# xiezhy6/PASTA-GAN-plusplus

Hardware: AMD Instinct MI355X
Metric: 512-res try-on images/sec (SynthesisNetwork fwd) (higher is better)
Workload: dtype f32

## Files before the change

include/pasta_gan_ops.h:

```cpp
#ifndef PASTA_GAN_OPS_H
#define PASTA_GAN_OPS_H

#include <stdint.h>

#ifdef __cplusplus
extern "C" {
#endif

#define PG_ABI_VERSION 20

enum pg_dtype { PG_F32 = 0, PG_F16 = 1, PG_BF16 = 2, PG_F64 = 3 };

enum pg_error {
    PG_OK = 0,
    PG_ERR_INVALID_ARG = -1,
    PG_ERR_UNSUPPORTED = -2,
    PG_ERR_TOO_LARGE = -3
};

enum pg_act {
    PG_ACT_LINEAR = 1, PG_ACT_RELU = 2, PG_ACT_LRELU = 3, PG_ACT_TANH = 4, PG_ACT_SIGMOID = 5,
    PG_ACT_ELU = 6, PG_ACT_SELU = 7, PG_ACT_SOFTPLUS = 8, PG_ACT_SWISH = 9
};

int pg_bias_act(const void* x, const void* b, const void* xref, const void* yref, const void* dy, void* y,
                int dtype, int64_t sizeX, int sizeB, int64_t stepB,
                int grad, int act, float alpha, float gain, float clamp, void* stream);
int pg_bias_act_abi_version(void);

int64_t pg_bias_act_grad_bias_workspace(int dtype, int64_t sizeX, int sizeB, int64_t stepB);
int pg_bias_act_grad_bias(const void* dy, const void* yref, void* dx, void* db, void* workspace, int64_t workspace_bytes,
                          int dtype, int64_t sizeX, int sizeB, int64_t stepB,
                          int act, float alpha, float gain, float clamp, void* stream);

int pg_upfirdn2d(const void* x, const float* f, void* y, int dtype,
                 int N, int C, int inH, int inW, const int64_t xstride[4],
                 int fh, int fw, const int64_t fstride[2],
                 int outH, int outW, const int64_t ystride[4],
                 int upx, int upy, int downx, int downy, int padx0, int pady0,
                 int flip, float gain, void* stream);
int pg_upfirdn2d_with_odd_samples(const void* x, const float* f, void* y, float* y_odd, int dtype,
                                  int N, int C, int inH, int inW, const int64_t xstride[4],
                                  int fh, int fw, const int64_t fstride[2],
                                  int outH, int outW, const int64_t ystride[4],
                                  int padx0, int pady0, int flip, float gain, void* stream);
typedef struct pg_fir_epilogue {
    const float* noise;
    int64_t      noise_batch_stride;
    float        noise_gain;
    const float* bias;
    int          act;
    float        alpha;
    float        act_gain;
    float        clamp;
} pg_fir_epilogue;
int pg_upfirdn2d_bias_act(const void* x, const float* f, void* y, int dtype,
                          int N, int C, int inH, int inW, const int64_t xstride[4],
                          int fh, int fw, const int64_t fstride[2],
                          int outH, int outW, const int64_t ystride[4],
                          int upx, int upy, int downx, int downy, int padx0, int pady0,
                          int flip, float gain, const pg_fir_epilogue* epilogue, void* stream);
int pg_upfirdn2d_abi_version(void);

int64_t pg_conv2d_packed_size(int Cout, int Cin, int KH, int KW);
int pg_conv2d_pack_weight(const float* w, float* packed, int Cout, int Cin, int KH, int KW,
                          float scale, int flip_hw, int transpose_oi, void* stream);

typedef struct pg_conv2d_fusion {
    const float* in_scale;
    const float* in_bias;
    int          in_act;
    float        in_alpha;
    float        in_gain;
    float        in_clamp;
    const float* out_scale;
    const float* noise;
    int64_t      noise_batch_stride;
    float        noise_gain;
    const float* bias;
    int          act;
    float        alpha;
    float        gain;
    float        clamp;
    const float* residual;
    const float* spade_x;
    const float* spade_mean;
    const float* spade_rstd;
    const float* x2;
    int          cin_split;
    float*       stats_partial;
} pg_conv2d_fusion;

int pg_conv2d_forward(const float* x, const float* packed_w, float* y,
                      int N, int Cin, int H, int W, int Cout, int KH, int KW,
                      int stride, int pad_y, int pad_x, int OH, int OW,
                      const int64_t ystride[4], int out_step_y, int out_step_x, int out_off_y, int out_off_x,
                      const pg_conv2d_fusion* fusion, void* stream);

int pg_conv2d_splitk_plan(int N, int Cin, int OH, int OW, int Cout, int KH, int KW, int stride);
int pg_conv2d_forward_splitk(const float* x, const float* packed_w, float* y,
                             int N, int Cin, int H, int W, int Cout, int KH, int KW,
                             int stride, int pad_y, int pad_x, int OH, int OW,
                             const int64_t ystride[4], int out_step_y, int out_step_x, int out_off_y, int out_off_x,
                             const pg_conv2d_fusion* fusion, float* workspace, int ksplit, void* stream);

enum { PG_WINO_F2 = 1, PG_WINO_F4 = 2, PG_WINO_F4B = 3, PG_WINO_F4X3 = 4 };
int64_t pg_conv2d_winograd_packed_size(int form, int Cout, int Cin);
int pg_conv2d_winograd_pack_weight(int form, const float* w, float* packed, int Cout, int Cin,
                                   float scale, int flip_hw, int transpose_oi, void* stream);
int pg_conv2d_winograd_forward(int form, const float* x, const float* packed_u, float* y,
                               int N, int Cin, int H, int W, int Cout, int pad_y, int pad_x, int OH, int OW,
                               const int64_t ystride[4], const pg_conv2d_fusion* fusion, void* stream);

int pg_conv2d_winograd4_stats_tiles(int OH, int OW);
int pg_instance_norm_finish(const float* stats_partial, float* mean, float* rstd, int NC, int T, int OH, int OW, float eps, void* stream);

int pg_modconv_dcoefs(const float* w, const float* styles, float* dcoefs,
                      int N, int Cout, int Cin, int KHW, float scale, void* stream);

int pg_modconv_w2(const float* w, float* w2, int Cout, int Cin, int KHW, float scale, void* stream);
int pg_modconv_prep(const float* w2, const float* styles, float* out, float* s_norm, void* s16, int half_dtype,
                    int N, int Cout, int Cin, int normalize, int demodulate, void* stream);

#define PG_MODCONV_PREP_MAX_JOBS 32
typedef struct {
    const float* w2[PG_MODCONV_PREP_MAX_JOBS];
    const float* styles[PG_MODCONV_PREP_MAX_JOBS];
    float*       out[PG_MODCONV_PREP_MAX_JOBS];
    float*       s_norm[PG_MODCONV_PREP_MAX_JOBS];
    void*        s16[PG_MODCONV_PREP_MAX_JOBS];
    int          cout[PG_MODCONV_PREP_MAX_JOBS];
    int          cin[PG_MODCONV_PREP_MAX_JOBS];
    int          flags[PG_MODCONV_PREP_MAX_JOBS];
    int          njobs;
    int          half_dtype;
} pg_modconv_prep_jobs;
int pg_modconv_prep_batched(const pg_modconv_prep_jobs* jobs, int N, void* stream);

int pg_conv2d_up2_forward(const float* x, const float* packed, float* y, int N, int Cin, int H, int W, int Cout,
                          const int64_t ystride[4], const float* in_scale, const float* out_scale, void* stream);
int pg_conv2d_up2_splitk_plan(int N, int Cin, int H, int W, int Cout);
int pg_conv2d_up2_forward_splitk(const float* x, const float* packed, float* y, int N, int Cin, int H, int W, int Cout,
                                 const int64_t ystride[4], const float* in_scale, const float* out_scale, float* workspace, int ksplit, void* stream);

int64_t pg_conv2d_up2x3_packed_size(int Cout, int Cin);
int pg_conv2d_up2x3_pack_weight(const float* packed, void* packed_x3, int Cout, int Cin, void* stream);
int pg_conv2d_up2x3_forward(const float* x, const float* packed, const void* packed_x3, float* y, int N, int Cin, int H, int W, int Cout,
                            const int64_t ystride[4], const float* in_scale, const float* out_scale, float* edge_column, void* stream);

int64_t pg_conv2d_stem7x3_packed_size(int Cout);
int pg_conv2d_stem7x3_pack_weight(const float* w, void* packed, int Cout, float scale, int flip_hw, void* stream);
int pg_conv2d_stem7x3_forward(const float* x, const void* packed, float* y, int N, int H, int W, int Cout, const int64_t ystride[4],
                              const pg_conv2d_fusion* fusion, void* stream);

int64_t pg_conv2d_s2x3_packed_size(int Cout, int Cin);
int pg_conv2d_s2x3_pack_weight(const float* packed, void* packed_x3, int Cout, int Cin, void* stream);
int pg_conv2d_s2x3_forward(const float* x, const void* packed_x3, float* y, int N, int Cin, int H, int W, int Cout, const int64_t ystride[4],
                           const pg_conv2d_fusion* fusion, void* stream);

int pg_conv1x1_small(const float* x, const float* w, const float* styles, const float* bias, const float* skip, float* y,
                     int N, int Cin, int64_t HW, int Cout, float scale, float clamp, void* stream);

int pg_conv1x1_fold_prep(const float* wm, const float* bm, const float* wh, const float* bh, const float* styles, float* w_out, float* b_out,
                         int N, int Cm, int C, int Cout, void* stream);
int pg_conv1x1_fold_heads(const float* x, const float* x2, const float* w, const float* bias, const float* skip, float* y_a, float* y_b,
                          int N, int C1, int C2, int64_t HW, int Cout, int c_a, int n_skip, float clamp, void* stream);

int pg_conv3x3_fold_head(const float* xa, const float* xb, const float* w, const float* bias, const float* skip, float* y,
                         int N, int C, int H, int W, int Cout, float clamp, void* stream);

int pg_conv3x3_cin1(const float* x, const float* w, float* y, int N, int H, int W, int Cout, float scale, int act, void* stream);

int pg_instance_norm_stats(const float* x, float* mean, float* rstd, int NC, int64_t HW, float eps, void* stream);
int pg_spade_norm(const float* x, const float* mean, const float* rstd, const float* gamma, const float* beta,
                  float* y, int NC, int64_t HW, void* stream);

#define PG_STATS16_MAX_CHUNKS 256
int pg_instance_norm_stats_cl16(const void* x, float* mean, float* rstd, float* workspace, int dtype, int N, int64_t HW, int C, float eps, void* stream);
int pg_spade_combine_cl16(const void* x, const float* mean, const float* rstd, const void* gamma_beta, void* y, int dtype, int N, int64_t HW, int C,
                          int act, float alpha, float gain, float clamp, void* stream);

int pg_spade_train_forward(const float* x, const float* mean, const float* rstd, const float* gamma, const float* beta, float* y,
                           int N, int C, int64_t HW, int64_t gamma_sample_stride, int64_t beta_sample_stride, void* stream);
int pg_spade_train_backward(const float* dy, const float* x, const float* mean, const float* rstd, const float* gamma, float* sums,
                            float* dx, float* dgamma, float* dbeta, int N, int C, int64_t HW,
                            int64_t gamma_sample_stride, int64_t dgamma_sample_stride, int64_t dbeta_sample_stride, void* stream);

int pg_spade_masked_sums(const float* feat, const float* mask, const float* denorm_mask, float* sums, float* counts,
                         int N, int C, int H, int W, void* stream);
int pg_spade_feat_assemble(const float* feat_upper, const float* feat_lower, const float* mask_upper, const float* mask_lower,
                           const float* denorm_mask_upper, const float* denorm_mask_lower,
                           const float* sums_upper, const float* sums_lower, const float* counts_upper, const float* counts_lower,
                           float* out, int N, int C, int H, int W, void* stream);
int pg_conv2d_abi_version(void);
int pg_conv2d_reserve_cus(int n);

int pg_conv2d_wgrad_plan(int N, int Cin, int OH, int OW, int Cout, int KH, int KW, int stride);
int pg_conv2d_wgrad(const float* x, const float* dy, float* dw, float* workspace,
                    int N, int Cin, int H, int W, int Cout, int KH, int KW, int stride, int pad_y, int pad_x, int OH, int OW,
                    int splits, void* stream);

int pg_conv2d16_wgrad_plan(int N, int Cin, int OH, int OW, int Cout, int KH, int KW, int stride);
int pg_conv2d16_wgrad(const void* x, const void* dy, float* dw, float* workspace, int dtype,
                      int N, int Cin, int H, int W, int Cout, int KH, int KW, int stride, int pad_y, int pad_x, int OH, int OW,
                      int splits, void* stream);

int pg_split3_bf16_cl(const float* x, void* out, int N, int C, int64_t HW, void* stream);
int pg_conv2d16_wgrad_x3(const void* x3, const void* dy3, float* dw, float* workspace,
                         int N, int Cin, int H, int W, int Cout, int KH, int KW, int stride, int pad_y, int pad_x, int OH, int OW,
                         int splits, void* stream);

int64_t pg_conv2d16_packed_size(int Cout, int Cin, int KH, int KW);
int pg_conv2d16_pack_weight(const float* w, void* packed, int dtype, int Cout, int Cin, int KH, int KW,
                            const int* taps_y, int ntaps_y, const int* taps_x, int ntaps_x,
                            float scale, int flip_hw, int transpose_oi,
                            const float* styles, const float* dcoefs, int nsamples, void* stream);
int pg_conv2d16_pack_weight_grouped(const float* w, void* packed, int dtype, int ngroups, int64_t w_group_stride,
                                    int Cout, int Cin, int KH, int KW, float scale, int flip_hw, int transpose_oi,
                                    const float* styles, const float* dcoefs, int nsamples, void* stream);

#define PG_CONV2D16_PACK_MAX_JOBS 16
typedef struct {
    const float* w[PG_CONV2D16_PACK_MAX_JOBS];
    void*        packed[PG_CONV2D16_PACK_MAX_JOBS];
    const float* styles[PG_CONV2D16_PACK_MAX_JOBS];
    const float* dcoefs[PG_CONV2D16_PACK_MAX_JOBS];
    int          cout[PG_CONV2D16_PACK_MAX_JOBS];
    int          cin[PG_CONV2D16_PACK_MAX_JOBS];
    int          flags[PG_CONV2D16_PACK_MAX_JOBS];
    int          dcoefs_mod[PG_CONV2D16_PACK_MAX_JOBS];
    float        scale[PG_CONV2D16_PACK_MAX_JOBS];
    int          njobs;
    int          nsamples;
    int          dtype;
} pg_conv2d16_pack_jobs;
int pg_conv2d16_pack_weight_batched(const pg_conv2d16_pack_jobs* jobs, void* stream);

typedef struct pg_conv2d16_fusion {
    const float* out_scale;
    const float* noise;
    int64_t      noise_batch_stride;
    float        noise_gain;
    const float* bias;
    int          act;
    float        alpha;
    float        gain;
    float        clamp;
    const void*  residual;
    int          phase_cout;
    int64_t      noise_phase_stride;
} pg_conv2d16_fusion;

int pg_conv2d16_forward(const void* x, const void* packed, void* y, int dtype, int out_dtype,
                        int N, int Cin, int H, int W, int Cout, int KH, int KW,
                        int stride, int pad_y, int pad_x, int OH, int OW, int64_t w_sample_stride,
                        const int64_t ystride[4], int out_step_y, int out_step_x, int out_off_y, int out_off_x,
                        const pg_conv2d16_fusion* fusion, void* stream);

int pg_conv2d16_up2_fused(const void* x, const void* packed, void* y, int dtype, int N, int Cin, int H, int W, int Cout,
                          int64_t w_sample_stride, const int64_t ystride[4], const float fir_x[4],
                          const pg_conv2d16_fusion* fusion, void* stream);

int pg_adam_flat_chunk(void);
int pg_adam_flat_step(float* p, float* g, float* m, float* v, const int* chunks, int nchunks, const float* alive, const float* steps_in, float* steps_out,
                      float lr, float beta1, float beta2, float eps, float nan_value, float posinf_value, float neginf_value, void* stream);

int pg_conv2d16_splitk_plan(int N, int Cin, int OH, int OW, int Cout, int KH, int KW, int stride);
int pg_conv2d16_forward_splitk(const void* x, const void* packed, void* y, int dtype, int out_dtype,
                               int N, int Cin, int H, int W, int Cout, int KH, int KW,
                               int stride, int pad_y, int pad_x, int OH, int OW, int64_t w_sample_stride,
                               const int64_t ystride[4], int out_step_y, int out_step_x, int out_off_y, int out_off_x,
                               const pg_conv2d16_fusion* fusion, float* workspace, int ksplit, void* stream);

int pg_conv1x1_small16(const void* x, const float* w, const float* styles, const float* bias, const float* skip, float* y,
                       int dtype, int N, int Cin, int64_t HW, int Cout, float clamp, int skip_up2_width, void* stream);

// ... 166 lines not shown
```

pasta-gan-plusplus_amd/csrc/conv1x1_fold.hip:

```cpp
#include "pg_common.h"

#ifndef PG_FOLD_MIN_WAVES
#define PG_FOLD_MIN_WAVES 1
#endif
#ifndef PG_FOLD_UNROLL
#define PG_FOLD_UNROLL 8
#endif

namespace {
typedef float f32x4s __attribute__((ext_vector_type(4)));

__global__ __launch_bounds__(256) void conv1x1_fold_prep_kernel(const float* __restrict__ wm, const float* __restrict__ bm, const float* __restrict__ wh,
                                                                const float* __restrict__ bh, const float* __restrict__ styles, float* __restrict__ w_out,
                                                                float* __restrict__ b_out, int Cm, int C, int Cout) {
    const int o = blockIdx.x, n = blockIdx.y;
    const float* who = wh + (int64_t)o * Cm;
    const float* sn = styles ? styles + (int64_t)n * Cm : nullptr;
    for (int c = threadIdx.x; c <= C; c += 256) {
        double acc = 0.0;
        if (c < C) {
            for (int k = 0; k < Cm; k++) acc += (double)who[k] * (double)(sn ? sn[k] : 1.f) * (double)wm[(int64_t)k * C + c];
            w_out[((int64_t)n * Cout + o) * C + c] = (float)acc;
        } else {
            if (bm)
                for (int k = 0; k < Cm; k++) acc += (double)who[k] * (double)(sn ? sn[k] : 1.f) * (double)bm[k];
            b_out[(int64_t)n * Cout + o] = (float)(acc + (double)(bh ? bh[o] : 0.f));
        }
    }
}

template <int CP>
__global__ __launch_bounds__(256, PG_FOLD_MIN_WAVES) void conv1x1_fold_heads_kernel(const float* __restrict__ x, const float* __restrict__ x2, const float* __restrict__ w,
                                                                 const float* __restrict__ bias, const float* __restrict__ skip, float* __restrict__ ya,
                                                                 float* __restrict__ yb, int C1, int C2, int64_t HW4, int Cout, int c_a, int n_skip, float clamp) {
    extern __shared__ __attribute__((aligned(16))) float wl[];
    const int n = blockIdx.y, C = C1 + C2;
    const float* wn = w + (int64_t)n * Cout * C;
    for (int e = threadIdx.x; e < CP * C; e += 256) {
        const int c = e / CP, o = e % CP;
        wl[e] = o < Cout ? wn[o * C + c] : 0.f;
    }
    __syncthreads();
    const float cl = clamp >= 0.f ? clamp : __builtin_inff();
    const f32x4s* xa = (const f32x4s*)x + (int64_t)n * C1 * HW4;
    const f32x4s* xb = (const f32x4s*)x2 + (int64_t)n * C2 * HW4;
    for (int64_t p = (int64_t)blockIdx.x * 256 + threadIdx.x; p < HW4; p += (int64_t)gridDim.x * 256) {
        f32x4s acc[CP];
#pragma unroll
        for (int o = 0; o < CP; o++) acc[o] = (f32x4s){0.f, 0.f, 0.f, 0.f};
        auto mac = [&](const f32x4s& xv, const float* wc) __attribute__((always_inline)) {
#pragma unroll
            for (int q = 0; q < CP / 4; q++) {
                const f32x4s wq = *(const f32x4s*)(wc + 4 * q);
#pragma unroll
                for (int j = 0; j < 4; j++) acc[4 * q + j] += xv * wq[j];
            }
        };
        auto walk = [&](const f32x4s* xs, int Cs, const float* ws) __attribute__((always_inline)) {
            int c0 = 0;
            for (; c0 + PG_FOLD_UNROLL <= Cs; c0 += PG_FOLD_UNROLL) {
                f32x4s v[PG_FOLD_UNROLL];
#pragma unroll
                for (int u = 0; u < PG_FOLD_UNROLL; u++) v[u] = xs[(int64_t)(c0 + u) * HW4 + p];
                __builtin_amdgcn_sched_barrier(0);
#pragma unroll
                for (int u = 0; u < PG_FOLD_UNROLL; u++) mac(v[u], ws + (c0 + u) * CP);
            }
            for (; c0 < Cs; c0++) mac(xs[(int64_t)c0 * HW4 + p], ws + c0 * CP);
        };
        walk(xa, C1, wl);
        walk(xb, C2, wl + C1 * CP);
#pragma unroll
        for (int o = 0; o < CP; o++) {
            if (o < Cout) {
                f32x4s r = acc[o] + bias[(int64_t)n * Cout + o];
#pragma unroll
                for (int e = 0; e < 4; e++) r[e] = fminf(fmaxf(r[e], -cl), cl);
                if (o < n_skip) r += ((const f32x4s*)skip)[((int64_t)n * n_skip + o) * HW4 + p];
                if (o < c_a) ((f32x4s*)ya)[((int64_t)n * c_a + o) * HW4 + p] = r;
                else ((f32x4s*)yb)[((int64_t)n * (Cout - c_a) + (o - c_a)) * HW4 + p] = r;
            }
        }
    }
}
}

PG_EXPORT int pg_conv1x1_fold_prep(const float* wm, const float* bm, const float* wh, const float* bh, const float* styles, float* w_out, float* b_out,
                                   int N, int Cm, int C, int Cout, void* stream) {
    if (!wm || !wh || !w_out || !b_out || N <= 0 || Cm <= 0 || C <= 0 || Cout <= 0) return PG_ERR_INVALID_ARG;
    if (N > 65535) return PG_ERR_TOO_LARGE;
    hipLaunchKernelGGL(conv1x1_fold_prep_kernel, dim3((unsigned)Cout, (unsigned)N), dim3(256), 0, (hipStream_t)stream, wm, bm, wh, bh, styles, w_out, b_out, Cm, C, Cout);
    return pg::launch_status();
}

PG_EXPORT int pg_conv1x1_fold_heads(const float* x, const float* x2, const float* w, const float* bias, const float* skip, float* y_a, float* y_b,
                                    int N, int C1, int C2, int64_t HW, int Cout, int c_a, int n_skip, float clamp, void* stream) {
    if (!x || !w || !bias || !y_a || N <= 0 || C1 <= 0 || C2 < 0 || HW <= 0 || Cout <= 0 || c_a <= 0 || c_a > Cout || n_skip < 0 || n_skip > Cout) return PG_ERR_INVALID_ARG;
    if ((C2 > 0 && !x2) || (c_a < Cout && !y_b) || (n_skip > 0 && !skip)) return PG_ERR_INVALID_ARG;
    const int CP = (Cout + 3) / 4 * 4;
    const size_t lds = (size_t)(C1 + C2) * CP * sizeof(float);
    if (Cout > 16 || HW % 4 != 0 || !pg::aligned16(x) || (C2 > 0 && !pg::aligned16(x2)) || !pg::aligned16(y_a) || (c_a < Cout && !pg::aligned16(y_b)) ||
        (n_skip > 0 && !pg::aligned16(skip)) || lds > 64 * 1024)
        return PG_ERR_UNSUPPORTED;
    if (N > 65535) return PG_ERR_TOO_LARGE;
    const int64_t HW4 = HW / 4;
    int64_t bx = (HW4 + 255) / 256;
    const int64_t cap = (int64_t)pg::num_cu() * 8 / N + 1;
    if (bx > cap) bx = cap;
    const dim3 grid((unsigned)bx, (unsigned)N);
    hipStream_t s = (hipStream_t)stream;
#define PG_FOLD(P) case P: hipLaunchKernelGGL((conv1x1_fold_heads_kernel<P>), grid, dim3(256), lds, s, x, x2, w, bias, skip, y_a, y_b, C1, C2, HW4, Cout, c_a, n_skip, clamp); break;
    switch (CP) { PG_FOLD(4) PG_FOLD(8) PG_FOLD(12) PG_FOLD(16) }
#undef PG_FOLD
    return pg::launch_status();
}
```

pasta-gan-plusplus_amd/csrc/conv2d.hip:

```cpp
#include "conv2d_kernel.h"
#include "bf16x3.h"

namespace {

using namespace pg;
using pgconv::ConvParams;
typedef float f32x4 __attribute__((ext_vector_type(4)));

__global__ __launch_bounds__(256) void pack_weight_kernel(const float* __restrict__ w, float* __restrict__ wp, int Cout, int Cin, int KH, int KW,
                                                          int CinP, int CoutP, float scale, int flip, int transpose_oi) {
    const int T = KH * KW;
    const int64_t total = (int64_t)CinP * T * CoutP;
    for (int64_t i = (int64_t)blockIdx.x * 256 + threadIdx.x; i < total; i += (int64_t)gridDim.x * 256) {
        const int co = (int)(i % CoutP);
        const int tap = (int)((i / CoutP) % T);
        const int ci = (int)(i / ((int64_t)CoutP * T));
        float v = 0.f;
        int ky = tap / KW, kx = tap % KW;
        int cs = ci;
        if (Cin == 3 && KH == 7 && KW == 7 && ci == 3 && (ky & 1) == 0 && ky + 1 < KH) { cs = 2; ky += 1; }
        if (co < Cout && cs < Cin) {
            const int ci = cs;
            if (flip) { ky = KH - 1 - ky; kx = KW - 1 - kx; }
            const int64_t src = transpose_oi ? (((int64_t)ci * Cout + co) * KH + ky) * KW + kx
                                             : (((int64_t)co * Cin + ci) * KH + ky) * KW + kx;
            v = w[src] * scale;
        }
        wp[i] = v;
    }
}

__device__ __forceinline__ float wino_gather(const float* __restrict__ w, int co, int ci, int ky, int kx, int Cout, int Cin, float scale, int flip, int transpose_oi) {
    if (co >= Cout || ci >= Cin) return 0.f;
    const int sy = flip ? 2 - ky : ky, sx = flip ? 2 - kx : kx;
    const int64_t src = transpose_oi ? (((int64_t)ci * Cout + co) * 3 + sy) * 3 + sx
                                     : (((int64_t)co * Cin + ci) * 3 + sy) * 3 + sx;
    return w[src] * scale;
}

__global__ __launch_bounds__(256) void wino_pack_kernel(const float* __restrict__ w, float* __restrict__ up, int Cout, int Cin,
                                                        int CinP, int CoutP, float scale, int flip, int transpose_oi) {
    const int64_t total = (int64_t)CinP * CoutP;
    for (int64_t i = (int64_t)blockIdx.x * 256 + threadIdx.x; i < total; i += (int64_t)gridDim.x * 256) {
        const int co = (int)(i % CoutP), ci = (int)(i / CoutP);
        float g[3][3];
#pragma unroll
        for (int ky = 0; ky < 3; ky++)
#pragma unroll
            for (int kx = 0; kx < 3; kx++) g[ky][kx] = wino_gather(w, co, ci, ky, kx, Cout, Cin, scale, flip, transpose_oi);
        float t[4][3];
#pragma unroll
        for (int kx = 0; kx < 3; kx++) {
            t[0][kx] = g[0][kx];
            t[1][kx] = 0.5f * (g[0][kx] + g[1][kx] + g[2][kx]);
            t[2][kx] = 0.5f * (g[0][kx] - g[1][kx] + g[2][kx]);
            t[3][kx] = g[2][kx];
        }
#pragma unroll
        for (int a = 0; a < 4; a++) {
            const float u[4] = {t[a][0], 0.5f * (t[a][0] + t[a][1] + t[a][2]), 0.5f * (t[a][0] - t[a][1] + t[a][2]), t[a][2]};
#pragma unroll
            for (int b = 0; b < 4; b++) {
                const int64_t dst = ((((int64_t)a * (CoutP / 32) + (co >> 5)) * (CinP / 2) + (ci >> 1)) * 2 + (ci & 1)) * 128 + (co & 31) * 4 + b;
                up[dst] = u[b];
            }
        }
    }
}

struct Wino4PackF4 {
    typedef float word;
    static __device__ __forceinline__ void store(float* __restrict__ up, int co, int ci, int a, int b, int nchunks, double u) {
        const int mb = co >> 6, mt = (co >> 5) & 1, m = co & 31;
        const int k = ci >> 4, cc = ci & 15, pair = cc >> 1, h = cc & 1, quad = pair >> 2, sp = pair & 3;
        const int jg = b / 3, jj = b % 3;
        const int64_t unit = ((int64_t)(mb * 2 + mt) * 6 + a) * nchunks + k;
        up[((((unit * 2 + jg) * 2 + quad) * 3 + jj) * 64 + (h * 32 + m)) * 4 + sp] = (float)u;
    }
};
struct Wino4PackF4B {
    typedef float word;
    static __device__ __forceinline__ void store(float* __restrict__ up, int co, int ci, int a, int b, int nchunks, double u) {
        const int mb = co >> 6, cbk = (co >> 4) & 3, m = co & 15;
        const int k = ci >> 4, cc = ci & 15, j = cc >> 2, kq = cc & 3;
// ... 312 lines not shown
            for (int u = 0; u < 2; u++)
                if (ok[u]) {
#pragma unroll
                    for (int k = 0; k < 4; k++) {
                        const float v = m[u][k] * d[u][k];
#pragma unroll
                        for (int g = 0; g < G; g++) s[g] += f[u][g][k] * v;
                        cnt += v;
                    }
                }
        }
    } else {
        for (int i = threadIdx.x; i < H * W; i += IN_THREADS) {
            const int y = i / W, x = i - y * W;
            const int64_t mi = (int64_t)(2 * y) * (2 * W) + 2 * x;
            const float v = (mp[mi] > 0.9f && dp[mi] > 0.9f) ? 1.f : 0.f;
#pragma unroll
            for (int g = 0; g < G; g++) s[g] += fp[g * HWl + i] * v;
            cnt += v;
        }
    }
    const float Cn = block_sum_1024(cnt, red);
#pragma unroll
    for (int g = 0; g < G; g++) {
        const float S = block_sum_1024(s[g], red);
        if (threadIdx.x == 0) sums[plane0 + g] = S;
    }
    if (threadIdx.x == 0 && plane0 % C == 0) counts[n] = Cn;
}

__global__ __launch_bounds__(256) void spade_feat_assemble_kernel(const float* __restrict__ fu, const float* __restrict__ fl,
                                                                  const float* __restrict__ mu, const float* __restrict__ ml,
                                                                  const float* __restrict__ du, const float* __restrict__ dl,
                                                                  const float* __restrict__ su, const float* __restrict__ sl,
                                                                  const float* __restrict__ cu, const float* __restrict__ cl,
                                                                  float* __restrict__ out, int C, int H, int W, int vec) {
    if (vec) {
        const int n = blockIdx.x;
        const float nu = cu[n] > 10.f ? cu[n] : 65536.f, nl = cl[n] > 10.f ? cl[n] : 65536.f;
        const int64_t mb = (int64_t)n * 4 * H * W, HWl = (int64_t)H * W;
        const int W4 = W / 4, n4 = H * W4;
        for (int i = blockIdx.y * 256 + threadIdx.x; i < n4; i += gridDim.y * 256) {
            const int y = i / W4, x4 = i - y * W4;
            const int64_t mi = mb + (int64_t)(2 * y) * (2 * W) + 8 * x4;
            const f32x4 m_u = even_mask4(mu + mi), m_l = even_mask4(ml + mi), d_u = even_mask4(du + mi), d_l = even_mask4(dl + mi);
            f32x4 r_u, r_l;
#pragma unroll
            for (int k = 0; k < 4; k++) { r_u[k] = m_u[k] - m_u[k] * d_u[k]; r_l[k] = m_l[k] - m_l[k] * d_l[k]; }
            const int cz = (C + gridDim.z - 1) / gridDim.z, c_lo = blockIdx.z * cz, c_hi = c_lo + cz < C ? c_lo + cz : C;
#pragma unroll 4
            for (int c = c_lo; c < c_hi; c++) {
                const int plane = n * C + c;
                const float au = su[plane] / nu, al = sl[plane] / nl;
                const int64_t pb = (int64_t)plane * HWl;
                const f32x4 a = ((const f32x4*)(fu + pb))[i], b = ((const f32x4*)(fl + pb))[i];
                f32x4 o;
#pragma unroll
                for (int k = 0; k < 4; k++) {
                    const float b_u = a[k] * (1.f - r_u[k]) + au * r_u[k];
                    const float b_l = b[k] * (1.f - r_l[k]) + al * r_l[k];
                    o[k] = b_u * m_u[k] + b_l * m_l[k];
                }
                ((f32x4*)(out + pb))[i] = o;
            }
        }
        return;
    }
    const int plane = blockIdx.x, n = plane / C;
    const float nu = cu[n] > 10.f ? cu[n] : 65536.f, nl = cl[n] > 10.f ? cl[n] : 65536.f;
    const float au = su[plane] / nu, al = sl[plane] / nl;
    const int64_t pb = (int64_t)plane * H * W, mb = (int64_t)n * 4 * H * W;
    for (int i = blockIdx.y * 256 + threadIdx.x; i < H * W; i += gridDim.y * 256) {
        const int y = i / W, x = i - y * W;
        const int64_t mi = mb + (int64_t)(2 * y) * (2 * W) + 2 * x;
        const float m_u = mu[mi] > 0.9f ? 1.f : 0.f, m_l = ml[mi] > 0.9f ? 1.f : 0.f;
        const float v_u = (m_u != 0.f && du[mi] > 0.9f) ? 1.f : 0.f, v_l = (m_l != 0.f && dl[mi] > 0.9f) ? 1.f : 0.f;
        const float r_u = m_u - v_u, r_l = m_l - v_l;
        const float b_u = fu[pb + i] * (1.f - r_u) + au * r_u;
        const float b_l = fl[pb + i] * (1.f - r_l) + al * r_l;
        out[pb + i] = b_u * m_u + b_l * m_l;
    }
}

__global__ __launch_bounds__(256) void splitk_finish_kernel(const float* __restrict__ ws, float* __restrict__ y, int ksplit, int64_t slice,
                                                            int N, int Cout, int OH, int OW, int64_t ys0, int64_t ys1, int64_t ys2, int64_t ys3,
                                                            int osy, int osx, int ooy, int oox, pg_conv2d_fusion f) {
    const int64_t total = (int64_t)N * Cout * OH * OW;
    const float slope = f.act == PG_ACT_LINEAR ? 1.f : (f.act == PG_ACT_RELU ? 0.f : f.alpha);
    const float cl = f.clamp >= 0.f ? f.clamp : __builtin_inff();
    for (int64_t i = (int64_t)blockIdx.x * 256 + threadIdx.x; i < total; i += (int64_t)gridDim.x * 256) {
        const int ox = (int)(i % OW), oy = (int)((i / OW) % OH), co = (int)((i / ((int64_t)OW * OH)) % Cout), n = (int)(i / ((int64_t)OW * OH * Cout));
        float v = 0.f;
        for (int z = 0; z < ksplit; z++) v += ws[(int64_t)z * slice + i];
        if (f.out_scale) v *= f.out_scale[(int64_t)n * Cout + co];
        if (f.noise) v += f.noise[n * f.noise_batch_stride + (int64_t)oy * OW + ox] * f.noise_gain;
        if (f.bias) v += f.bias[co];
        v = v > 0.f ? v : v * slope;
        v = fminf(fmaxf(v * f.gain, -cl), cl);
        const int64_t off = n * ys0 + co * ys1 + (int64_t)(oy * osy + ooy) * ys2 + (int64_t)(ox * osx + oox) * ys3;
        if (f.residual) v += f.residual[off];
        y[off] = v;
    }
}

inline int round_up(int v, int m) { return (v + m - 1) / m * m; }

}

PG_EXPORT int pg_conv2d_abi_version(void) { return PG_ABI_VERSION; }

PG_EXPORT int pg_conv2d_reserve_cus(int n) {
    pg::reserved_cus().store(n > 0 ? n : 0, std::memory_order_relaxed);
    return pg::num_cu();
}

PG_EXPORT int64_t pg_conv2d_packed_size(int Cout, int Cin, int KH, int KW) {
    if (Cout <= 0 || Cin <= 0 || KH <= 0 || KW <= 0) return 0;
    return (int64_t)round_up(Cin, 16) * KH * KW * round_up(Cout, 32);
}

PG_EXPORT int pg_conv2d_pack_weight(const float* w, float* packed, int Cout, int Cin, int KH, int KW,
                                    float scale, int flip_hw, int transpose_oi, void* stream) {
    if (!w || !packed || Cout <= 0 || Cin <= 0 || KH <= 0 || KW <= 0) return PG_ERR_INVALID_ARG;
    const int CinP = round_up(Cin, 16), CoutP = round_up(Cout, 32);
    const int64_t total = (int64_t)CinP * KH * KW * CoutP;
    int64_t blocks = (total + 255) / 256;
    if (blocks > pg::max_stream_blocks()) blocks = pg::max_stream_blocks();
    hipLaunchKernelGGL(pack_weight_kernel, dim3((unsigned)blocks), dim3(256), 0, (hipStream_t)stream, w, packed, Cout, Cin, KH, KW, CinP, CoutP, scale, flip_hw, transpose_oi);
    return pg::launch_status();
}

static int conv_forward(int form, const float* x, const float* packed_w, float* y,
                        int N, int Cin, int H, int W, int Cout, int KH, int KW,
                        int stride, int pad_y, int pad_x, int OH, int OW,
                        const int64_t ystride[4], int out_step_y, int out_step_x, int out_off_y, int out_off_x,
                        const pg_conv2d_fusion* fusion, void* stream, float* workspace = nullptr, int ksplit = 1) {
    if (!x || !packed_w || !y || !ystride) return PG_ERR_INVALID_ARG;
    if (N <= 0 || Cin <= 0 || H <= 0 || W <= 0 || Cout <= 0 || OH <= 0 || OW <= 0) return PG_ERR_INVALID_ARG;
    if (out_step_y < 1 || out_step_x < 1) return PG_ERR_INVALID_ARG;
    if ((int64_t)Cin * H * W * 4 > 0x7fffffffLL || (int64_t)16 * H * W * 4 > 0x7fffffffLL) return PG_ERR_TOO_LARGE;
    {
        int64_t ext = 1 + (int64_t)(N - 1) * ystride[0] + (int64_t)(Cout - 1) * ystride[1] +
                      ((int64_t)(OH - 1) * out_step_y + out_off_y) * ystride[2] + ((int64_t)(OW - 1) * out_step_x + out_off_x) * ystride[3];
        if (ext > 0x7fffffffLL || (int64_t)N * OH * OW > 0x7fffffffLL) return PG_ERR_TOO_LARGE;
    }
    ConvParams p;
    p.ksplit = 1; p.kpart = 0; p.ws_slice = 0; p.wino_gmap = 0; p.rowpair = 0;
    p.rowpair_pack = 1;
    p.x = x; p.wp = packed_w; p.y = y;
    p.N = N; p.Cin = Cin; p.H = H; p.W = W; p.Cout = Cout; p.CoutP = round_up(Cout, 32); p.OH = OH; p.OW = OW;
    p.pad_y = pad_y; p.pad_x = pad_x;
    for (int i = 0; i < 4; i++) p.ys[i] = ystride[i];
    p.osy = out_step_y; p.osx = out_step_x; p.ooy = out_off_y; p.oox = out_off_x;
    if (fusion) {
        p.f = *fusion;
    } else {
        pg_conv2d_fusion z = {};
        z.in_clamp = -1.f; z.clamp = -1.f;
        p.f = z;
    }
    if (p.f.in_gain == 0.f) p.f.in_gain = 1.f;
    if (p.f.gain == 0.f) p.f.gain = 1.f;
    if (p.f.in_act == 0) p.f.in_act = PG_ACT_LINEAR;
    if (p.f.act == 0) p.f.act = PG_ACT_LINEAR;
    if (p.f.in_act < PG_ACT_LINEAR || p.f.in_act > PG_ACT_SWISH || p.f.act < PG_ACT_LINEAR || p.f.act > PG_ACT_SWISH) return PG_ERR_INVALID_ARG;
    if (p.f.in_act > PG_ACT_LRELU || p.f.act > PG_ACT_LRELU) return PG_ERR_UNSUPPORTED;
// ... 43 lines not shown
        else if (KH == 1 && KW == 2) st = pgconv::launch_k1x2(p, s);
        else if (KH == 7 && KW == 7) st = pgconv::launch_k7s1(p, s);
    } else if (stride == 2) {
        if (KH == 3 && KW == 3) st = pgconv::launch_k3s2(p, s);
        else if (KH == 1 && KW == 1) st = pgconv::launch_k1s2(p, s);
    }
    if (st != PG_OK || ksplit <= 1) return st;
    int64_t blocks = (slice + 255) / 256;
    if (blocks > pg::max_stream_blocks()) blocks = pg::max_stream_blocks();
    hipLaunchKernelGGL(splitk_finish_kernel, dim3((unsigned)blocks), dim3(256), 0, s, workspace, y, ksplit, slice, N, Cout, OH, OW,
                       ystride[0], ystride[1], ystride[2], ystride[3], out_step_y, out_step_x, out_off_y, out_off_x, tail);
    return pg::launch_status();
}

PG_EXPORT int pg_conv2d_forward(const float* x, const float* packed_w, float* y,
                                int N, int Cin, int H, int W, int Cout, int KH, int KW,
                                int stride, int pad_y, int pad_x, int OH, int OW,
                                const int64_t ystride[4], int out_step_y, int out_step_x, int out_off_y, int out_off_x,
                                const pg_conv2d_fusion* fusion, void* stream) {
    return conv_forward(0, x, packed_w, y, N, Cin, H, W, Cout, KH, KW, stride, pad_y, pad_x, OH, OW,
                        ystride, out_step_y, out_step_x, out_off_y, out_off_x, fusion, stream);
}

PG_EXPORT int pg_conv2d_splitk_plan(int N, int Cin, int OH, int OW, int Cout, int KH, int KW, int stride) {
    if (N <= 0 || Cin <= 0 || OH <= 0 || OW <= 0 || Cout <= 0) return 1;
    if (!((stride == 1 && ((KH == 3 && KW == 3) || (KH == 1 && KW == 1) || (KH == 2 && KW == 2) || (KH == 2 && KW == 1) || (KH == 1 && KW == 2) || (KH == 7 && KW == 7))) ||
          (stride == 2 && ((KH == 3 && KW == 3) || (KH == 1 && KW == 1))))) return 1;
    const int kc = pgconv::kc_for(KH, KW, stride);
    const int nchunks = round_up(Cin, kc) / kc;
    const int64_t tiles64 = (int64_t)N * ((OW + pgconv::TW - 1) / pgconv::TW) * ((OH + pgconv::TH - 1) / pgconv::TH) * ((round_up(Cout, 32) + 63) / 64);
    if (tiles64 >= pg::num_cu() || nchunks < 8) return 1;
    int best = 1;
    for (int k = 2; k <= 16; k++)
        if (nchunks % k == 0 && nchunks / k >= 4 && tiles64 * k <= 4 * pg::num_cu()) best = k;
    return best;
}

PG_EXPORT int pg_conv2d_forward_splitk(const float* x, const float* packed_w, float* y,
                                       int N, int Cin, int H, int W, int Cout, int KH, int KW,
                                       int stride, int pad_y, int pad_x, int OH, int OW,
                                       const int64_t ystride[4], int out_step_y, int out_step_x, int out_off_y, int out_off_x,
                                       const pg_conv2d_fusion* fusion, float* workspace, int ksplit, void* stream) {
    if (ksplit < 1 || (ksplit > 1 && !workspace)) return PG_ERR_INVALID_ARG;
    return conv_forward(0, x, packed_w, y, N, Cin, H, W, Cout, KH, KW, stride, pad_y, pad_x, OH, OW,
                        ystride, out_step_y, out_step_x, out_off_y, out_off_x, fusion, stream, workspace, ksplit);
}

PG_EXPORT int64_t pg_conv2d_winograd_packed_size(int form, int Cout, int Cin) {
    static const int per_weight[] = {0, 16, 36, 36, 54};
    if (form < PG_WINO_F2 || form > PG_WINO_F4X3 || Cout <= 0 || Cin <= 0) return 0;
    return (int64_t)per_weight[form] * round_up(Cin, 16) * round_up(Cout, 64);
}

PG_EXPORT int pg_conv2d_winograd_pack_weight(int form, const float* w, float* packed, int Cout, int Cin,
                                             float scale, int flip_hw, int transpose_oi, void* stream) {
    if (form < PG_WINO_F2 || form > PG_WINO_F4X3 || !w || !packed || Cout <= 0 || Cin <= 0) return PG_ERR_INVALID_ARG;
    const int CinP = round_up(Cin, 16), CoutP = round_up(Cout, 64);
    const int64_t total = (int64_t)CinP * CoutP;
    int64_t blocks = (total + 255) / 256;
    if (blocks > pg::max_stream_blocks()) blocks = pg::max_stream_blocks();
    const dim3 grid((unsigned)blocks), block(256);
    hipStream_t s = (hipStream_t)stream;
    switch (form) {
    case PG_WINO_F2:   hipLaunchKernelGGL(wino_pack_kernel, grid, block, 0, s, w, packed, Cout, Cin, CinP, CoutP, scale, flip_hw, transpose_oi); break;
    case PG_WINO_F4:   hipLaunchKernelGGL(wino4_pack_kernel<Wino4PackF4>, grid, block, 0, s, w, packed, Cout, Cin, CinP, CoutP, scale, flip_hw, transpose_oi); break;
    case PG_WINO_F4B:  hipLaunchKernelGGL(wino4_pack_kernel<Wino4PackF4B>, grid, block, 0, s, w, packed, Cout, Cin, CinP, CoutP, scale, flip_hw, transpose_oi); break;
    case PG_WINO_F4X3: hipLaunchKernelGGL(wino4_pack_kernel<Wino4PackF4X3>, grid, block, 0, s, w, (unsigned short*)packed, Cout, Cin, CinP, CoutP, scale, flip_hw, transpose_oi); break;
    }
    return pg::launch_status();
}

PG_EXPORT int pg_conv2d_winograd_forward(int form, const float* x, const float* packed_u, float* y,
                                         int N, int Cin, int H, int W, int Cout, int pad_y, int pad_x, int OH, int OW,
                                         const int64_t ystride[4], const pg_conv2d_fusion* fusion, void* stream) {
    if (form < PG_WINO_F2 || form > PG_WINO_F4X3) return PG_ERR_INVALID_ARG;
    return conv_forward(form, x, packed_u, y, N, Cin, H, W, Cout, 3, 3, 1, pad_y, pad_x, OH, OW, ystride, 1, 1, 0, 0, fusion, stream);
}

namespace {
typedef float f32x4s __attribute__((ext_vector_type(4)));
template <int COUT>
__global__ __launch_bounds__(256) void conv1x1_small_f32_kernel(const float* __restrict__ x, const float* __restrict__ w, const float* __restrict__ styles,
                                                                const float* __restrict__ bias, const float* __restrict__ skip, float* __restrict__ y,
                                                                int Cin, int64_t HW4, float scale, float clamp) {
    extern __shared__ __attribute__((aligned(16))) float wl[];
    const int n = blockIdx.y;
    for (int e = threadIdx.x; e < 8 * Cin; e += 256) {
        const int c = e >> 3, o = e & 7;
        wl[e] = o < COUT ? w[o * Cin + c] * scale * (styles ? styles[(int64_t)n * Cin + c] : 1.f) : 0.f;
    }
    __syncthreads();
    const float cl = clamp >= 0.f ? clamp : __builtin_inff();
    const f32x4s* xn = (const f32x4s*)x + (int64_t)n * Cin * HW4;
    for (int64_t p = (int64_t)blockIdx.x * 256 + threadIdx.x; p < HW4; p += (int64_t)gridDim.x * 256) {
        f32x4s acc[COUT];
#pragma unroll
        for (int o = 0; o < COUT; o++) acc[o] = (f32x4s){0.f, 0.f, 0.f, 0.f};
        auto mac = [&](const f32x4s& xv, int c) __attribute__((always_inline)) {
            const f32x4s w0 = *(const f32x4s*)(wl + c * 8), w1 = *(const f32x4s*)(wl + c * 8 + 4);
#pragma unroll
            for (int o = 0; o < COUT; o++) acc[o] += xv * (o < 4 ? w0[o & 3] : w1[o & 3]);
        };
        int c0 = 0;
        for (; c0 + 8 <= Cin; c0 += 8) {
            f32x4s v[8];
#pragma unroll
            for (int u = 0; u < 8; u++) v[u] = xn[(int64_t)(c0 + u) * HW4 + p];
            __builtin_amdgcn_sched_barrier(0);
#pragma unroll
            for (int u = 0; u < 8; u++) mac(v[u], c0 + u);
        }
        for (; c0 < Cin; c0++) mac(xn[(int64_t)c0 * HW4 + p], c0);
#pragma unroll
        for (int o = 0; o < COUT; o++) {
            f32x4s r = acc[o] + (bias ? bias[o] : 0.f);
#pragma unroll
            for (int e = 0; e < 4; e++) r[e] = fminf(fmaxf(r[e], -cl), cl);
            const int64_t off = ((int64_t)n * COUT + o) * HW4 + p;
            if (skip) r += ((const f32x4s*)skip)[off];
            ((f32x4s*)y)[off] = r;
        }
    }
}


template <int COUT, int QB>
__global__ __launch_bounds__(256) void conv1x1_small_f32_split_kernel(const float* __restrict__ x, const float* __restrict__ w, const float* __restrict__ styles,
                                                                      const float* __restrict__ bias, const float* __restrict__ skip, float* __restrict__ y,
                                                                      int Cin, int64_t HW4, float scale, float clamp) {
    constexpr int CS = 256 / QB;
    static_assert(QB * COUT <= 256, "one output thread per (quad, channel)");
    __shared__ f32x4s part[CS][COUT][QB];
    const int n = blockIdx.y;
    const int q = threadIdx.x % QB, cs = threadIdx.x / QB;
    const int64_t p = (int64_t)blockIdx.x * QB + q;
    const bool live = p < HW4;
    const f32x4s* xn = (const f32x4s*)x + (int64_t)n * Cin * HW4 + (live ? p : 0);
    const float* sn = styles ? styles + (int64_t)n * Cin : nullptr;
    f32x4s acc[COUT];
#pragma unroll
    for (int o = 0; o < COUT; o++) acc[o] = (f32x4s){0.f, 0.f, 0.f, 0.f};
    for (int c0 = cs; c0 < Cin; c0 += 8 * CS) {
        f32x4s v[8];
        float wv[8][COUT];
#pragma unroll
        for (int u = 0; u < 8; u++) {
            const int c = c0 + u * CS;
            const bool ok = c < Cin;
            v[u] = ok ? xn[(int64_t)c * HW4] : (f32x4s){0.f, 0.f, 0.f, 0.f};
            const float sc = ok ? scale * (sn ? sn[c] : 1.f) : 0.f;
#pragma unroll
            for (int o = 0; o < COUT; o++) wv[u][o] = ok ? w[o * Cin + c] * sc : 0.f;
        }
#pragma unroll
        for (int u = 0; u < 8; u++)
#pragma unroll
            for (int o = 0; o < COUT; o++) acc[o] += v[u] * wv[u][o];
    }
#pragma unroll
    for (int o = 0; o < COUT; o++) part[cs][o][q] = acc[o];
    __syncthreads();
    if (threadIdx.x < QB * COUT) {
        const int oq = threadIdx.x % QB, o = threadIdx.x / QB;
        const int64_t po = (int64_t)blockIdx.x * QB + oq;
        f32x4s r = part[0][o][oq];
#pragma unroll 8
        for (int z = 1; z < CS; z++) r += part[z][o][oq];
        r += bias ? bias[o] : 0.f;
        const float cl = clamp >= 0.f ? clamp : __builtin_inff();
#pragma unroll
        for (int e = 0; e < 4; e++) r[e] = fminf(fmaxf(r[e], -cl), cl);
        if (po < HW4) {
            const int64_t off = ((int64_t)n * COUT + o) * HW4 + po;
            if (skip) r += ((const f32x4s*)skip)[off];
            ((f32x4s*)y)[off] = r;
        }
    }
}


template <bool RELU>
__global__ __launch_bounds__(256) void conv3x3_cin1_kernel(const float* __restrict__ x, const float* __restrict__ w, float* __restrict__ y,
                                                           int H, int W, int Cout, float scale) {
    const int n = blockIdx.y;
    const int W4 = W >> 2;
    const int64_t HW = (int64_t)H * W;
    const float* xn = x + (int64_t)n * HW;
    for (int64_t q = (int64_t)blockIdx.x * 256 + threadIdx.x; q < (int64_t)H * W4; q += (int64_t)gridDim.x * 256) {
        const int oy = (int)(q / W4), ox = 4 * (int)(q % W4);
        float v[3][6];
#pragma unroll
        for (int r = 0; r < 3; r++) {
            const int gy = oy + r - 1;
            const bool row_ok = gy >= 0 && gy < H;
            const float* row = xn + (int64_t)(row_ok ? gy : 0) * W;
            const f32x4s m = *(const f32x4s*)(row + ox);
            const float l = row[ox > 0 ? ox - 1 : 0], rr = row[ox + 4 < W ? ox + 4 : W - 1];
            v[r][0] = (row_ok && ox > 0) ? l : 0.f;
            v[r][5] = (row_ok && ox + 4 < W) ? rr : 0.f;
#pragma unroll
            for (int e = 0; e < 4; e++) v[r][1 + e] = row_ok ? m[e] : 0.f;
        }
        f32x4s* yo = (f32x4s*)(y + (int64_t)n * Cout * HW + (int64_t)oy * W + ox);
        for (int co = 0; co < Cout; co++) {
            const float* wc = w + co * 9;
            f32x4s acc = {0.f, 0.f, 0.f, 0.f};
#pragma unroll
            for (int r = 0; r < 3; r++)
#pragma unroll
                for (int k = 0; k < 3; k++) {
                    const float wk = wc[r * 3 + k] * scale;
#pragma unroll
                    for (int e = 0; e < 4; e++) acc[e] = fmaf(v[r][e + k], wk, acc[e]);
                }
            if (RELU) {
#pragma unroll
                for (int e = 0; e < 4; e++) acc[e] = fmaxf(acc[e], 0.f);
            }
            yo[(int64_t)co * (HW >> 2)] = acc;
        }
    }
}
}

PG_EXPORT int pg_conv1x1_small(const float* x, const float* w, const float* styles, const float* bias, const float* skip, float* y,
                               int N, int Cin, int64_t HW, int Cout, float scale, float clamp, void* stream) {
    if (!x || !w || !y || N <= 0 || Cin <= 0 || HW <= 0 || Cout <= 0) return PG_ERR_INVALID_ARG;
    if (Cout > 8 || HW % 4 != 0 || !pg::aligned16(x) || !pg::aligned16(y) || (skip && !pg::aligned16(skip)) || (size_t)Cin * 32 > 64 * 1024) return PG_ERR_UNSUPPORTED;
    if (N > 65535) return PG_ERR_TOO_LARGE;
    const int64_t HW4 = HW / 4;
    hipStream_t s = (hipStream_t)stream;
    static const bool split_on = [] { const char* e = getenv("PG_HEAD32_SPLIT"); return !e || atoi(e) != 0; }();
    if (split_on && (int64_t)N * ((HW4 + 255) / 256) < (int64_t)pg::num_cu() / 2 && Cin >= 64) {
        int qb = 4;
        if ((int64_t)N * ((HW4 + 15) / 16) >= 2 * (int64_t)pg::num_cu()) qb = 16;
        const dim3 g2((unsigned)((HW4 + qb - 1) / qb), (unsigned)N);
#define PG_SPLIT(C) case C: \
        if (qb == 16) hipLaunchKernelGGL((conv1x1_small_f32_split_kernel<C, 16>), g2, dim3(256), 0, s, x, w, styles, bias, skip, y, Cin, HW4, scale, clamp); \
        else hipLaunchKernelGGL((conv1x1_small_f32_split_kernel<C, 4>), g2, dim3(256), 0, s, x, w, styles, bias, skip, y, Cin, HW4, scale, clamp); \
        break;
        switch (Cout) { PG_SPLIT(1) PG_SPLIT(2) PG_SPLIT(3) PG_SPLIT(4) PG_SPLIT(5) PG_SPLIT(6) PG_SPLIT(7) PG_SPLIT(8) }
#undef PG_SPLIT
        return pg::launch_status();
    }
    int64_t bx = (HW4 + 255) / 256;
    const int64_t cap = (int64_t)pg::num_cu() * 8 / N + 1;
    if (bx > cap) bx = cap;
    const dim3 grid((unsigned)bx, (unsigned)N);
    const size_t lds = (size_t)Cin * 32;
#define PG_SMALL(C) case C: hipLaunchKernelGGL((conv1x1_small_f32_kernel<C>), grid, dim3(256), lds, s, x, w, styles, bias, skip, y, Cin, HW4, scale, clamp); break;
    switch (Cout) { PG_SMALL(1) PG_SMALL(2) PG_SMALL(3) PG_SMALL(4) PG_SMALL(5) PG_SMALL(6) PG_SMALL(7) PG_SMALL(8) }
#undef PG_SMALL
    return pg::launch_status();
}

PG_EXPORT int pg_conv3x3_cin1(const float* x, const float* w, float* y, int N, int H, int W, int Cout, float scale, int act, void* stream) {
    if (!x || !w || !y || N <= 0 || H <= 0 || W <= 0 || Cout <= 0) return PG_ERR_INVALID_ARG;
    if (act != PG_ACT_LINEAR && act != PG_ACT_RELU) return PG_ERR_UNSUPPORTED;
    if (W % 4 != 0 || !pg::aligned16(x) || !pg::aligned16(y)) return PG_ERR_UNSUPPORTED;
    if (N > 65535 || (int64_t)Cout * H * W > 0x7fffffffLL * 4) return PG_ERR_TOO_LARGE;
    int64_t bx = ((int64_t)H * (W / 4) + 255) / 256;
    const int64_t cap = (int64_t)pg::num_cu() * 8 / N + 1;
    if (bx > cap) bx = cap;
    const dim3 grid((unsigned)bx, (unsigned)N);
    if (act == PG_ACT_RELU) hipLaunchKernelGGL(conv3x3_cin1_kernel<true>, grid, dim3(256), 0, (hipStream_t)stream, x, w, y, H, W, Cout, scale);
    else hipLaunchKernelGGL(conv3x3_cin1_kernel<false>, grid, dim3(256), 0, (hipStream_t)stream, x, w, y, H, W, Cout, scale);
    return pg::launch_status();
}

PG_EXPORT int pg_modconv_dcoefs(const float* w, const float* styles, float* dcoefs,
                                int N, int Cout, int Cin, int KHW, float scale, void* stream) {
    if (!w || !styles || !dcoefs || N <= 0 || Cout <= 0 || Cin <= 0 || KHW <= 0) return PG_ERR_INVALID_ARG;
    hipLaunchKernelGGL(dcoefs_kernel, dim3((unsigned)(N * Cout)), dim3(256), 0, (hipStream_t)stream, w, styles, dcoefs, Cout, Cin, KHW, scale);
    return pg::launch_status();
}

PG_EXPORT int pg_modconv_w2(const float* w, float* w2, int Cout, int Cin, int KHW, float scale, void* stream) {
    if (!w || !w2 || Cout <= 0 || Cin <= 0 || KHW <= 0) return PG_ERR_INVALID_ARG;
    const int64_t total = (int64_t)Cout * Cin;
    hipLaunchKernelGGL(modconv_w2_kernel, dim3((unsigned)((total + 255) / 256)), dim3(256), 0, (hipStream_t)stream, w, w2, total, KHW, scale * scale);
    return pg::launch_status();
}

PG_EXPORT int pg_modconv_prep(const float* w2, const float* styles, float* out, float* s_norm, void* s16, int half_dtype,
                              int N, int Cout, int Cin, int normalize, int demodulate, void* stream) {
    if (!styles || !out || N <= 0 || Cout <= 0 || Cin <= 0 || (demodulate && !w2)) return PG_ERR_INVALID_ARG;
    if (s16 && half_dtype != PG_BF16 && half_dtype != PG_F16) return PG_ERR_INVALID_ARG;
    if (N > 65535 || (size_t)Cin * 4 > 64 * 1024) return PG_ERR_TOO_LARGE;
    hipLaunchKernelGGL(modconv_prep_kernel, dim3((unsigned)((Cout + 15) / 16), (unsigned)N), dim3(256), (size_t)Cin * 4, (hipStream_t)stream,
                       w2, styles, out, s_norm, (unsigned short*)s16, half_dtype, Cout, Cin, normalize, demodulate);
    return pg::launch_status();
}

PG_EXPORT int pg_modconv_prep_batched(const pg_modconv_prep_jobs* jobs, int N, void* stream) {
    if (!jobs || N <= 0 || N > 65535 || jobs->njobs <= 0 || jobs->njobs > PG_MODCONV_PREP_MAX_JOBS) return PG_ERR_INVALID_ARG;
    if (jobs->half_dtype != 0 && jobs->half_dtype != PG_BF16 && jobs->half_dtype != PG_F16) return PG_ERR_INVALID_ARG;
    int max_cout = 0, max_cin = 0;
    for (int j = 0; j < jobs->njobs; j++) {
        const int dem = (jobs->flags[j] >> 1) & 1;
        if (!jobs->styles[j] || !jobs->out[j] || jobs->cout[j] <= 0 || jobs->cin[j] <= 0 || (dem && !jobs->w2[j])) return PG_ERR_INVALID_ARG;
        if (jobs->s16[j] && !jobs->half_dtype) return PG_ERR_INVALID_ARG;
        if (jobs->cout[j] > max_cout) max_cout = jobs->cout[j];
        if (jobs->cin[j] > max_cin) max_cin = jobs->cin[j];
    }
    if ((size_t)max_cin * 4 > 64 * 1024) return PG_ERR_TOO_LARGE;
    hipLaunchKernelGGL(modconv_prep_batched_kernel, dim3((unsigned)((max_cout + 15) / 16), (unsigned)N, (unsigned)jobs->njobs), dim3(256), (size_t)max_cin * 4,
                       (hipStream_t)stream, *jobs);
    return pg::launch_status();
}

PG_EXPORT int pg_instance_norm_stats(const float* x, float* mean, float* rstd, int NC, int64_t HW, float eps, void* stream) {
    if (!x || !mean || !rstd || NC <= 0 || HW <= 0) return PG_ERR_INVALID_ARG;
    hipLaunchKernelGGL(instance_norm_stats_kernel, dim3((unsigned)NC), dim3(IN_THREADS), 0, (hipStream_t)stream, x, mean, rstd, HW, eps);
    return pg::launch_status();
}

__global__ __launch_bounds__(64) void instance_norm_finish_kernel(const float* __restrict__ part, float* __restrict__ mean, float* __restrict__ rstd, int T, int OH, int OW, float eps) {
    const float* pp = part + (int64_t)blockIdx.x * T * 2;
    const int tiles_x = (OW + 63) / 64;
    double n = 0.0, s = 0.0, q = 0.0;
    auto merge = [](double& na, double& sa, double& qa, double nb, double sb, double qb) {
        if (nb <= 0.0) return;
        if (na <= 0.0) { na = nb; sa = sb; qa = qb; return; }
        const double d = sb / nb - sa / na;
        qa += qb + d * d * na * nb / (na + nb);
        sa += sb; na += nb;
    };
    for (int t = threadIdx.x; t < T; t += 64) {
        const int ty = t / tiles_x, tx = t - ty * tiles_x;
        const int rows = OH - ty * 8 < 8 ? OH - ty * 8 : 8, cols = OW - tx * 64 < 64 ? OW - tx * 64 : 64;
        merge(n, s, q, (double)rows * cols, (double)pp[2 * t], (double)pp[2 * t + 1]);
    }
#pragma unroll
// ... 29 lines not shown
    if (blocks > pg::max_stream_blocks()) blocks = pg::max_stream_blocks();
    if (vec)
        hipLaunchKernelGGL(spade_norm_kernel, dim3((unsigned)blocks), dim3(256), 0, (hipStream_t)stream, x, mean, rstd, gamma, beta, y, HW / 4, total / 4);
    else
        hipLaunchKernelGGL(spade_norm_scalar_kernel, dim3((unsigned)blocks), dim3(256), 0, (hipStream_t)stream, x, mean, rstd, gamma, beta, y, HW, total);
    return pg::launch_status();
}

PG_EXPORT int pg_spade_train_forward(const float* x, const float* mean, const float* rstd, const float* gamma, const float* beta, float* y,
                                     int N, int C, int64_t HW, int64_t gamma_sample_stride, int64_t beta_sample_stride, void* stream) {
    if (!x || !mean || !rstd || !gamma || !beta || !y || N <= 0 || C <= 0 || HW <= 0) return PG_ERR_INVALID_ARG;
    const int64_t total = (int64_t)N * C * HW;
    const bool vec = HW % 4 == 0 && gamma_sample_stride % 4 == 0 && beta_sample_stride % 4 == 0 && pg::aligned16(x) && pg::aligned16(gamma) && pg::aligned16(beta) && pg::aligned16(y);
    int64_t blocks = ((vec ? total / 4 : total) + 255) / 256;
    if (blocks > pg::max_stream_blocks()) blocks = pg::max_stream_blocks();
    if (vec)
        hipLaunchKernelGGL(spade_train_forward_kernel<4>, dim3((unsigned)blocks), dim3(256), 0, (hipStream_t)stream, x, mean, rstd, gamma, beta, y, C, HW / 4, total / 4,
                           gamma_sample_stride, beta_sample_stride);
    else
        hipLaunchKernelGGL(spade_train_forward_kernel<1>, dim3((unsigned)blocks), dim3(256), 0, (hipStream_t)stream, x, mean, rstd, gamma, beta, y, C, HW, total,
                           gamma_sample_stride, beta_sample_stride);
    return pg::launch_status();
}

PG_EXPORT int pg_spade_train_backward(const float* dy, const float* x, const float* mean, const float* rstd, const float* gamma, float* sums,
                                      float* dx, float* dgamma, float* dbeta, int N, int C, int64_t HW,
                                      int64_t gamma_sample_stride, int64_t dgamma_sample_stride, int64_t dbeta_sample_stride, void* stream) {
    if (!dy || !x || !mean || !rstd || !gamma || !sums || N <= 0 || C <= 0 || HW <= 0 || (!dgamma != !dbeta) || (!dx && !dgamma)) return PG_ERR_INVALID_ARG;
    const int64_t total = (int64_t)N * C * HW;
    const bool vec = HW % 4 == 0 && gamma_sample_stride % 4 == 0 && dgamma_sample_stride % 4 == 0 && dbeta_sample_stride % 4 == 0 && pg::aligned16(dy) && pg::aligned16(x) &&
                     pg::aligned16(gamma) && (!dx || pg::aligned16(dx)) && (!dgamma || (pg::aligned16(dgamma) && pg::aligned16(dbeta)));
    if (dx)
        hipLaunchKernelGGL(spade_train_sums_kernel, dim3((unsigned)(N * C)), dim3(IN_THREADS), 0, (hipStream_t)stream, dy, x, mean, rstd, gamma, sums, C, HW,
                           gamma_sample_stride, (int)vec);
    int64_t blocks = ((vec ? total / 4 : total) + 255) / 256;
    if (blocks > pg::max_stream_blocks()) blocks = pg::max_stream_blocks();
    if (vec)
        hipLaunchKernelGGL(spade_train_backward_kernel<4>, dim3((unsigned)blocks), dim3(256), 0, (hipStream_t)stream, dy, x, mean, rstd, gamma, (const float*)sums, dx, dgamma, dbeta,
                           C, HW / 4, total / 4, gamma_sample_stride, dgamma_sample_stride, dbeta_sample_stride);
    else
        hipLaunchKernelGGL(spade_train_backward_kernel<1>, dim3((unsigned)blocks), dim3(256), 0, (hipStream_t)stream, dy, x, mean, rstd, gamma, (const float*)sums, dx, dgamma, dbeta,
                           C, HW, total, gamma_sample_stride, dgamma_sample_stride, dbeta_sample_stride);
    return pg::launch_status();
}

PG_EXPORT int pg_spade_masked_sums(const float* feat, const float* mask, const float* denorm_mask, float* sums, float* counts,
                                   int N, int C, int H, int W, void* stream) {
    if (!feat || !mask || !denorm_mask || !sums || !counts || N <= 0 || C <= 0 || H <= 0 || W <= 0) return PG_ERR_INVALID_ARG;
    if ((int64_t)H * W > 0x3fffffffLL) return PG_ERR_TOO_LARGE;
    const int vec = (W % 4 == 0 && pg::aligned16(feat) && pg::aligned16(mask) && pg::aligned16(denorm_mask)) ? 1 : 0;
    static const int grp = [] { const char* e = getenv("PG_SPADE_SUMS_G"); return e ? atoi(e) : 0; }();
    const int g = grp ? grp : ((int64_t)N * C / 4 >= pg::num_cu() ? 4 : 2);
    if (g == 4 && C % 4 == 0) hipLaunchKernelGGL(spade_masked_sums_kernel<4>, dim3((unsigned)(N * C / 4)), dim3(IN_THREADS), 0, (hipStream_t)stream, feat, mask, denorm_mask, sums, counts, C, H, W, vec);
    else if (g >= 2 && C % 2 == 0) hipLaunchKernelGGL(spade_masked_sums_kernel<2>, dim3((unsigned)(N * C / 2)), dim3(IN_THREADS), 0, (hipStream_t)stream, feat, mask, denorm_mask, sums, counts, C, H, W, vec);
    else hipLaunchKernelGGL(spade_masked_sums_kernel<1>, dim3((unsigned)(N * C)), dim3(IN_THREADS), 0, (hipStream_t)stream, feat, mask, denorm_mask, sums, counts, C, H, W, vec);
    return pg::launch_status();
}

PG_EXPORT int pg_spade_feat_assemble(const float* feat_upper, const float* feat_lower, const float* mask_upper, const float* mask_lower,
                                     const float* denorm_mask_upper, const float* denorm_mask_lower,
                                     const float* sums_upper, const float* sums_lower, const float* counts_upper, const float* counts_lower,
                                     float* out, int N, int C, int H, int W, void* stream) {
    if (!feat_upper || !feat_lower || !mask_upper || !mask_lower || !denorm_mask_upper || !denorm_mask_lower || !sums_upper || !sums_lower ||
        !counts_upper || !counts_lower || !out || N <= 0 || C <= 0 || H <= 0 || W <= 0) return PG_ERR_INVALID_ARG;
    if ((int64_t)H * W > 0x3fffffffLL) return PG_ERR_TOO_LARGE;
    const int vec = (W % 4 == 0 && pg::aligned16(feat_upper) && pg::aligned16(feat_lower) && pg::aligned16(out) && pg::aligned16(mask_upper) && pg::aligned16(mask_lower) &&
                     pg::aligned16(denorm_mask_upper) && pg::aligned16(denorm_mask_lower)) ? 1 : 0;
    int chunks = (int)(((int64_t)H * W + 256 * 16 - 1) / (256 * 16));
    if (chunks < 1) chunks = 1;
    if (chunks > 64) chunks = 64;
    if (vec) {
        chunks = (int)(((int64_t)H * (W / 4) + 255) / 256);
        const int want = (8 * pg::num_cu() + N - 1) / N;
        if (chunks > want) chunks = want;
        if (chunks < 1) chunks = 1;
    }
    static const int zsplit = [] { const char* e = getenv("PG_SPADE_ASM_Z"); return e && atoi(e) > 0 ? atoi(e) : 2; }();
    const int gz = vec ? (C >= 4 * zsplit ? zsplit : 1) : 1;
    hipLaunchKernelGGL(spade_feat_assemble_kernel, dim3((unsigned)(vec ? N : N * C), (unsigned)chunks, (unsigned)gz), dim3(256), 0, (hipStream_t)stream,
                       feat_upper, feat_lower, mask_upper, mask_lower, denorm_mask_upper, denorm_mask_lower,
                       sums_upper, sums_lower, counts_upper, counts_lower, out, C, H, W, vec);
    return pg::launch_status();
}
```

pasta-gan-plusplus_amd/csrc/conv3x3_fold.hip:

```cpp
#include "pg_common.h"

namespace {
typedef float f32x4s __attribute__((ext_vector_type(4)));
typedef unsigned u32x4s __attribute__((ext_vector_type(4)));

constexpr int F3_ROWS = 4;
constexpr int F3_WAVES = 4;
constexpr int F3_COLS = 256;
constexpr int F3_OOB = 0x40000000;
constexpr int DPP_WAVE_SHL1 = 0x130, DPP_WAVE_SHR1 = 0x138;

template <int CTRL> __device__ __forceinline__ float dpp_or(float old, float v) {
    return __builtin_bit_cast(float, __builtin_amdgcn_update_dpp(__builtin_bit_cast(int, old), __builtin_bit_cast(int, v), CTRL, 0xf, 0xf, false));
}

struct F3Planes {
    f32x4s a[F3_ROWS + 2];
    float e[F3_ROWS + 2];
    f32x4s b[F3_ROWS];
};

template <int CO>
__global__ __launch_bounds__(256, 2) void conv3x3_fold_head_kernel(const float* __restrict__ xa, const float* __restrict__ xb, const float* __restrict__ w,
                                                                   const float* __restrict__ bias, const float* __restrict__ skip, float* __restrict__ y,
                                                                   int C, int H, int W, float clamp) {
    const int n = blockIdx.z;
    const int wave = __builtin_amdgcn_readfirstlane((int)threadIdx.x >> 6), lane = (int)threadIdx.x & 63;
    const int r0 = ((int)blockIdx.y * F3_WAVES + wave) * F3_ROWS;
    if (r0 >= H) return;
    const int col = (int)blockIdx.x * F3_COLS + lane * 4;
    const bool colok = col < W;
    const int plane_bytes = H * W * 4;
    const int off_col = colok ? col * 4 : F3_OOB;
    const int off_edge = lane == 0 ? (col > 0 && colok ? (col - 1) * 4 : F3_OOB) : (lane == 63 && col + 4 < W ? (col + 4) * 4 : F3_OOB);
    int off_a[F3_ROWS + 2], off_e[F3_ROWS + 2];
#pragma unroll
    for (int j = 0; j < F3_ROWS + 2; j++) {
        const int r = r0 - 1 + j;
        const int ro = r >= 0 && r < H ? r * W * 4 : F3_OOB;
        off_a[j] = ro + off_col;
        off_e[j] = ro + off_edge;
    }
    const float* pa = xa + (int64_t)n * C * H * W;
    const float* pb = xb + (int64_t)n * C * H * W;
    const float* wn = w + (int64_t)n * CO * 10 * C;
    const int64_t HW = (int64_t)H * W;

    auto load = [&](int c, F3Planes& p) __attribute__((always_inline)) {
        const __amdgpu_buffer_rsrc_t ra = __builtin_amdgcn_make_buffer_rsrc(const_cast<float*>(pa + c * HW), 0, plane_bytes, 0x00020000);
        const __amdgpu_buffer_rsrc_t rb = __builtin_amdgcn_make_buffer_rsrc(const_cast<float*>(pb + c * HW), 0, plane_bytes, 0x00020000);
#pragma unroll
        for (int j = 0; j < F3_ROWS + 2; j++) p.a[j] = __builtin_bit_cast(f32x4s, __builtin_amdgcn_raw_buffer_load_b128(ra, off_a[j], 0, 0));
#pragma unroll
        for (int j = 0; j < F3_ROWS; j++) p.b[j] = __builtin_bit_cast(f32x4s, __builtin_amdgcn_raw_buffer_load_b128(rb, off_a[j + 1], 0, 0));
#pragma unroll
        for (int j = 0; j < F3_ROWS + 2; j++) p.e[j] = __builtin_bit_cast(float, __builtin_amdgcn_raw_buffer_load_b32(ra, off_e[j], 0, 0));
    };

    float acc[CO][F3_ROWS][4];
#pragma unroll
    for (int o = 0; o < CO; o++)
#pragma unroll
        for (int t = 0; t < F3_ROWS; t++)
#pragma unroll
            for (int q = 0; q < 4; q++) acc[o][t][q] = 0.f;

    auto mac = [&](int c, const F3Planes& p) __attribute__((always_inline)) {
        float w3[CO][9], w1[CO];
#pragma unroll
        for (int o = 0; o < CO; o++) {
#pragma unroll
            for (int k = 0; k < 9; k++) w3[o][k] = wn[o * 10 * C + c * 9 + k];
            w1[o] = wn[o * 10 * C + 9 * C + c];
        }
        float v[F3_ROWS + 2][6];
#pragma unroll
        for (int j = 0; j < F3_ROWS + 2; j++) {
            v[j][0] = dpp_or<DPP_WAVE_SHR1>(p.e[j], p.a[j][3]);
            v[j][1] = p.a[j][0]; v[j][2] = p.a[j][1]; v[j][3] = p.a[j][2]; v[j][4] = p.a[j][3];
            v[j][5] = dpp_or<DPP_WAVE_SHL1>(p.e[j], p.a[j][0]);
        }
#pragma unroll
        for (int t = 0; t < F3_ROWS; t++) {
            float part[CO][4];
#pragma unroll
            for (int o = 0; o < CO; o++)
#pragma unroll
                for (int q = 0; q < 4; q++) part[o][q] = p.b[t][q] * w1[o];
#pragma unroll
            for (int ky = 0; ky < 3; ky++)
#pragma unroll
                for (int kx = 0; kx < 3; kx++)
#pragma unroll
                    for (int o = 0; o < CO; o++)
#pragma unroll
                        for (int q = 0; q < 4; q++) part[o][q] = __builtin_fmaf(v[t + ky][q + kx], w3[o][3 * ky + kx], part[o][q]);
#pragma unroll
            for (int o = 0; o < CO; o++)
#pragma unroll
                for (int q = 0; q < 4; q++) acc[o][t][q] += part[o][q];
        }
    };

    F3Planes pA, pB;
    load(0, pA);
    int c = 0;
    for (; c + 1 < C; c += 2) {
        load(c + 1, pB);
        __builtin_amdgcn_sched_barrier(0);
        mac(c, pA);
        if (c + 2 < C) load(c + 2, pA);
        __builtin_amdgcn_sched_barrier(0);
        mac(c + 1, pB);
    }
    if (c < C) mac(c, pA);

    if (!colok) return;
    const float cl = clamp >= 0.f ? clamp : __builtin_inff();
#pragma unroll
    for (int o = 0; o < CO; o++) {
        const float bo = bias[n * CO + o];
#pragma unroll
        for (int t = 0; t < F3_ROWS; t++) {
            if (r0 + t < H) {
                const int64_t at = (((int64_t)n * CO + o) * H + (r0 + t)) * W + col;
                f32x4s r;
#pragma unroll
                for (int q = 0; q < 4; q++) r[q] = fminf(fmaxf(acc[o][t][q] + bo, -cl), cl);
                if (skip) r += *(const f32x4s*)(skip + at);
                *(f32x4s*)(y + at) = r;
            }
        }
    }
}
}

PG_EXPORT int pg_conv3x3_fold_head(const float* xa, const float* xb, const float* w, const float* bias, const float* skip, float* y,
                                   int N, int C, int H, int W, int Cout, float clamp, void* stream) {
    if (!xa || !xb || !w || !bias || !y || N <= 0 || C <= 0 || H <= 0 || W <= 0 || Cout <= 0) return PG_ERR_INVALID_ARG;
    if (Cout > 4 || W % 4 != 0 || !pg::aligned16(xa) || !pg::aligned16(xb) || !pg::aligned16(y) || (skip && !pg::aligned16(skip))) return PG_ERR_UNSUPPORTED;
    if ((int64_t)H * W * 4 > (int64_t)1 << 29 || (int64_t)C * 10 * Cout > (int64_t)1 << 24) return PG_ERR_UNSUPPORTED;
    const int64_t by = ((int64_t)H + F3_WAVES * F3_ROWS - 1) / (F3_WAVES * F3_ROWS);
    if (N > 65535 || by > 65535) return PG_ERR_TOO_LARGE;
    const dim3 grid((unsigned)((W + F3_COLS - 1) / F3_COLS), (unsigned)by, (unsigned)N);
    hipStream_t s = (hipStream_t)stream;
#define PG_FOLD3(P) case P: hipLaunchKernelGGL((conv3x3_fold_head_kernel<P>), grid, dim3(64 * F3_WAVES), 0, s, xa, xb, w, bias, skip, y, C, H, W, clamp); break;
    switch (Cout) { PG_FOLD3(1) PG_FOLD3(2) PG_FOLD3(3) PG_FOLD3(4) }
#undef PG_FOLD3
    return pg::launch_status();
}
```

pasta-gan-plusplus_amd/torch_utils/custom_ops.py:

```python

import concurrent.futures
import ctypes
import fcntl
import glob
import hashlib
import os
import re
import shutil
import subprocess
import sys

verbosity = 'brief'

CSRC_DIR = os.path.normpath(os.path.join(os.path.dirname(os.path.abspath(__file__)), '..', 'csrc'))
INCLUDE_DIR = os.path.normpath(os.path.join(CSRC_DIR, '..', '..', 'include'))
DEV_DIR = os.path.join(CSRC_DIR, 'dev')
OFFLOAD_ARCH = 'gfx950'
HIPCC_FLAGS = ['-O3', '-std=c++17', '-fPIC', '-fvisibility=hidden', f'--offload-arch={OFFLOAD_ARCH}']

PLUGIN_SOURCES = {
    'bias_act_plugin': ['bias_act.hip'],
    'upfirdn2d_plugin': ['upfirdn2d.hip'],
    'patch_routing_plugin': ['patch_routing.hip'],
    'augment_plugin': ['augment.hip'],
    'tryon_plugin': ['tryon.hip'],
    'tryon_front_plugin': ['tryon_front.hip'],
    'train_fetch_plugin': ['train_fetch.hip'],
    'snapshot_grid_plugin': ['snapshot_grid.hip'],
    'vgg_loss_plugin': ['vgg_loss.hip'],
    'image_metrics_plugin': ['image_metrics.hip'],
    'conv2d_plugin': ['conv2d.hip', 'conv2d_inst_k3s1.hip', 'conv2d_inst_k1s1.hip', 'conv2d_inst_k2x2.hip', 'conv2d_inst_k2x1.hip',
                      'conv2d_inst_k1x2.hip', 'conv2d_inst_k7s1.hip', 'conv2d_inst_k3s2.hip', 'conv2d_inst_k1s2.hip', 'conv2d_inst_wino.hip', 'conv2d_inst_wino4.hip', 'conv2d_inst_wino4s.hip', 'conv2d_inst_wino4t.hip', 'conv2d_inst_wino4x.hip', 'conv2d_inst_wino4xs.hip', 'conv2d_inst_wino4xt.hip', 'conv2d_inst_wino4b.hip', 'conv2d_inst_wino4bs.hip', 'conv2d_inst_up2.hip', 'conv2d_inst_stem7.hip', 'conv2d_inst_s2x3.hip', 'conv2d_inst_s1x1.hip',
                      'conv2d_wgrad.hip', 'conv2d16.hip', 'conv2d16_inst_k3s1.hip', 'conv2d16_inst_k3s1b.hip', 'conv2d16_inst_k1s1.hip', 'conv2d16_inst_k2x2.hip', 'conv2d16_inst_k2x1.hip',
                      'conv2d16_inst_k1x2.hip', 'conv2d16_inst_k3s2.hip', 'conv2d16_inst_up2f.hip', 'conv1x1_head16.hip', 'spade16.hip', 'conv1x1_fold.hip', 'conv3x3_fold.hip', 'optim.hip'],
}

ABI_VERSION = 20

_cached_plugins = dict()


class NativePlugin:

    def __init__(self, name, path, abi_name=None):
        self.name = name
        self.path = path
        self.lib = ctypes.CDLL(path)
        probe = getattr(self.lib, 'pg_' + (abi_name or name).replace('_plugin', '') + '_abi_version', None)
        if probe is None:
            raise RuntimeError(f'{path} does not export its ABI version; rebuild it from csrc/')
        probe.restype = ctypes.c_int
        if probe() != ABI_VERSION:
            raise RuntimeError(f'{path} implements ABI version {probe()}, the bindings expect {ABI_VERSION}; rebuild it from csrc/')

    def __repr__(self):
        return f'<NativePlugin {self.name} at {self.path}>'


def _find_hipcc():
    for cand in (os.environ.get('HIPCC'), shutil.which('hipcc'), '/opt/rocm/bin/hipcc'):
        if cand and os.path.isfile(cand):
            return cand
    return None


def _digest(sources, extra_flags):
    h = hashlib.md5()
    deps = sorted(set(list(sources) + glob.glob(os.path.join(CSRC_DIR, '*.h')) + glob.glob(os.path.join(INCLUDE_DIR, '*.h'))))
    for path in deps:
        h.update(os.path.basename(path).encode())
        with open(path, 'rb') as f:
            h.update(f.read())
    h.update(' '.join(HIPCC_FLAGS + list(extra_flags)).encode())
    return h.hexdigest()


def _log(msg, end='\n'):
    if verbosity != 'none':
        print(msg, end=end, flush=True)


def source_flags(src):
    flags = []
    with open(src) as f:
        for _ in range(8):
            m = re.match(r'\s*//\s*hipcc-flags:\s*(.*)', f.readline())
            if m:
                flags += m.group(1).split()
    return flags


def _compile_one(hipcc, src, obj, extra_flags):
    cmd = [hipcc] + HIPCC_FLAGS + list(extra_flags) + source_flags(src) + ['-I', INCLUDE_DIR, '-I', CSRC_DIR, '-c', src, '-o', obj]
    if verbosity == 'full':
        print(' '.join(cmd), flush=True)
    proc = subprocess.run(cmd, stdout=subprocess.PIPE, stderr=subprocess.STDOUT, text=True)
    if proc.returncode != 0:
        raise RuntimeError(f'hipcc failed on {src}:\n{proc.stdout}')
    return obj


def _build(module_name, sources, so_path, digest, extra_flags):
    hipcc = _find_hipcc()
    if hipcc is None:
        raise RuntimeError(f'cannot build "{module_name}": hipcc not found and no up-to-date {so_path}')
    obj_dir = os.path.join(CSRC_DIR, 'build', module_name)
    os.makedirs(obj_dir, exist_ok=True)
    jobs = max(1, min(len(sources), int(os.environ.get('PG_BUILD_JOBS', os.cpu_count() or 1))))
    objs = [os.path.join(obj_dir, os.path.splitext(os.path.basename(s))[0] + '.o') for s in sources]
    with concurrent.futures.ThreadPoolExecutor(max_workers=jobs) as pool:
        list(pool.map(lambda so: _compile_one(hipcc, so[0], so[1], extra_flags), zip(sources, objs)))
    tmp = so_path + f'.tmp{os.getpid()}'
    cmd = [hipcc, '-shared', '-fPIC', f'--offload-arch={OFFLOAD_ARCH}', '-o', tmp] + objs
    try:
        proc = subprocess.run(cmd, stdout=subprocess.PIPE, stderr=subprocess.STDOUT, text=True)
        if proc.returncode != 0:
            raise RuntimeError(f'link of {module_name} failed:\n{proc.stdout}')
        os.replace(tmp, so_path)
    finally:
        clean(only=module_name)
# ... 130 lines not shown
```

pasta-gan-plusplus_amd/torch_utils/ops/conv2d_mfma.py:

```python

import contextlib
import ctypes
import os
import weakref

import torch

from .. import custom_ops
from . import _native as nat

ACT_INDEX = {'linear': 1, 'relu': 2, 'lrelu': 3, 'tanh': 4, 'sigmoid': 5, 'elu': 6, 'selu': 7, 'softplus': 8, 'swish': 9}

FUSED_ACTS = ('linear', 'relu', 'lrelu')

SUPPORTED = {(3, 3, 1), (1, 1, 1), (2, 2, 1), (2, 1, 1), (1, 2, 1), (7, 7, 1), (3, 3, 2), (1, 1, 2)}


class Fusion(ctypes.Structure):
    _fields_ = [
        ('in_scale', ctypes.c_void_p), ('in_bias', ctypes.c_void_p), ('in_act', ctypes.c_int), ('in_alpha', ctypes.c_float),
        ('in_gain', ctypes.c_float), ('in_clamp', ctypes.c_float),
        ('out_scale', ctypes.c_void_p), ('noise', ctypes.c_void_p), ('noise_batch_stride', ctypes.c_int64), ('noise_gain', ctypes.c_float),
        ('bias', ctypes.c_void_p), ('act', ctypes.c_int), ('alpha', ctypes.c_float), ('gain', ctypes.c_float), ('clamp', ctypes.c_float),
        ('residual', ctypes.c_void_p),
# ... 2 lines not shown
        ('stats_partial', ctypes.c_void_p),
    ]


_plugin = None

_timeline = None
_wgrad_timeline = None


def reserve_cus(n):
    lib = _init().lib
    lib.pg_conv2d_reserve_cus.restype = ctypes.c_int
    lib.pg_conv2d_reserve_cus.argtypes = [ctypes.c_int]
    return int(lib.pg_conv2d_reserve_cus(int(n)))


def start_timeline():
    global _timeline
    _timeline = []
    return _timeline


def start_wgrad_timeline():
    global _wgrad_timeline
    _wgrad_timeline = []
    return _wgrad_timeline


def stop_wgrad_timeline():
    global _wgrad_timeline
    tl, _wgrad_timeline = _wgrad_timeline, None
    return tl


def stop_timeline():
    global _timeline
    tl, _timeline = _timeline, None
    return tl


def timed_launch(tl):
    if tl is None:
        return None
    ev0, ev1 = torch.cuda.Event(enable_timing=True), torch.cuda.Event(enable_timing=True)
    ev0.record()

    def done(key, flops, nbytes):
        ev1.record()
        tl.append((key, flops, ev0, ev1, nbytes))
    return done


def _init(plugin_name='conv2d_plugin'):
    global _plugin
    if _plugin is None:
        plugin = custom_ops.get_plugin(plugin_name)
        lib = plugin.lib
        i, f, vp, i64 = ctypes.c_int, ctypes.c_float, ctypes.c_void_p, ctypes.c_int64
        lib.pg_conv2d_packed_size.restype = i64
        lib.pg_conv2d_packed_size.argtypes = [i, i, i, i]
        lib.pg_conv2d_pack_weight.restype = i
        lib.pg_conv2d_pack_weight.argtypes = [vp, vp, i, i, i, i, f, i, i, vp]
        lib.pg_conv2d_forward.restype = i
        lib.pg_conv2d_forward.argtypes = [vp, vp, vp, i, i, i, i, i, i, i, i, i, i, i, i, ctypes.POINTER(i64), i, i, i, i, ctypes.POINTER(Fusion), vp]
        lib.pg_conv2d_splitk_plan.restype = i
        lib.pg_conv2d_splitk_plan.argtypes = [i] * 8
        lib.pg_conv2d_forward_splitk.restype = i
        lib.pg_conv2d_forward_splitk.argtypes = [vp, vp, vp, i, i, i, i, i, i, i, i, i, i, i, i, ctypes.POINTER(i64), i, i, i, i, ctypes.POINTER(Fusion), vp, i, vp]
        lib.pg_conv2d_winograd_packed_size.restype = i64
        lib.pg_conv2d_winograd_packed_size.argtypes = [i, i, i]
        lib.pg_conv2d_winograd_pack_weight.restype = i
        lib.pg_conv2d_winograd_pack_weight.argtypes = [i, vp, vp, i, i, f, i, i, vp]
        lib.pg_conv2d_winograd_forward.restype = i
        lib.pg_conv2d_winograd_forward.argtypes = [i, vp, vp, vp, i, i, i, i, i, i, i, i, i, ctypes.POINTER(i64), ctypes.POINTER(Fusion), vp]
        lib.pg_conv2d_winograd4_stats_tiles.restype = i
        lib.pg_conv2d_winograd4_stats_tiles.argtypes = [i, i]
        lib.pg_instance_norm_finish.restype = i
        lib.pg_instance_norm_finish.argtypes = [vp, vp, vp, i, i, i, i, f, vp]
        lib.pg_spade_masked_sums.restype = i
        lib.pg_spade_masked_sums.argtypes = [vp, vp, vp, vp, vp, i, i, i, i, vp]
        lib.pg_spade_feat_assemble.restype = i
        lib.pg_spade_feat_assemble.argtypes = [vp] * 11 + [i, i, i, i, vp]
        lib.pg_modconv_dcoefs.restype = i
        lib.pg_modconv_dcoefs.argtypes = [vp, vp, vp, i, i, i, i, f, vp]
        lib.pg_modconv_w2.restype = i
        lib.pg_modconv_w2.argtypes = [vp, vp, i, i, i, f, vp]
        lib.pg_modconv_prep.restype = i
        lib.pg_modconv_prep.argtypes = [vp, vp, vp, vp, vp, i, i, i, i, i, i, vp]
        lib.pg_modconv_prep_batched.restype = i
        lib.pg_modconv_prep_batched.argtypes = [ctypes.POINTER(PrepJobs), i, vp]
        lib.pg_instance_norm_stats.restype = i
        lib.pg_instance_norm_stats.argtypes = [vp, vp, vp, i, i64, f, vp]
        lib.pg_spade_norm.restype = i
        lib.pg_spade_norm.argtypes = [vp, vp, vp, vp, vp, vp, i, i64, vp]
        lib.pg_spade_train_forward.restype = i
        lib.pg_spade_train_forward.argtypes = [vp] * 6 + [i, i, i64, i64, i64, vp]
        lib.pg_spade_train_backward.restype = i
        lib.pg_spade_train_backward.argtypes = [vp] * 9 + [i, i, i64, i64, i64, i64, vp]
        lib.pg_conv2d_wgrad_plan.restype = i
        lib.pg_conv2d_wgrad_plan.argtypes = [i] * 8
        lib.pg_conv2d_wgrad.restype = i
        lib.pg_conv2d_wgrad.argtypes = [vp, vp, vp, vp] + [i] * 13 + [vp]
        lib.pg_conv2d_up2_forward.restype = i
        lib.pg_conv2d_up2_forward.argtypes = [vp, vp, vp, i, i, i, i, i, ctypes.POINTER(ctypes.c_int64), vp, vp, vp]
        lib.pg_split3_bf16_cl.restype = i
        lib.pg_split3_bf16_cl.argtypes = [vp, vp, i, i, i64, vp]
        lib.pg_conv2d16_wgrad_x3.restype = i
        lib.pg_conv2d16_wgrad_x3.argtypes = [vp, vp, vp, vp] + [i] * 13 + [vp]
        lib.pg_conv2d16_wgrad_plan.restype = i
        lib.pg_conv2d16_wgrad_plan.argtypes = [i] * 8
        lib.pg_conv2d_up2_splitk_plan.restype = i
        lib.pg_conv2d_up2_splitk_plan.argtypes = [i, i, i, i, i]
        lib.pg_conv2d_up2x3_packed_size.restype = i64
        lib.pg_conv2d_up2x3_packed_size.argtypes = [i, i]
        lib.pg_conv2d_up2x3_pack_weight.restype = i
        lib.pg_conv2d_up2x3_pack_weight.argtypes = [vp, vp, i, i, vp]
        lib.pg_conv2d_up2x3_forward.restype = i
        lib.pg_conv2d_up2x3_forward.argtypes = [vp, vp, vp, vp, i, i, i, i, i, ctypes.POINTER(ctypes.c_int64), vp, vp, vp, vp]
        lib.pg_conv2d_up2_forward_splitk.restype = i
        lib.pg_conv2d_up2_forward_splitk.argtypes = [vp, vp, vp, i, i, i, i, i, ctypes.POINTER(ctypes.c_int64), vp, vp, vp, i, vp]
        lib.pg_conv2d_stem7x3_packed_size.restype = i64
        lib.pg_conv2d_stem7x3_packed_size.argtypes = [i]
        lib.pg_conv2d_stem7x3_pack_weight.restype = i
        lib.pg_conv2d_stem7x3_pack_weight.argtypes = [vp, vp, i, ctypes.c_float, i, vp]
        lib.pg_conv2d_stem7x3_forward.restype = i
        lib.pg_conv2d_stem7x3_forward.argtypes = [vp, vp, vp, i, i, i, i, ctypes.POINTER(ctypes.c_int64), ctypes.POINTER(Fusion), vp]
        lib.pg_conv2d_s2x3_packed_size.restype = i64
        lib.pg_conv2d_s2x3_packed_size.argtypes = [i, i]
        lib.pg_conv2d_s2x3_pack_weight.restype = i
        lib.pg_conv2d_s2x3_pack_weight.argtypes = [vp, vp, i, i, vp]
        lib.pg_conv2d_s2x3_forward.restype = i
        lib.pg_conv2d_s2x3_forward.argtypes = [vp, vp, vp, i, i, i, i, i, ctypes.POINTER(i64), ctypes.POINTER(Fusion), vp]
        lib.pg_conv3x3_cin1.restype = i
        lib.pg_conv3x3_cin1.argtypes = [vp, vp, vp, i, i, i, i, f, i, vp]
        lib.pg_conv1x1_small.restype = i
        lib.pg_conv1x1_small.argtypes = [vp] * 6 + [i, i, i64, i, f, f, vp]
        lib.pg_conv1x1_fold_prep.restype = i
        lib.pg_conv1x1_fold_prep.argtypes = [vp] * 7 + [i, i, i, i, vp]
        lib.pg_conv1x1_fold_heads.restype = i
        lib.pg_conv1x1_fold_heads.argtypes = [vp] * 7 + [i, i, i, i64, i, i, i, f, vp]
        lib.pg_conv3x3_fold_head.restype = i
        lib.pg_conv3x3_fold_head.argtypes = [vp] * 6 + [i, i, i, i, i, f, vp]
        _plugin = plugin
    return _plugin


WINO_F2, WINO_F4, WINO_F4B, WINO_F4X3 = 1, 2, 3, 4
WINO_FORMS = {0: ('direct', False, False), WINO_F2: ('winograd', False, False), WINO_F4: ('winograd4', True, False),
              WINO_F4B: ('winograd4', False, True), WINO_F4X3: ('winograd4x3', True, False)}


def _wino_form(winograd):
    if int(winograd) not in WINO_FORMS:
        raise nat.NativeOpError(f'conv2d_mfma: winograd={winograd!r} is not one of the forms {sorted(WINO_FORMS)}')
    return (int(winograd), *WINO_FORMS[int(winograd)])


_WINO4B = os.environ.get('PG_WINO4B', '1')
F4_FORM = WINO_F4 if _WINO4B == '0' else WINO_F4B
F4_WIDE = WINO_F4 if os.environ.get('PG_WINO4_X3', '1') == '0' else WINO_F4X3


def f4_form(hw):
    if _WINO4B == '2':
        return WINO_F4B
    return F4_FORM if int(hw[1]) < 64 else F4_WIDE


_algo_override = []


@contextlib.contextmanager
def algo(mode):
    if mode is None:
        yield
        return
    assert mode in ('auto', 'direct', 'winograd', 'winograd2', 'winograd4')
    _algo_override.append(mode)
    try:
        yield
    finally:
        _algo_override.pop()


def use_winograd(kh, kw, stride, cout, cin=None, x2=None, pad=None, hw=None, xf=False, ep=None):
    if (int(kh), int(kw), int(stride)) != (3, 3, 1) or x2 is not None:
        return 0
    if pad is not None and not 0 <= int(pad[1]) <= 4:
        return 0
    mode = _algo_override[-1] if _algo_override else os.environ.get('PG_CONV_ALGO', 'auto')
    if mode == 'direct':
        return 0
    f4_possible = hw is not None and not xf and int(hw[1]) % 4 == 0 and (pad is None or (int(hw[1]) + 2 * int(pad[1]) - 2) % 4 == 0)
    if ep:
        gain = ep.get('gain', 1.0)
        alpha = ep.get('alpha', 0.2)
        if (gain is not None and not float(gain) > 0) or (ep.get('act', 'linear') == 'lrelu' and alpha is not None and not 0 <= float(alpha) <= 1):
            f4_possible = False
    if mode == 'winograd4' and f4_possible:
        return f4_form(hw)
    if mode in ('winograd', 'winograd2', 'winograd4'):
        return WINO_F2
    if not (int(cout) > 32 and (cin is None or int(cin) >= 16)):
        return 0
    if f4_possible and cin is not None and int(cin) >= 64 and int(cin) % 16 == 0 and int(cout) % 64 == 0 and int(hw[0]) >= 32 and int(hw[1]) >= 32:
        return f4_form(hw)
    return WINO_F2


def supported(kh, kw, stride):
    return (int(kh), int(kw), int(stride)) in SUPPORTED


def _f32c(t, name):
    if t is None:
        return None
    if t.dtype != torch.float32 or not t.is_cuda:
        raise nat.NativeOpError(f'conv2d_mfma: {name} must be a float32 GPU tensor')
    return t.contiguous()


def pack_weight(w, scale=1.0, flip=False, transpose_oi=False, winograd=False):
    lib = _init().lib
    w = _f32c(w.detach(), 'weight')
    if transpose_oi:
# ... 345 lines not shown
    with torch.cuda.device(x.device):
        done = timed_launch(_timeline)
        ksplit = lib.pg_conv2d_up2_splitk_plan(n, cin, h, w, cout)
        x3 = packs.get('x3') if (x3 is not False and UP2_X3 and ksplit == 1 and w > 16 and w % 4 == 0 and cin % 16 == 0 and cin >= 32 and x.data_ptr() % 16 == 0) else None
        if x3 is not None:
            xcol = torch.empty([n * cin * h], dtype=torch.float32, device=x.device) if edge_column else None
            st = lib.pg_conv2d_up2x3_forward(nat.ptr(x), nat.ptr(packs['main']), nat.ptr(x3), nat.ptr(y), n, cin, h, w, cout, nat.i64arr(y.stride()), nat.ptr(s_in), nat.ptr(s_out),
                                             nat.ptr(xcol), nat.stream_of(x))
        elif ksplit > 1:
            ws = torch.empty([ksplit * buf.numel()], dtype=torch.float32, device=x.device)
            st = lib.pg_conv2d_up2_forward_splitk(nat.ptr(x), nat.ptr(packs['main']), nat.ptr(y), n, cin, h, w, cout, nat.i64arr(y.stride()), nat.ptr(s_in), nat.ptr(s_out),
                                                  nat.ptr(ws), ksplit, nat.stream_of(x))
        else:
            st = lib.pg_conv2d_up2_forward(nat.ptr(x), nat.ptr(packs['main']), nat.ptr(y), n, cin, h, w, cout, nat.i64arr(y.stride()), nat.ptr(s_in), nat.ptr(s_out),
                                           nat.stream_of(x))
        if done:
            done((3, 3, 2, 'direct', f'N{n} {cin}->{cout} {h}x{w} up2' + (' x3' if x3 is not None else '') + (' mod' if in_scale is not None else '')), 2.0 * n * cout * cin * 9 * h * w,
                 4 * (x.numel() + n * cout * oh * ow))
    nat.check(st, 'pg_conv2d_up2_forward')
    return y


STEM7_X3 = os.environ.get('PG_STEM7_X3', '1') != '0'


def pack_stem7(weight, scale=1.0, flip=False):
    lib = _init().lib
    w = _f32c(weight.detach(), 'weight')
    cout, cin, kh, kw = w.shape
    if (cin, kh, kw) != (3, 7, 7):
        raise nat.NativeOpError('conv2d_mfma.pack_stem7: a [Cout, 3, 7, 7] kernel')
    packed = torch.empty([lib.pg_conv2d_stem7x3_packed_size(cout)], dtype=torch.uint8, device=w.device)
    with torch.cuda.device(w.device):
        nat.check(lib.pg_conv2d_stem7x3_pack_weight(nat.ptr(w), nat.ptr(packed), cout, float(scale), int(bool(flip)), nat.stream_of(w)), 'pg_conv2d_stem7x3_pack_weight')
    return packed


def conv_stem7_forward(x, packed, cout, bias=None, act='linear', alpha=0.0, gain=1.0, clamp=None):
    lib = _init().lib
    x = _f32c(x, 'x')
    n, cin, h, w = x.shape
    if cin != 3 or act not in FUSED_ACTS:
        raise nat.NativeNotCovered('conv2d_mfma.conv_stem7_forward: three input channels, linear / relu / lrelu')
    y = torch.empty([n, cout, h, w], dtype=torch.float32, device=x.device)
    fz = Fusion()
    b = _f32c(bias, 'bias') if bias is not None else None
    fz.bias = b.data_ptr() if b is not None else None
    fz.act, fz.alpha, fz.gain = ACT_INDEX[act], float(alpha), float(gain)
    fz.clamp = -1.0 if clamp is None else float(clamp)
    fz.in_clamp, fz.in_gain = -1.0, 1.0
    with torch.cuda.device(x.device):
        done = timed_launch(_timeline)
        st = lib.pg_conv2d_stem7x3_forward(nat.ptr(x), nat.ptr(packed), nat.ptr(y), n, h, w, cout, nat.i64arr(y.stride()), ctypes.byref(fz), nat.stream_of(x))
        if done:
            done((7, 7, 1, 'direct', f'N{n} 3->{cout} {h}x{w} x3'), 2.0 * n * cout * h * w * 3 * 49, 4 * (x.numel() + y.numel()))
    if st == -2:
        raise nat.NativeNotCovered('pg_conv2d_stem7x3_forward declined the launch')
    nat.check(st, 'pg_conv2d_stem7x3_forward')
    return y


def conv3x3_cin1_ok(x, weight, padding=1):
    return (x.dtype == torch.float32 and x.is_cuda and x.is_contiguous() and int(x.shape[1]) == 1 and tuple(weight.shape[1:]) == (1, 3, 3)
            and int(padding) == 1 and x.shape[3] % 4 == 0)


def conv3x3_cin1(x, weight, scale=1.0, act='linear'):
    lib = _init().lib
    n, _, h, w = x.shape
    cout = int(weight.shape[0])
    wf = _f32c(weight.detach(), 'weight')
    y = torch.empty([n, cout, h, w], dtype=torch.float32, device=x.device)
    with torch.cuda.device(x.device):
        rc = lib.pg_conv3x3_cin1(nat.ptr(x), nat.ptr(wf), nat.ptr(y), n, h, w, cout, float(scale), ACT_INDEX[act], nat.stream_of(x))
    nat.check(rc, 'pg_conv3x3_cin1')
    return y


def conv1x1_small_ok(x, weight, skip=None):
    return (x.dtype == torch.float32 and x.is_cuda and x.is_contiguous() and tuple(weight.shape[2:]) == (1, 1) and int(weight.shape[0]) <= 8
            and (x.shape[2] * x.shape[3]) % 4 == 0 and int(x.shape[1]) <= 2048 and (skip is None or (skip.dtype == torch.float32 and skip.is_contiguous())))


def conv1x1_small(x, weight, styles=None, bias=None, skip=None, scale=1.0, clamp=None):
    lib = _init().lib
    n, cin, h, w = x.shape
    cout = int(weight.shape[0])
    wf = _f32c(weight.detach().reshape(cout, cin), 'weight')
    st = _f32c(styles.detach(), 'styles') if styles is not None else None
    b = _f32c(bias.detach(), 'bias') if bias is not None else None
    y = torch.empty([n, cout, h, w], dtype=torch.float32, device=x.device)
    with torch.cuda.device(x.device):
        rc = lib.pg_conv1x1_small(nat.ptr(x), nat.ptr(wf), nat.ptr(st), nat.ptr(b), nat.ptr(skip), nat.ptr(y), n, cin, h * w, cout,
                                  float(scale), float(clamp) if clamp is not None else -1.0, nat.stream_of(x))
    nat.check(rc, 'pg_conv1x1_small')
    return y


def conv1x1_fold_ok(x, x2, skip=None):
    return (x.dtype == torch.float32 and x.is_cuda and x.is_contiguous() and x2.dtype == torch.float32 and x2.is_cuda and x2.is_contiguous()
            and x.shape[0] == x2.shape[0] and x.shape[2:] == x2.shape[2:] and (x.shape[2] * x.shape[3]) % 4 == 0
            and (skip is None or (skip.dtype == torch.float32 and skip.is_cuda and skip.is_contiguous() and skip.shape[0] == x.shape[0] and skip.shape[2:] == x.shape[2:])))


def conv1x1_fold_prep(wm, bm, wh, bh, styles):
    lib = _init().lib
    wm, bm, wh, bh, styles = _f32c(wm, 'wm'), _f32c(bm, 'bm'), _f32c(wh, 'wh'), _f32c(bh, 'bh'), _f32c(styles, 'styles')
    cm, c = wm.shape
    cout, n = int(wh.shape[0]), int(styles.shape[0])
    if tuple(wh.shape) != (cout, cm) or tuple(styles.shape) != (n, cm) or (bm is not None and bm.numel() != cm) or (bh is not None and bh.numel() != cout):
        raise nat.NativeOpError('conv1x1_fold_prep: wm [Cm, C], bm [Cm], wh [Cout, Cm], bh [Cout], styles [N, Cm]')
    w = torch.empty([n, cout, c], dtype=torch.float32, device=wm.device)
    b = torch.empty([n, cout], dtype=torch.float32, device=wm.device)
    with torch.cuda.device(wm.device):
        rc = lib.pg_conv1x1_fold_prep(nat.ptr(wm), nat.ptr(bm), nat.ptr(wh), nat.ptr(bh), nat.ptr(styles), nat.ptr(w), nat.ptr(b), n, cm, c, cout, nat.stream_of(wm))
    nat.check(rc, 'pg_conv1x1_fold_prep')
    return w, b


def conv1x1_fold_heads(x, x2, w, b, c_a, skip=None, clamp=None):
    lib = _init().lib
    x, x2, w, b, skip = _f32c(x, 'x'), _f32c(x2, 'x2'), _f32c(w, 'w'), _f32c(b, 'b'), _f32c(skip, 'skip')
    n, c1, h, wd = x.shape
    c2, cout, c_a = int(x2.shape[1]), int(w.shape[1]), int(c_a)
    n_skip = int(skip.shape[1]) if skip is not None else 0
    if (tuple(x2.shape) != (n, c2, h, wd) or tuple(w.shape) != (n, cout, c1 + c2) or tuple(b.shape) != (n, cout) or not 0 < c_a <= cout
            or (skip is not None and (tuple(skip.shape) != (n, n_skip, h, wd) or n_skip > cout))):
        raise nat.NativeOpError('conv1x1_fold_heads: x [N, C1, H, W], x2 [N, C2, H, W], w [N, Cout, C1 + C2], b [N, Cout], skip [N, <= Cout, H, W]')
    ya = torch.empty([n, c_a, h, wd], dtype=torch.float32, device=x.device)
    yb = torch.empty([n, cout - c_a, h, wd], dtype=torch.float32, device=x.device) if c_a < cout else None
    with torch.cuda.device(x.device):
        rc = lib.pg_conv1x1_fold_heads(nat.ptr(x), nat.ptr(x2), nat.ptr(w), nat.ptr(b), nat.ptr(skip), nat.ptr(ya), nat.ptr(yb), n, c1, c2, h * wd, cout, c_a,
                                       n_skip, float(clamp) if clamp is not None else -1.0, nat.stream_of(x))
    nat.check(rc, 'pg_conv1x1_fold_heads')
    return ya, yb


def conv3x3_fold_ok(xa, xb, skip=None):
    return (xa.dtype == torch.float32 and xa.is_cuda and xa.is_contiguous() and xb.dtype == torch.float32 and xb.is_cuda and xb.is_contiguous()
            and xa.shape == xb.shape
            and (skip is None or (skip.dtype == torch.float32 and skip.is_cuda and skip.is_contiguous() and skip.shape[0] == xa.shape[0] and skip.shape[2:] == xa.shape[2:])))


def conv3x3_fold_head(xa, xb, w, b, skip=None, clamp=None):
    lib = _init().lib
    xa, xb, w, b, skip = _f32c(xa, 'xa'), _f32c(xb, 'xb'), _f32c(w, 'w'), _f32c(b, 'b'), _f32c(skip, 'skip')
    n, c, h, wd = xa.shape
    cout = int(w.shape[1])
    if (tuple(xb.shape) != (n, c, h, wd) or tuple(w.shape) != (n, cout, 10 * c) or tuple(b.shape) != (n, cout)
            or (skip is not None and tuple(skip.shape) != (n, cout, h, wd))):
        raise nat.NativeOpError('conv3x3_fold_head: xa, xb [N, C, H, W], w [N, Cout, 10 C], b [N, Cout], skip [N, Cout, H, W]')
    y = torch.empty([n, cout, h, wd], dtype=torch.float32, device=xa.device)
    with torch.cuda.device(xa.device):
        rc = lib.pg_conv3x3_fold_head(nat.ptr(xa), nat.ptr(xb), nat.ptr(w), nat.ptr(b), nat.ptr(skip), nat.ptr(y), n, c, h, wd, cout,
                                      float(clamp) if clamp is not None else -1.0, nat.stream_of(xa))
    nat.check(rc, 'pg_conv3x3_fold_head')
    return y


def modconv_dcoefs(weight, styles, scale=1.0):
    lib = _init().lib
    weight, styles = _f32c(weight.detach(), 'weight'), _f32c(styles.detach(), 'styles')
    cout, cin, kh, kw = weight.shape
    n = styles.shape[0]
    assert styles.shape[1] == cin
    d = torch.empty([n, cout], dtype=torch.float32, device=weight.device)
    with torch.cuda.device(weight.device):
        st = lib.pg_modconv_dcoefs(nat.ptr(weight), nat.ptr(styles), nat.ptr(d), n, cout, cin, kh * kw, float(scale), nat.stream_of(weight))
    nat.check(st, 'pg_modconv_dcoefs')
    return d


def modconv_w2(weight, scale=1.0):
    lib = _init().lib
    weight = _f32c(weight.detach(), 'weight')
    cout, cin, kh, kw = weight.shape
    w2 = torch.empty([cout, cin], dtype=torch.float32, device=weight.device)
    with torch.cuda.device(weight.device):
        st = lib.pg_modconv_w2(nat.ptr(weight), nat.ptr(w2), cout, cin, kh * kw, float(scale), nat.stream_of(weight))
    nat.check(st, 'pg_modconv_w2')
    return w2


PREP_MAX_JOBS = 32


class PrepJobs(ctypes.Structure):
    _fields_ = [('w2', ctypes.c_void_p * PREP_MAX_JOBS), ('styles', ctypes.c_void_p * PREP_MAX_JOBS), ('out', ctypes.c_void_p * PREP_MAX_JOBS),
                ('s_norm', ctypes.c_void_p * PREP_MAX_JOBS), ('s16', ctypes.c_void_p * PREP_MAX_JOBS), ('cout', ctypes.c_int * PREP_MAX_JOBS),
                ('cin', ctypes.c_int * PREP_MAX_JOBS), ('flags', ctypes.c_int * PREP_MAX_JOBS), ('njobs', ctypes.c_int), ('half_dtype', ctypes.c_int)]


_prep_registry = {}


def modconv_prep_batched(jobs, half_dtype=None):
    lib = _init().lib
    assert 0 < len(jobs) <= PREP_MAX_JOBS
    table = PrepJobs()
    table.njobs, table.half_dtype = len(jobs), (nat.PG_DTYPE[half_dtype] if half_dtype is not None else 0)
    n = int(jobs[0][1].shape[0])
    keep = []
    for j, (w2, styles, cout, normalize, demodulate) in enumerate(jobs):
        assert styles.dtype == torch.float32 and styles.is_contiguous() and styles.shape[0] == n
        cin = int(styles.shape[1])
        out = torch.empty([n, cout], dtype=torch.float32, device=styles.device)
        s_norm = torch.empty_like(styles) if normalize else None
        s16 = torch.empty([n, cin], dtype=half_dtype, device=styles.device) if (normalize and half_dtype is not None) else None
        if demodulate:
            w2 = _f32c(w2, 'w2')
            assert tuple(w2.shape) == (cout, cin)
        table.w2[j] = w2.data_ptr() if demodulate else None
        table.styles[j], table.out[j] = styles.data_ptr(), out.data_ptr()
        table.s_norm[j] = s_norm.data_ptr() if s_norm is not None else None
        table.s16[j] = s16.data_ptr() if s16 is not None else None
        table.cout[j], table.cin[j], table.flags[j] = int(cout), cin, int(bool(normalize)) | (int(bool(demodulate)) << 1)
        keep.append((styles, w2))
        _prep_registry[styles.data_ptr()] = (bool(normalize), bool(demodulate), half_dtype if normalize else None, (out, s_norm, s16), styles)
    with torch.cuda.device(jobs[0][1].device):
        st = lib.pg_modconv_prep_batched(ctypes.byref(table), n, nat.stream_of(jobs[0][1]))
    nat.check(st, 'pg_modconv_prep_batched')


def modconv_prep_peek(styles):
    hit = _prep_registry.get(styles.data_ptr())
    if hit is None or hit[0] or not hit[1]:
        return None
    return hit[3][0]


def modconv_prep_clear():
    _prep_registry.clear()


def modconv_prep(w2, styles, cout, normalize=False, demodulate=True, half_dtype=None):
    hit = _prep_registry.pop(styles.data_ptr(), None) if _prep_registry else None
    if hit is not None and hit[0] == bool(normalize) and hit[1] == bool(demodulate) and hit[2] == (half_dtype if normalize else None) and hit[3][0].shape[1] == cout:
        return hit[3]
# ... 10 lines not shown
    with torch.cuda.device(styles.device):
        st = lib.pg_modconv_prep(nat.ptr(w2) if demodulate else None, nat.ptr(styles), nat.ptr(out), nat.ptr(s_norm) if s_norm is not None else None,
                                 nat.ptr(s16) if s16 is not None else None, code, n, cout, cin, int(bool(normalize)), int(bool(demodulate)), nat.stream_of(styles))
    nat.check(st, 'pg_modconv_prep')
    return out, s_norm, s16


def instance_norm_stats(x, eps=1e-5):
    lib = _init().lib
    x = _f32c(x, 'x')
    n, c, h, w = x.shape
    mean = torch.empty([n * c], dtype=torch.float32, device=x.device)
    rstd = torch.empty_like(mean)
    with torch.cuda.device(x.device):
        st = lib.pg_instance_norm_stats(nat.ptr(x), nat.ptr(mean), nat.ptr(rstd), n * c, h * w, float(eps), nat.stream_of(x))
    nat.check(st, 'pg_instance_norm_stats')
    return mean, rstd


def spade_norm(x, mean, rstd, gamma, beta):
    lib = _init().lib
    x, gamma, beta = _f32c(x, 'x'), _f32c(gamma, 'gamma'), _f32c(beta, 'beta')
    assert gamma.shape == x.shape and beta.shape == x.shape
    n, c, h, w = x.shape
    y = torch.empty_like(x)
    with torch.cuda.device(x.device):
        st = lib.pg_spade_norm(nat.ptr(x), nat.ptr(mean), nat.ptr(rstd), nat.ptr(gamma), nat.ptr(beta), nat.ptr(y), n * c, h * w, nat.stream_of(x))
    nat.check(st, 'pg_spade_norm')
    return y


def _gamma_beta_planes(gb, c):
    gb = _f32c(gb, 'gamma_beta')
    assert gb.shape[1] == 2 * c
    return gb, int(gb.stride(0)), int(gb.stride(1)) * c


def spade_train_forward(x, mean, rstd, gamma_beta):
    lib = _init().lib
    x = _f32c(x, 'x')
    n, c, h, w = x.shape
    gb, gs, off = _gamma_beta_planes(gamma_beta, c)
    y = torch.empty_like(x)
    with torch.cuda.device(x.device):
        st = lib.pg_spade_train_forward(nat.ptr(x), nat.ptr(mean), nat.ptr(rstd), gb.data_ptr(), gb.data_ptr() + 4 * off, nat.ptr(y), n, c, h * w, gs, gs, nat.stream_of(x))
    nat.check(st, 'pg_spade_train_forward')
    return y


def spade_train_backward(dy, x, mean, rstd, gamma_beta, need_dx=True, need_dgb=True):
    lib = _init().lib
    x, dy = _f32c(x, 'x'), _f32c(dy, 'dy')
    n, c, h, w = x.shape
    gb, gs, off = _gamma_beta_planes(gamma_beta, c)
    sums = torch.empty([2 * n * c], dtype=torch.float32, device=x.device)
    dx = torch.empty_like(x) if need_dx else None
    dgb = torch.empty_like(gb) if need_dgb else None
    with torch.cuda.device(x.device):
        st = lib.pg_spade_train_backward(nat.ptr(dy), nat.ptr(x), nat.ptr(mean), nat.ptr(rstd), gb.data_ptr(), nat.ptr(sums), nat.ptr(dx),
                                         dgb.data_ptr() if need_dgb else None, dgb.data_ptr() + 4 * off if need_dgb else None,
                                         n, c, h * w, gs, gs, gs, nat.stream_of(x))
    nat.check(st, 'pg_spade_train_backward')
    return dx, dgb


def spade_feat_assemble(feat_upper, feat_lower, mask_upper, mask_lower, denorm_mask_upper, denorm_mask_lower):
    lib = _init().lib
    fu, fl = _f32c(feat_upper, 'feat_upper'), _f32c(feat_lower, 'feat_lower')
    masks = [_f32c(m, 'mask') for m in (mask_upper, mask_lower, denorm_mask_upper, denorm_mask_lower)]
    n, c, h, w = fu.shape
    if fl.shape != fu.shape or any(tuple(m.shape) != (n, 1, 2 * h, 2 * w) for m in masks):
        raise nat.NativeOpError('spade_feat_assemble: feat [N,C,H,W] x2 and masks [N,1,2H,2W] x4 expected')
    mu, ml, du, dl = masks
    sums = torch.empty([2, n * c], dtype=torch.float32, device=fu.device)
    counts = torch.empty([2, n], dtype=torch.float32, device=fu.device)
    out = torch.empty_like(fu)
    with torch.cuda.device(fu.device):
        st = nat.stream_of(fu)
        nat.check(lib.pg_spade_masked_sums(nat.ptr(fu), nat.ptr(mu), nat.ptr(du), nat.ptr(sums[0]), nat.ptr(counts[0]), n, c, h, w, st), 'pg_spade_masked_sums')
        nat.check(lib.pg_spade_masked_sums(nat.ptr(fl), nat.ptr(ml), nat.ptr(dl), nat.ptr(sums[1]), nat.ptr(counts[1]), n, c, h, w, st), 'pg_spade_masked_sums')
        nat.check(lib.pg_spade_feat_assemble(nat.ptr(fu), nat.ptr(fl), nat.ptr(mu), nat.ptr(ml), nat.ptr(du), nat.ptr(dl), nat.ptr(sums[0]), nat.ptr(sums[1]),
                                             nat.ptr(counts[0]), nat.ptr(counts[1]), nat.ptr(out), n, c, h, w, st), 'pg_spade_feat_assemble')
    return out
```

pasta-gan-plusplus_amd/training/networks.py:

```python

import os
from typing import NamedTuple, Optional
import numpy as np
import torch
import torch.nn as nn

from torch_utils import misc
from torch_utils.ops import _native as nat
from torch_utils.ops import bias_act
from torch_utils.ops import conv2d_gradfix
from torch_utils.ops import conv2d_mfma
from torch_utils.ops import conv2d_mfma16
from torch_utils.ops import conv2d_resample
from torch_utils.ops import fma
from torch_utils.ops import upfirdn2d

SQRT_HALF = float(np.sqrt(0.5))


def _needs_graph(*tensors):
    return torch.is_grad_enabled() and any(t is not None and t.requires_grad for t in tensors)


def _fast_ok(x, *others):
# ... 878 lines not shown
        self.skip = Spade_Conv2dLayer(in_channels, out_channels, kernel_size=1, **kw)
        self.spade_skip = Spade_Norm_Block(spade_channels, in_channels)
        self.spade0 = Spade_Norm_Block(spade_channels, in_channels)
        self.spade1 = Spade_Norm_Block(spade_channels, out_channels)

    def forward(self, x, denorm_feat, _defer_tail=False):
        if (_fast_ok(x, denorm_feat, self.conv.weight, self.conv0.weight) or _fast16_ok(x, denorm_feat, self.conv.weight, self.conv0.weight)) and all(l.bias is None and l.activation in conv2d_mfma.FUSED_ACTS for l in (self.skip, self.conv0, self.conv1)):
            assert self.spade_skip.param_free_norm.eps == self.spade0.param_free_norm.eps
            x, stats = self.conv(x, no_act=True, stats_eps=self.spade0.param_free_norm.eps)
            s = self.spade_skip(x, denorm_feat, post=self.skip.pre_activation(SQRT_HALF), stats=stats)
            defer = _defer_tail and s.dtype == torch.float32
            y = None if defer else self.skip(s, no_act=True)
            x, stats1 = self.conv0(self.spade0(x, denorm_feat, post=self.conv0.pre_activation(), stats=stats), no_act=True, stats_eps=self.spade1.param_free_norm.eps)
            h = self.spade1(x, denorm_feat, post=self.conv1.pre_activation(SQRT_HALF), stats=stats1)
            return (h, s) if defer else self.conv1(h, no_act=True, residual=y)
        x = self.conv(x, no_act=True)
        y = self.skip(self.spade_skip(x, denorm_feat), gain=SQRT_HALF)
        x = self.conv0(self.spade0(x, denorm_feat))
        return self.conv1(self.spade1(x, denorm_feat), gain=SQRT_HALF, residual=y)

    def tail(self, h, s):
        return self.conv1(h, no_act=True, residual=self.skip(s, no_act=True))


class SynthesisLayer(nn.Module):

    def __init__(self, in_channels, out_channels, w_dim, resolution, kernel_size=3, up=1, use_noise=True, activation='lrelu',
                 resample_filter=[1, 3, 3, 1], conv_clamp=None, channels_last=False):
        super().__init__()
        self.resolution, self.up, self.use_noise, self.activation, self.conv_clamp = resolution, up, use_noise, activation, conv_clamp
        self.register_buffer('resample_filter', upfirdn2d.setup_filter(resample_filter))
        self.padding = kernel_size // 2
        self.act_gain = bias_act.activation_funcs[activation].def_gain
        self.affine = FullyConnectedLayer(w_dim, in_channels, bias_init=1)
        memory_format = torch.channels_last if channels_last else torch.contiguous_format
        self.weight = nn.Parameter(torch.randn([out_channels, in_channels, kernel_size, kernel_size]).to(memory_format=memory_format))
        if use_noise:
            self.register_buffer('noise_const', torch.randn([resolution, resolution]))
            self.noise_strength = nn.Parameter(torch.zeros([]))
        self.bias = nn.Parameter(torch.zeros([out_channels]))
        self._cache = _PackCache()

    def forward(self, x, w, noise_mode='random', fused_modconv=True, gain=1, styles=None):
        assert noise_mode in ['random', 'const', 'none']
        in_res = self.resolution // self.up
        misc.assert_shape(x, [None, self.weight.shape[1], in_res, in_res])
        if styles is None:
            styles = self.affine(w)
        noise = None
        if self.use_noise and noise_mode == 'random':
            noise = torch.randn([x.shape[0], 1, self.resolution, self.resolution], device=x.device) * self.noise_strength
        if self.use_noise and noise_mode == 'const':
            if torch.is_grad_enabled() and self.noise_strength.requires_grad:
                noise = self.noise_const * self.noise_strength
            else:
                noise = self._cache.get(('noise',), [self.noise_const, self.noise_strength], lambda: (self.noise_const * self.noise_strength).detach())
        act_gain = self.act_gain * gain
        act_clamp = self.conv_clamp * gain if self.conv_clamp is not None else None
        fusable = (_fast_ok(x, self.weight, self.bias, styles, noise) or _fast16_ok(x, self.weight, self.bias, styles, noise)
                   or (self.up == 1 and _train_fused_ok(x, self.weight, styles, noise, self.padding))
                   or (self.up == 2 and _train_fused_up2_ok(x, self.weight, styles, noise, self.padding, self.resample_filter)))
        if fusable and self.activation in conv2d_mfma.FUSED_ACTS:
            ep = dict(bias=self.bias, act=self.activation, alpha=bias_act.activation_funcs[self.activation].def_alpha, gain=act_gain, clamp=act_clamp)
            return modulated_conv2d(x=x, weight=self.weight, styles=styles, noise=noise, up=self.up, padding=self.padding,
                                    resample_filter=self.resample_filter, flip_weight=(self.up == 1), fused_modconv=fused_modconv,
                                    _cache=self._cache, _epilogue=ep)
        x = modulated_conv2d(x=x, weight=self.weight, styles=styles, noise=noise, up=self.up, padding=self.padding,
                             resample_filter=self.resample_filter, flip_weight=(self.up == 1), fused_modconv=fused_modconv)
        return bias_act.bias_act(x, self.bias.to(x.dtype), act=self.activation, gain=act_gain, clamp=act_clamp)




def _is_1331(f):
    hit = getattr(f, '_pg_is_1331', None)
    if hit is None or hit[0] != f._version:
        ref = torch.tensor([1.0, 3.0, 3.0, 1.0])
        ref = torch.outer(ref, ref) / 64.0
        hit = (f._version, bool(f.ndim == 2 and tuple(f.shape) == (4, 4) and torch.equal(f.detach().float().cpu(), ref)))
        f._pg_is_1331 = hit
    return hit[1]


class _ToRGBBase(nn.Module):
    PARSING_CHANNELS = 7

    def __init__(self, in_channels, out_channels, w_dim, kernel_size=1, conv_clamp=None, channels_last=False, is_last=False, is_style=False):
        super().__init__()
        self.conv_clamp = conv_clamp
        self.affine = FullyConnectedLayer(w_dim, in_channels, bias_init=1)
        memory_format = torch.channels_last if channels_last else torch.contiguous_format
        self.weight = nn.Parameter(torch.randn([out_channels, in_channels, kernel_size, kernel_size]).to(memory_format=memory_format))
        self.bias = nn.Parameter(torch.zeros([out_channels]))
        self.weight_gain = 1 / np.sqrt(in_channels * (kernel_size ** 2))
        self.is_last, self.is_style = is_last, is_style
        if self.is_last and self.is_style:
            self.m_weight1 = nn.Parameter(torch.randn([self.PARSING_CHANNELS, in_channels, kernel_size, kernel_size]).to(memory_format=memory_format))
            self.m_bias1 = nn.Parameter(torch.zeros([self.PARSING_CHANNELS]))
        self._cache, self._cache_p = _PackCache(), _PackCache()

    def forward(self, x, w, fused_modconv=True, skip_img=None, styles=None, skip_up2_filter=None):
        if styles is None:
            styles = self.affine(w) * self.weight_gain
        if _fast16_ok(x, self.weight, self.bias, styles, skip_img) and self.weight.shape[2:] == (1, 1):
            up2 = False
            if skip_up2_filter is not None and skip_img is not None:
                if _is_1331(skip_up2_filter) and x.shape[2] % 2 == 0 and x.shape[3] % 2 == 0 and skip_img.dtype == torch.float32 and os.environ.get('PG_HEAD16_UP2', '1') != '0':
                    up2 = True
                else:
                    skip_img = upfirdn2d.upsample2d(skip_img, skip_up2_filter)
            pred_parsing = None
            if self.is_last and self.is_style:
                pred_parsing = conv2d_mfma16.conv1x1_small(x, self.m_weight1, styles, self.m_bias1, clamp=self.conv_clamp)
            return conv2d_mfma16.conv1x1_small(x, self.weight, styles, self.bias, skip=skip_img, clamp=self.conv_clamp, skip_up2=up2), pred_parsing
        if skip_up2_filter is not None and skip_img is not None:
            skip_img = upfirdn2d.upsample2d(skip_img, skip_up2_filter)
        fast = _fast_ok(x, self.weight, self.bias, styles, skip_img)
        if fast and conv2d_mfma.conv1x1_small_ok(x, self.weight, skip_img) and os.environ.get('PG_HEAD_STREAM', '1') != '0':
            pred_parsing = None
            if self.is_last and self.is_style:
                pred_parsing = conv2d_mfma.conv1x1_small(x, self.m_weight1, styles, self.m_bias1, clamp=self.conv_clamp)
            return conv2d_mfma.conv1x1_small(x, self.weight, styles, self.bias, skip=skip_img, clamp=self.conv_clamp), pred_parsing
        pred_parsing = None
        if self.is_last and self.is_style:
            if fast:
                pred_parsing = modulated_conv2d(x=x, weight=self.m_weight1, styles=styles, demodulate=False, fused_modconv=fused_modconv,
                                                _cache=self._cache_p, _epilogue=dict(bias=self.m_bias1, clamp=self.conv_clamp))
            elif _train_fused_ok(x, self.m_weight1, styles, None, 0):
                pred_parsing = modulated_conv2d(x=x, weight=self.m_weight1, styles=styles, demodulate=False, fused_modconv=fused_modconv,
                                                _epilogue=dict(bias=self.m_bias1, clamp=self.conv_clamp))
            else:
                pred_parsing = modulated_conv2d(x=x, weight=self.m_weight1, styles=styles, demodulate=False, fused_modconv=fused_modconv)
                pred_parsing = bias_act.bias_act(pred_parsing, self.m_bias1.to(x.dtype), clamp=self.conv_clamp)
        if fast:
            y = modulated_conv2d(x=x, weight=self.weight, styles=styles, demodulate=False, fused_modconv=fused_modconv,
                                 _cache=self._cache, _epilogue=dict(bias=self.bias, clamp=self.conv_clamp, residual=skip_img))
            return y, pred_parsing
        if _train_fused_ok(x, self.weight, styles, None, 0):
            y = modulated_conv2d(x=x, weight=self.weight, styles=styles, demodulate=False, fused_modconv=fused_modconv,
                                 _epilogue=dict(bias=self.bias, clamp=self.conv_clamp))
        else:
            y = modulated_conv2d(x=x, weight=self.weight, styles=styles, demodulate=False, fused_modconv=fused_modconv)
            y = bias_act.bias_act(y, self.bias.to(x.dtype), clamp=self.conv_clamp)
        if skip_img is not None:
            y = skip_img + y
        return y, pred_parsing


class ToRGBLayerFull_v1_v5(_ToRGBBase):
    PARSING_CHANNELS = 7


class ToRGBLayerFull_v1_v4(_ToRGBBase):
    PARSING_CHANNELS = 6


class _SynthesisBlockBase(nn.Module):
    TORGB = ToRGBLayerFull_v1_v5
    TEXTURE = False

    def __init__(self, in_channels, out_channels, w_dim, resolution, img_channels, is_last, is_style=False, architecture='skip',
                 resample_filter=[1, 3, 3, 1], conv_clamp=None, use_fp16=False, fp16_channels_last=False, **layer_kwargs):
        assert architecture in ['orig', 'skip', 'resnet']
        super().__init__()
        self.in_channels, self.w_dim, self.resolution, self.img_channels = in_channels, w_dim, resolution, img_channels
        self.is_last, self.architecture, self.use_fp16 = is_last, architecture, use_fp16
        self.channels_last = (use_fp16 and fp16_channels_last)
        self.half_dtype = None
        self.register_buffer('resample_filter', upfirdn2d.setup_filter(resample_filter))
        first = in_channels == 0
        layer = dict(w_dim=w_dim, resolution=resolution, conv_clamp=conv_clamp, channels_last=self.channels_last, **layer_kwargs)
        if first:
            self.const = nn.Parameter(torch.randn([out_channels, resolution, resolution]))
        else:
            self.conv0 = SynthesisLayer(in_channels, out_channels, up=2, resample_filter=resample_filter, **layer)
        self.conv1 = SynthesisLayer(out_channels, out_channels, **layer)
        self.num_conv = 1 if first else 2
        self.has_torgb = is_last or architecture == 'skip'
        self.num_torgb = int(self.has_torgb)
        if self.has_torgb:
            self.torgb = self.TORGB(out_channels, img_channels, w_dim=w_dim, conv_clamp=conv_clamp, channels_last=self.channels_last,
                                    is_last=is_last, is_style=is_style)
        if not first and architecture == 'resnet':
            self.skip = Conv2dLayer(in_channels, out_channels, kernel_size=1, bias=False, up=2, resample_filter=resample_filter, channels_last=self.channels_last)
        if resolution > 32:
            self.merge_conv = Conv2dLayer(out_channels + 64, out_channels, kernel_size=1, resample_filter=resample_filter, channels_last=self.channels_last)
        if self.TEXTURE:
            self.spade_b512 = Spade_ResBlockV4_512(out_channels, out_channels, spade_channels=1)
        self._fold_cache = _PackCache()

    def affine_layers(self):
        convs = [self.conv1] if self.in_channels == 0 else [self.conv0, self.conv1]
        return [(m, i, 1.0) for i, m in enumerate(convs)] + ([(self.torgb, self.num_conv, self.torgb.weight_gain)] if self.has_torgb else [])

    def _heads_folded(self, x, feat, w, styles, img):
        mc, tr = getattr(self, 'merge_conv', None), getattr(self, 'torgb', None)
        if mc is None or tr is None or self.TEXTURE or self.architecture != 'skip' or os.environ.get('PG_HEAD_FOLD', '1') == '0' or os.environ.get('PG_HEAD_STREAM', '1') == '0':
            return None
        if (mc.conv_clamp is not None or mc.activation != 'linear' or mc.up != 1 or mc.down != 1 or tuple(mc.weight.shape[2:]) != (1, 1)
                or tuple(tr.weight.shape[2:]) != (1, 1) or int(mc.weight.shape[1]) != int(x.shape[1]) + int(feat.shape[1])):
            return None
        parsing = tr.is_last and tr.is_style
        params = [mc.weight, tr.weight, tr.bias] + ([mc.bias] if mc.bias is not None else []) + ([tr.m_weight1, tr.m_bias1] if parsing else [])
        if not (_fast_ok(x, feat, styles, img, tr.affine.weight, tr.affine.bias, *params) and conv2d_mfma.conv1x1_fold_ok(x, feat, img)):
            return None

        def build():
            cm = int(mc.weight.shape[0])
            heads = [(tr.weight, tr.bias)] + ([(tr.m_weight1, tr.m_bias1)] if parsing else [])
            return ((mc.weight.detach().float().reshape(cm, -1) * mc.weight_gain * mc.act_gain).contiguous(),
                    (mc.bias.detach().float() * mc.act_gain).contiguous() if mc.bias is not None else None,
                    torch.cat([hw.detach().float().reshape(hw.shape[0], cm) for hw, _ in heads]).contiguous(),
                    torch.cat([hb.detach().float() for _, hb in heads]).contiguous())
        wm, bm, wh, bh = self._fold_cache.get(('fold',), params, build)
        if styles is None:
            styles = tr.affine(w) * tr.weight_gain
        try:
            wn, bn = conv2d_mfma.conv1x1_fold_prep(wm, bm, wh, bh, styles)
            return conv2d_mfma.conv1x1_fold_heads(x, feat, wn, bn, int(tr.weight.shape[0]), skip=img, clamp=tr.conv_clamp)
        except nat.NativeNotCovered:
            return None

    def _merge_heads(self, x, feat, w, styles, img, fused_modconv, feat_unused=False):
        if feat_unused:
            heads = self._heads_folded(x, feat, w, styles, img)
            if heads is not None:
                return (None,) + tuple(heads)
        x = self.merge_conv(x, x2=feat)
        rgb, pred_parsing = self.torgb(x, w, fused_modconv=fused_modconv, skip_img=img, styles=styles)
        return x, rgb, pred_parsing

    def _tail_fold_ok(self):
        sb, tr = getattr(self, 'spade_b512', None), getattr(self, 'torgb', None)
        if sb is None or tr is None or not self.TEXTURE or torch.is_grad_enabled() or os.environ.get('PG_TEX_FOLD', '1') == '0':
            return False
        c1, sk = sb.conv1, sb.skip
        cm = int(tr.weight.shape[1])
        return (all(l.bias is None and l.up == 1 and l.down == 1 and int(l.weight.shape[0]) == cm for l in (c1, sk))
                and tuple(c1.weight.shape[2:]) == (3, 3) and c1.padding == 1 and tuple(sk.weight.shape[2:]) == (1, 1) and sk.padding == 0
                and c1.weight.shape[1] == sk.weight.shape[1] and tuple(tr.weight.shape[2:]) == (1, 1) and not (tr.is_last and tr.is_style))

    def _tail_folded(self, h, s, w, styles, img):
        sb, tr = self.spade_b512, self.torgb
        c1, sk = sb.conv1, sb.skip
        params = [c1.weight, sk.weight, tr.weight, tr.bias]
        if not (_fast_ok(h, s, styles, img, tr.affine.weight, tr.affine.bias, *params) and conv2d_mfma.conv3x3_fold_ok(h, s, img)):
            return None

        def build():
            cm = int(c1.weight.shape[0])
            return (torch.cat([(c1.weight.detach().float() * c1.weight_gain).reshape(cm, -1), (sk.weight.detach().float() * sk.weight_gain).reshape(cm, -1)], dim=1).contiguous(),
                    tr.weight.detach().float().reshape(tr.weight.shape[0], cm).contiguous(), tr.bias.detach().float().contiguous())
        wm, wh, bh = self._fold_cache.get(('tail',), params, build)
        if styles is None:
            styles = tr.affine(w) * tr.weight_gain
        try:
            wn, bn = conv2d_mfma.conv1x1_fold_prep(wm, None, wh, bh, styles)
            return conv2d_mfma.conv3x3_fold_head(h, s, wn, bn, skip=img, clamp=tr.conv_clamp)
        except nat.NativeNotCovered:
            return None

    def _spade_heads(self, x, parsing, w, styles, img, fused_modconv, feat_unused=False):
        x = self.spade_b512(x, parsing, _defer_tail=feat_unused and self._tail_fold_ok())
        if isinstance(x, tuple):
            rgb = self._tail_folded(*x, w, styles, img)
            if rgb is not None:
                return None, rgb, None
            x = self.spade_b512.tail(*x)
        rgb, pred_parsing = self.torgb(x, w, fused_modconv=fused_modconv, skip_img=img, styles=styles)
        return x, rgb, pred_parsing

    def _forward(self, x, img, ws, pose_feature, cat_feat, parsing, force_fp32, fused_modconv, styles=None, _feat_unused=False, **layer_kwargs):
        misc.assert_shape(ws, [None, self.num_conv + self.num_torgb, self.w_dim])
        half = (self.use_fp16 or self.half_dtype is not None) and not force_fp32
        fmt = dict(dtype=(self.half_dtype or torch.float16) if half else torch.float32,
                   memory_format=torch.channels_last if ((self.channels_last or self.half_dtype is not None) and not force_fp32) else torch.contiguous_format)
        if fused_modconv is None:
            fused_modconv = (not self.training) and (not half or int(ws.shape[0]) == 1)
        style = lambda i: ws[:, i]
        st = styles if styles is not None else [None] * (self.num_conv + self.num_torgb)
        conv = lambda layer, t, i, **kw: layer(t, style(i), fused_modconv=fused_modconv, styles=st[i], **kw, **layer_kwargs)

        if self.in_channels == 0:
            x = conv(self.conv1, pose_feature.to(**fmt), 0)
        else:
            misc.assert_shape(x, [None, self.in_channels, self.resolution // 2, self.resolution // 2])
            x = x.to(**fmt)
            if self.architecture == 'resnet':
                shortcut = self.skip(x, gain=SQRT_HALF)
                x = conv(self.conv1, conv(self.conv0, x, 0), 1, gain=SQRT_HALF)
                x = shortcut.add_(x)
            else:
                x = conv(self.conv1, conv(self.conv0, x, 0), 1)
                if self.resolution > 32:
                    feat = cat_feat[str(self.resolution)].to(**fmt)
                    if _feat_unused and self.has_torgb and not self.TEXTURE and not half:
                        if img is not None:
                            misc.assert_shape(img, [None, self.img_channels, self.resolution // 2, self.resolution // 2])
                            img = upfirdn2d.upsample2d(img, self.resample_filter)
                        x, rgb, pred_parsing = self._merge_heads(x, feat, style(self.num_conv), st[self.num_conv], img, fused_modconv, feat_unused=True)
                        return x, rgb.to(dtype=torch.float32, memory_format=torch.contiguous_format), pred_parsing
                    x = self.merge_conv(x, x2=feat)
                if self.TEXTURE:
                    if _feat_unused and self.has_torgb and not half:
                        if img is not None:
                            misc.assert_shape(img, [None, self.img_channels, self.resolution // 2, self.resolution // 2])
                            img = upfirdn2d.upsample2d(img, self.resample_filter)
                        x, rgb, pred_parsing = self._spade_heads(x, parsing, style(self.num_conv), st[self.num_conv], img, fused_modconv, feat_unused=True)
                        return x, rgb.to(dtype=torch.float32, memory_format=torch.contiguous_format), pred_parsing
                    x = self.spade_b512(x, parsing)

        if img is not None:
            misc.assert_shape(img, [None, self.img_channels, self.resolution // 2, self.resolution // 2])
            img = upfirdn2d.upsample2d(img, self.resample_filter)
        pred_parsing = None
        if self.has_torgb:
            rgb, pred_parsing = self.torgb(x, style(self.num_conv), fused_modconv=fused_modconv, skip_img=img, styles=st[self.num_conv])
            img = rgb.to(dtype=torch.float32, memory_format=torch.contiguous_format)
        return x, img, pred_parsing


class SynthesisBlockFull_v1_v6(_SynthesisBlockBase):
    TORGB = ToRGBLayerFull_v1_v5

    def forward(self, x, img, ws, pose_feature, cat_feat, force_fp32=False, fused_modconv=None, styles=None, _feat_unused=False, **layer_kwargs):
        return self._forward(x, img, ws, pose_feature, cat_feat, None, force_fp32, fused_modconv, styles=styles, _feat_unused=_feat_unused, **layer_kwargs)


class SynthesisBlockFull_v1_v4(_SynthesisBlockBase):
    TORGB = ToRGBLayerFull_v1_v4
    TEXTURE = True

    def forward(self, x, img, ws, pose_feature, cat_feat, parsing, force_fp32=False, fused_modconv=None, styles=None, _feat_unused=False, **layer_kwargs):
        return self._forward(x, img, ws, pose_feature, cat_feat, parsing, force_fp32, fused_modconv, styles=styles, _feat_unused=_feat_unused, **layer_kwargs)


def _half_nearest(t):
    return t[:, :, ::2, ::2]


def _batched_affine(owner, entries, ws, num_ws, w_dim):
    n = ws.shape[0]
    params = [t for _, m, _, _ in entries for t in (m.affine.weight, m.affine.bias)]

    def build():
        wt = torch.cat([m.affine.weight.detach().float() * (m.affine.weight_gain * g) for _, m, _, g in entries]).t().contiguous()
        b = torch.cat([m.affine.bias.detach().float() * (m.affine.bias_gain * g) for _, m, _, g in entries]).contiguous()
        return wt, b
    if not hasattr(owner, '_affine_cache'):
        owner._affine_cache, owner._gather = _PackCache(), {}
    wt, b = owner._affine_cache.get(('all',), params, build)
    total = wt.shape[1]
    key = (n, ws.device)
    if key not in owner._gather:
        idx, col = [], 0
        rows = torch.arange(n, dtype=torch.int64)[:, None] * num_ws
        for _, m, wi, _ in entries:
            c = m.affine.weight.shape[0]
            idx.append(((rows + wi) * total + col + torch.arange(c, dtype=torch.int64)[None, :]).reshape(-1))
            col += c
        owner._gather[key] = torch.cat(idx).to(ws.device)
    flat = torch.addmm(b, ws.reshape(n * num_ws, w_dim), wt).reshape(-1).index_select(0, owner._gather[key])
    out, off = {}, 0
    for k, m, _, _ in entries:
        c = m.affine.weight.shape[0]
        out.setdefault(k, []).append(flat[off:off + n * c].view(n, c))
        off += n * c
    return out


class SynthesisNetworkFull_v18(nn.Module):

    def __init__(self, w_dim, img_resolution, img_channels, channel_base=32768, channel_max=512, num_fp16_res=0, **block_kwargs):
        assert img_resolution >= 8 and img_resolution & (img_resolution - 1) == 0
        super().__init__()
        self.w_dim, self.img_resolution, self.img_channels = w_dim, img_resolution, img_channels
        self.img_resolution_log2 = int(np.log2(img_resolution))
        self.block_resolutions = [1 << e for e in range(3, self.img_resolution_log2 + 1)]
        width = lambda res: min(channel_base // res, channel_max)
        common = dict(w_dim=w_dim, img_channels=img_channels, use_fp16=False, **block_kwargs)
        self.num_ws = 0
        for res in self.block_resolutions:
            last = res == img_resolution
            block = SynthesisBlockFull_v1_v6(width(res // 2) if res > 8 else 0, width(res), resolution=res, is_last=last, is_style=True, **common)
            setattr(self, f'b{res}', block)
            self.num_ws += block.num_conv + (block.num_torgb if last else 0)
        mid, top = self.block_resolutions[-2], self.block_resolutions[-1]
        self.spade_b256_1 = Spade_ResBlockV4_512(width(mid), width(mid), spade_channels=128)
        self.spade_b256_2 = Spade_ResBlockV4_512(width(mid), width(mid), spade_channels=128)
        self.texture_b512 = SynthesisBlockFull_v1_v4(width(mid), width(top), resolution=top, is_last=True, is_style=False, **common)
        ngf = 64
        self.spade_encoder = nn.Sequential(
            Conv2dLayer(3, ngf, kernel_size=7, activation='relu'),
            ResBlock(ngf, ngf, kernel_size=4, activation='relu'),
            ResBlock(ngf, ngf * 2, kernel_size=4, activation='relu', down=2),
        )
        self.half_dtype, self.half_from_res = None, 64

    def set_half(self, dtype, from_res=64):
        if dtype is not None and dtype not in conv2d_mfma16.DTYPES:
            raise ValueError(f'set_half: dtype must be None, torch.bfloat16 or torch.float16, not {dtype!r}')
        if dtype is not None:
            narrow = [res for res in self.block_resolutions if res >= int(from_res) and any(int(c) % 16 for c in (getattr(self, f'b{res}').in_channels, getattr(self, f'b{res}').conv1.weight.shape[0]))]
            if narrow:
                raise ValueError(f'set_half: the 16-bit kernels need channel counts that are multiples of 16; the blocks at {narrow} have narrower layers')
        self.half_dtype, self.half_from_res = dtype, int(from_res)
        for res in self.block_resolutions:
            getattr(self, f'b{res}').half_dtype = dtype if res >= int(from_res) else None
        self.texture_b512.half_dtype = dtype if self.block_resolutions[-1] >= int(from_res) else None
        return self

    def _half_on(self, block, ws):
        return block.half_dtype is not None and ws.is_cuda and not torch.is_grad_enabled() and not self.training

    def get_spade_feat(self, mask_512, denorm_mask, denorm_input):
        region = mask_512 > 0.9
        region_256 = _half_nearest(region)
        covered = region_256 & (_half_nearest(denorm_mask) > 0.9)
        hole = (region_256 & ~covered).to(denorm_input.dtype)
        feat = self.spade_encoder(torch.where(region, denorm_input, -1.0))
        covered = covered.to(feat.dtype)
        count = covered.sum(dim=(2, 3), keepdim=True)
        count = torch.where(count > 10, count, 256.0 * 256.0)
        mean = (feat * covered).sum(dim=(2, 3), keepdim=True) / count
        return feat * (1 - hole) + mean * hole

    def _block_styles(self, ws):
        misc.assert_shape(ws, [None, self.num_ws, self.w_dim])
        ws = ws.to(torch.float32)
        out, start = [], 0
        for res in self.block_resolutions:
            block = getattr(self, f'b{res}')
            out.append(ws[:, start:start + block.num_conv + block.num_torgb])
            start += block.num_conv
        return out

    def forward(self, ws, pose_feat, cat_feat, denorm_upper_input, denorm_lower_input, denorm_upper_mask,
                denorm_lower_mask, gt_parsing, **block_kwargs):
        styles = self._block_styles(ws)
        pre = None
        if ws.is_cuda and not torch.is_grad_enabled() and os.environ.get('PG_AFFINE_BATCHED', '1') != '0':
            entries, start = [], 0
            for res in self.block_resolutions:
                block = getattr(self, f'b{res}')
                entries += [(res, m, start + i, g) for m, i, g in block.affine_layers()]
                last_start, start = start, start + block.num_conv
            entries += [('texture', m, last_start + i, g) for m, i, g in self.texture_b512.affine_layers()]
            pre = _batched_affine(self, entries, ws.to(torch.float32), self.num_ws, self.w_dim)
            if os.environ.get('PG_PREP_BATCHED', '1') != '0':
                jobs, seen = [], {}
                for key, m, _, _ in entries:
                    j = seen.get(key, 0)
                    seen[key] = j + 1
                    if isinstance(m, SynthesisLayer) and getattr(m, '_cache', None) is not None:
                        w2 = m._cache.get(('w2',), [m.weight], lambda m=m: conv2d_mfma.modconv_w2(m.weight))
                        jobs.append((w2, pre[key][j], int(m.weight.shape[0]), False, True))
                if 0 < len(jobs) <= conv2d_mfma.PREP_MAX_JOBS:
                    conv2d_mfma.modconv_prep_batched(jobs)
        try:
            return self._forward_body(ws, styles, pre, pose_feat, cat_feat, denorm_upper_input, denorm_lower_input, denorm_upper_mask, denorm_lower_mask, gt_parsing, block_kwargs)
        finally:
            if pre is not None:
                conv2d_mfma.modconv_prep_clear()

    def _forward_body(self, ws, styles, pre, pose_feat, cat_feat, denorm_upper_input, denorm_lower_input, denorm_upper_mask, denorm_lower_mask, gt_parsing, block_kwargs):
        x = img = pred_parsing = None
        kept = {}
        for res, w in zip(self.block_resolutions, styles):
            block = getattr(self, f'b{res}')
            x, img, pred_parsing = block(x, img, w, pose_feat, cat_feat, force_fp32=not self._half_on(block, ws), styles=pre[res] if pre is not None else None,
                                         _feat_unused=(res == self.block_resolutions[-1]), **block_kwargs)
            kept[res] = (x, img)
        x_256, img_256 = kept[self.block_resolutions[-2]]

        if gt_parsing is not None:
            parsing_index = gt_parsing
        else:
            parsing_index = pred_parsing.detach().argmax(dim=1, keepdim=True).float()
        upper_mask = ((parsing_index == 1) | (parsing_index == 4)).float()
        lower_mask = ((parsing_index == 2) | (parsing_index == 3)).float()

        if _fast_ok(x_256, denorm_upper_input, denorm_lower_input, denorm_upper_mask, denorm_lower_mask) and denorm_upper_mask.dtype == torch.float32:
            feat_u = self.spade_encoder(torch.where(upper_mask > 0.9, denorm_upper_input, -1.0))
            feat_l = self.spade_encoder(torch.where(lower_mask > 0.9, denorm_lower_input, -1.0))
            spade_feat = conv2d_mfma.spade_feat_assemble(feat_u, feat_l, upper_mask, lower_mask, denorm_upper_mask, denorm_lower_mask)
        else:
            spade_feat = (self.get_spade_feat(upper_mask.detach(), denorm_upper_mask, denorm_upper_input) * (_half_nearest(upper_mask) > 0.9)
                          + self.get_spade_feat(lower_mask.detach(), denorm_lower_mask, denorm_lower_input) * (_half_nearest(lower_mask) > 0.9))

        if x_256.dtype != torch.float32:
            spade_feat = spade_feat.to(dtype=x_256.dtype, memory_format=torch.channels_last)
        x_spade = self.spade_b256_2(self.spade_b256_1(x_256, spade_feat), spade_feat)
        _, finetune_img, _ = self.texture_b512(x_spade, img_256, styles[-1], pose_feat, cat_feat, parsing_index, force_fp32=not self._half_on(self.texture_b512, ws),
                                               styles=pre['texture'] if pre is not None else None, _feat_unused=True, **block_kwargs)
        return img, finetune_img, pred_parsing


class SynthesisStackBlock(nn.Module):

    def __init__(self, in_channels, out_channels, w_dim, resolution, img_channels, resample_filter=[1, 3, 3, 1], conv_clamp=None,
                 half_dtype=None, **layer_kwargs):
        super().__init__()
        self.in_channels, self.w_dim, self.resolution, self.img_channels, self.half_dtype = in_channels, w_dim, resolution, img_channels, half_dtype
        self.register_buffer('resample_filter', upfirdn2d.setup_filter(resample_filter))
        layer = dict(w_dim=w_dim, resolution=resolution, conv_clamp=conv_clamp, **layer_kwargs)
        if in_channels == 0:
            self.const = nn.Parameter(torch.randn([out_channels, resolution, resolution]))
        else:
            self.conv0 = SynthesisLayer(in_channels, out_channels, up=2, resample_filter=resample_filter, **layer)
        self.conv1 = SynthesisLayer(out_channels, out_channels, **layer)
        self.torgb = ToRGBLayerFull_v1_v5(out_channels, img_channels, w_dim=w_dim, conv_clamp=conv_clamp)
        self.num_conv = 1 if in_channels == 0 else 2
        self.num_torgb = 1

    def affine_layers(self):
        convs = [self.conv1] if self.in_channels == 0 else [self.conv0, self.conv1]
        return [(m, i, 1.0) for i, m in enumerate(convs)] + [(self.torgb, self.num_conv, self.torgb.weight_gain)]

    def forward(self, x, img, ws, force_fp32=False, styles=None, **layer_kwargs):
        misc.assert_shape(ws, [None, self.num_conv + self.num_torgb, self.w_dim])
        half = self.half_dtype is not None and not force_fp32
        fmt = dict(dtype=self.half_dtype if half else torch.float32, memory_format=torch.channels_last if half else torch.contiguous_format)
        st = list(styles) if styles is not None else [None] * (self.num_conv + self.num_torgb)
        if self.in_channels == 0:
            x = self.const.to(fmt['dtype'])[None].expand(ws.shape[0], -1, -1, -1).contiguous(memory_format=fmt['memory_format'])
            x = self.conv1(x, ws[:, 0], styles=st[0], **layer_kwargs)
        else:
            x = self.conv1(self.conv0(x.to(**fmt), ws[:, 0], styles=st[0], **layer_kwargs), ws[:, 1], styles=st[1], **layer_kwargs)
        rgb, _ = self.torgb(x, ws[:, self.num_conv], skip_img=img, styles=st[self.num_conv], skip_up2_filter=self.resample_filter if img is not None else None)
        return x, rgb.to(dtype=torch.float32, memory_format=torch.contiguous_format)


class SynthesisStack(nn.Module):

    def __init__(self, w_dim, img_resolution, img_channels=3, channel_base=32768, channel_max=512, num_fp16_res=0, half_dtype=torch.float16,
                 conv_clamp=None, **block_kwargs):
        assert img_resolution >= 8 and img_resolution & (img_resolution - 1) == 0
        super().__init__()
        self.w_dim, self.img_resolution, self.img_channels = w_dim, img_resolution, img_channels
        log2 = int(np.log2(img_resolution))
        self.block_resolutions = [1 << e for e in range(3, log2 + 1)]
        width = lambda res: min(channel_base // res, channel_max)
        half_from = max(1 << (log2 + 1 - num_fp16_res), 8) if num_fp16_res > 0 else (img_resolution * 2)
        self.num_ws = 0
        for res in self.block_resolutions:
            block = SynthesisStackBlock(width(res // 2) if res > 8 else 0, width(res), w_dim=w_dim, resolution=res, img_channels=img_channels,
                                        conv_clamp=conv_clamp, half_dtype=half_dtype if res >= half_from else None, **block_kwargs)
            setattr(self, f'b{res}', block)
            self.num_ws += block.num_conv + (block.num_torgb if res == img_resolution else 0)

    def all_styles(self, ws):
        entries, start = [], 0
        for res in self.block_resolutions:
            block = getattr(self, f'b{res}')
            entries += [(res, m, start + i, g) for m, i, g in block.affine_layers()]
            start += block.num_conv
        return _batched_affine(self, entries, ws, self.num_ws, self.w_dim)

    def forward(self, ws, **block_kwargs):
        misc.assert_shape(ws, [None, self.num_ws, self.w_dim])
        ws = ws.to(torch.float32)
        x = img = None
        start = 0
        styles = self.all_styles(ws) if (ws.is_cuda and not torch.is_grad_enabled() and os.environ.get('PG_AFFINE_BATCHED', '1') != '0') else None
        try:
            if styles is not None and os.environ.get('PG_PREP_BATCHED', '1') != '0':
                self._prepare_all(styles, bool(block_kwargs.get('force_fp32', False)))
# ... 291 lines not shown
```

Before: 292.7.

## Fuse skip-image 2x upsample into head convs and fuse parsing-to-mask encoder prep

```diff
diff --git a/include/pasta_gan_ops.h b/include/pasta_gan_ops.h
--- a/include/pasta_gan_ops.h
+++ b/include/pasta_gan_ops.h
@@ -7,7 +7,7 @@
 extern "C" {
 #endif
 
-#define PG_ABI_VERSION 20
+#define PG_ABI_VERSION 21
 
 enum pg_dtype { PG_F32 = 0, PG_F16 = 1, PG_BF16 = 2, PG_F64 = 3 };
 
@@ -159,15 +159,17 @@
                            const pg_conv2d_fusion* fusion, void* stream);
 
 int pg_conv1x1_small(const float* x, const float* w, const float* styles, const float* bias, const float* skip, float* y,
-                     int N, int Cin, int64_t HW, int Cout, float scale, float clamp, void* stream);
-
+                     int N, int Cin, int64_t HW, int Cout, float scale, float clamp, int skip_up2_width, void* stream);
+
+#define PG_FOLD_PREP_LANES 0
+#define PG_FOLD_PREP_SERIAL 1
 int pg_conv1x1_fold_prep(const float* wm, const float* bm, const float* wh, const float* bh, const float* styles, float* w_out, float* b_out,
-                         int N, int Cm, int C, int Cout, void* stream);
+                         int N, int Cm, int C, int Cout, int form, void* stream);
 int pg_conv1x1_fold_heads(const float* x, const float* x2, const float* w, const float* bias, const float* skip, float* y_a, float* y_b,
-                          int N, int C1, int C2, int64_t HW, int Cout, int c_a, int n_skip, float clamp, void* stream);
+                          int N, int C1, int C2, int64_t HW, int Cout, int c_a, int n_skip, float clamp, int skip_up2_width, void* stream);
 
 int pg_conv3x3_fold_head(const float* xa, const float* xb, const float* w, const float* bias, const float* skip, float* y,
-                         int N, int C, int H, int W, int Cout, float clamp, void* stream);
+                         int N, int C, int H, int W, int Cout, float clamp, int skip_up2, void* stream);
 
 int pg_conv3x3_cin1(const float* x, const float* w, float* y, int N, int H, int W, int Cout, float scale, int act, void* stream);
 
@@ -192,6 +194,9 @@
                            const float* denorm_mask_upper, const float* denorm_mask_lower,
                            const float* sums_upper, const float* sums_lower, const float* counts_upper, const float* counts_lower,
                            float* out, int N, int C, int H, int W, void* stream);
+int pg_parsing_to_encoder_inputs(const float* pred_parsing, const float* parsing_index_in, const float* denorm_upper, const float* denorm_lower,
+                                 float* parsing_index_out, float* upper_mask, float* lower_mask, float* upper_input, float* lower_input,
+                                 int N, int C, int Ci, int H, int W, void* stream);
 int pg_conv2d_abi_version(void);
 int pg_conv2d_reserve_cus(int n);
 
diff --git a/pasta-gan-plusplus_amd/csrc/conv1x1_fold.hip b/pasta-gan-plusplus_amd/csrc/conv1x1_fold.hip
--- a/pasta-gan-plusplus_amd/csrc/conv1x1_fold.hip
+++ b/pasta-gan-plusplus_amd/csrc/conv1x1_fold.hip
@@ -1,4 +1,5 @@
 #include "pg_common.h"
+#include "skip_up2.h"
 
 #ifndef PG_FOLD_MIN_WAVES
 #define PG_FOLD_MIN_WAVES 1
@@ -29,10 +30,36 @@
     }
 }
 
+__global__ __launch_bounds__(256) void conv1x1_fold_prep_lanes_kernel(const float* __restrict__ wm, const float* __restrict__ bm, const float* __restrict__ wh,
+                                                                      const float* __restrict__ bh, const float* __restrict__ styles, float* __restrict__ w_out,
+                                                                      float* __restrict__ b_out, int Cm, int C, int Cout) {
+    __shared__ double part[4][64];
+    const int o = blockIdx.y, n = blockIdx.z;
+    const int lane = threadIdx.x & 63, wave = threadIdx.x >> 6;
+    const int c = blockIdx.x * 64 + lane;
+    const float* who = wh + (int64_t)o * Cm;
+    const float* sn = styles ? styles + (int64_t)n * Cm : nullptr;
+    const int ks = (Cm + 3) / 4, k0 = wave * ks, k1 = k0 + ks < Cm ? k0 + ks : Cm;
+    const float* col = c < C ? wm + c : bm;
+    const int64_t step = c < C ? C : 1;
+    double acc = 0.0;
+    if (c <= C && col) {
+#pragma unroll 8
+        for (int k = k0; k < k1; k++) acc += (double)who[k] * (double)(sn ? sn[k] : 1.f) * (double)col[(int64_t)k * step];
+    }
+    part[wave][lane] = acc;
+    __syncthreads();
+    if (wave == 0 && c <= C) {
+        const double sum = ((part[0][lane] + part[1][lane]) + part[2][lane]) + part[3][lane];
+        if (c < C) w_out[((int64_t)n * Cout + o) * C + c] = (float)sum;
+        else b_out[(int64_t)n * Cout + o] = (float)(sum + (double)(bh ? bh[o] : 0.f));
+    }
+}
+
 template <int CP>
 __global__ __launch_bounds__(256, PG_FOLD_MIN_WAVES) void conv1x1_fold_heads_kernel(const float* __restrict__ x, const float* __restrict__ x2, const float* __restrict__ w,
                                                                  const float* __restrict__ bias, const float* __restrict__ skip, float* __restrict__ ya,
-                                                                 float* __restrict__ yb, int C1, int C2, int64_t HW4, int Cout, int c_a, int n_skip, float clamp) {
+                                                                 float* __restrict__ yb, int C1, int C2, int64_t HW4, int Cout, int c_a, int n_skip, float clamp, int up_w4) {
     extern __shared__ __attribute__((aligned(16))) float wl[];
     const int n = blockIdx.y, C = C1 + C2;
     const float* wn = w + (int64_t)n * Cout * C;
@@ -70,13 +97,17 @@
         };
         walk(xa, C1, wl);
         walk(xb, C2, wl + C1 * CP);
+        const int oy = up_w4 ? (int)((unsigned)p / (unsigned)up_w4) : 0, ox = up_w4 ? 4 * ((int)p - oy * up_w4) : 0;
 #pragma unroll
         for (int o = 0; o < CP; o++) {
             if (o < Cout) {
                 f32x4s r = acc[o] + bias[(int64_t)n * Cout + o];
 #pragma unroll
                 for (int e = 0; e < 4; e++) r[e] = fminf(fmaxf(r[e], -cl), cl);
-                if (o < n_skip) r += ((const f32x4s*)skip)[((int64_t)n * n_skip + o) * HW4 + p];
+                if (o < n_skip) {
+                    if (up_w4) r += pg::skip_up2_quad(skip + ((int64_t)n * n_skip + o) * HW4, (int)(HW4 / up_w4) >> 1, 2 * up_w4, oy, ox);
+                    else r += ((const f32x4s*)skip)[((int64_t)n * n_skip + o) * HW4 + p];
+                }
                 if (o < c_a) ((f32x4s*)ya)[((int64_t)n * c_a + o) * HW4 + p] = r;
                 else ((f32x4s*)yb)[((int64_t)n * (Cout - c_a) + (o - c_a)) * HW4 + p] = r;
             }
@@ -86,30 +117,38 @@
 }
 
 PG_EXPORT int pg_conv1x1_fold_prep(const float* wm, const float* bm, const float* wh, const float* bh, const float* styles, float* w_out, float* b_out,
-                                   int N, int Cm, int C, int Cout, void* stream) {
-    if (!wm || !wh || !w_out || !b_out || N <= 0 || Cm <= 0 || C <= 0 || Cout <= 0) return PG_ERR_INVALID_ARG;
-    if (N > 65535) return PG_ERR_TOO_LARGE;
+                                   int N, int Cm, int C, int Cout, int form, void* stream) {
+    if (!wm || !wh || !w_out || !b_out || N <= 0 || Cm <= 0 || C <= 0 || Cout <= 0 || (form != PG_FOLD_PREP_LANES && form != PG_FOLD_PREP_SERIAL)) return PG_ERR_INVALID_ARG;
+    if (N > 65535 || Cout > 65535) return PG_ERR_TOO_LARGE;
+    if (form == PG_FOLD_PREP_LANES) {
+        hipLaunchKernelGGL(conv1x1_fold_prep_lanes_kernel, dim3((unsigned)(C / 64 + 1), (unsigned)Cout, (unsigned)N), dim3(256), 0, (hipStream_t)stream, wm, bm, wh, bh, styles,
+                           w_out, b_out, Cm, C, Cout);
+        return pg::launch_status();
+    }
     hipLaunchKernelGGL(conv1x1_fold_prep_kernel, dim3((unsigned)Cout, (unsigned)N), dim3(256), 0, (hipStream_t)stream, wm, bm, wh, bh, styles, w_out, b_out, Cm, C, Cout);
     return pg::launch_status();
 }
 
 PG_EXPORT int pg_conv1x1_fold_heads(const float* x, const float* x2, const float* w, const float* bias, const float* skip, float* y_a, float* y_b,
-                                    int N, int C1, int C2, int64_t HW, int Cout, int c_a, int n_skip, float clamp, void* stream) {
+                                    int N, int C1, int C2, int64_t HW, int Cout, int c_a, int n_skip, float clamp, int skip_up2_width, void* stream) {
     if (!x || !w || !bias || !y_a || N <= 0 || C1 <= 0 || C2 < 0 || HW <= 0 || Cout <= 0 || c_a <= 0 || c_a > Cout || n_skip < 0 || n_skip > Cout) return PG_ERR_INVALID_ARG;
+    if (skip_up2_width < 0 || (skip_up2_width && (n_skip == 0 || skip_up2_width % 2 || HW % skip_up2_width || (HW / skip_up2_width) % 2))) return PG_ERR_INVALID_ARG;
     if ((C2 > 0 && !x2) || (c_a < Cout && !y_b) || (n_skip > 0 && !skip)) return PG_ERR_INVALID_ARG;
     const int CP = (Cout + 3) / 4 * 4;
     const size_t lds = (size_t)(C1 + C2) * CP * sizeof(float);
     if (Cout > 16 || HW % 4 != 0 || !pg::aligned16(x) || (C2 > 0 && !pg::aligned16(x2)) || !pg::aligned16(y_a) || (c_a < Cout && !pg::aligned16(y_b)) ||
         (n_skip > 0 && !pg::aligned16(skip)) || lds > 64 * 1024)
         return PG_ERR_UNSUPPORTED;
+    if (skip_up2_width && (skip_up2_width % 4 || HW / 4 > 0x7fffffffLL)) return PG_ERR_UNSUPPORTED;
     if (N > 65535) return PG_ERR_TOO_LARGE;
     const int64_t HW4 = HW / 4;
+    const int up_w4 = skip_up2_width / 4;
     int64_t bx = (HW4 + 255) / 256;
     const int64_t cap = (int64_t)pg::num_cu() * 8 / N + 1;
     if (bx > cap) bx = cap;
     const dim3 grid((unsigned)bx, (unsigned)N);
     hipStream_t s = (hipStream_t)stream;
-#define PG_FOLD(P) case P: hipLaunchKernelGGL((conv1x1_fold_heads_kernel<P>), grid, dim3(256), lds, s, x, x2, w, bias, skip, y_a, y_b, C1, C2, HW4, Cout, c_a, n_skip, clamp); break;
+#define PG_FOLD(P) case P: hipLaunchKernelGGL((conv1x1_fold_heads_kernel<P>), grid, dim3(256), lds, s, x, x2, w, bias, skip, y_a, y_b, C1, C2, HW4, Cout, c_a, n_skip, clamp, up_w4); break;
     switch (CP) { PG_FOLD(4) PG_FOLD(8) PG_FOLD(12) PG_FOLD(16) }
 #undef PG_FOLD
     return pg::launch_status();
diff --git a/pasta-gan-plusplus_amd/csrc/conv2d.hip b/pasta-gan-plusplus_amd/csrc/conv2d.hip
--- a/pasta-gan-plusplus_amd/csrc/conv2d.hip
+++ b/pasta-gan-plusplus_amd/csrc/conv2d.hip
@@ -1,5 +1,6 @@
 #include "conv2d_kernel.h"
 #include "bf16x3.h"
+#include "skip_up2.h"
 
 namespace {
 
@@ -478,6 +479,53 @@
     }
 }
 
+template <int V>
+__global__ __launch_bounds__(256) void parsing_to_encoder_inputs_kernel(const float* __restrict__ logits, const float* __restrict__ index_in,
+                                                                        const float* __restrict__ du, const float* __restrict__ dl,
+                                                                        float* __restrict__ index_out, float* __restrict__ mu, float* __restrict__ ml,
+                                                                        float* __restrict__ eu, float* __restrict__ el, int C, int Ci, int64_t HWv, int64_t total) {
+    typedef vec_t<float, V> VT;
+    for (int64_t i = (int64_t)blockIdx.x * 256 + threadIdx.x; i < total; i += (int64_t)gridDim.x * 256) {
+        const int64_t n = i / HWv, q = i - n * HWv;
+        VT idx;
+        if (logits) {
+            const VT* lp = (const VT*)logits + n * C * HWv + q;
+            VT best = lp[0];
+#pragma unroll
+            for (int k = 0; k < V; k++) idx.v[k] = 0.f;
+#pragma unroll 8
+            for (int c = 1; c < C; c++) {
+                const VT v = lp[c * HWv];
+#pragma unroll
+                for (int k = 0; k < V; k++)
+                    if (best.v[k] == best.v[k] && (v.v[k] > best.v[k] || v.v[k] != v.v[k])) { best.v[k] = v.v[k]; idx.v[k] = (float)c; }
+            }
+            ((VT*)index_out)[i] = idx;
+        } else {
+            idx = ((const VT*)index_in)[i];
+        }
+        VT m_u, m_l;
+#pragma unroll
+        for (int k = 0; k < V; k++) {
+            m_u.v[k] = (idx.v[k] == 1.f || idx.v[k] == 4.f) ? 1.f : 0.f;
+            m_l.v[k] = (idx.v[k] == 2.f || idx.v[k] == 3.f) ? 1.f : 0.f;
+        }
+        ((VT*)mu)[i] = m_u;
+        ((VT*)ml)[i] = m_l;
+        for (int c = 0; c < Ci; c++) {
+            const int64_t at = (n * Ci + c) * HWv + q;
+            VT a = ((const VT*)du)[at], b = ((const VT*)dl)[at];
+#pragma unroll
+            for (int k = 0; k < V; k++) {
+                a.v[k] = m_u.v[k] != 0.f ? a.v[k] : -1.f;
+                b.v[k] = m_l.v[k] != 0.f ? b.v[k] : -1.f;
+            }
+            ((VT*)eu)[at] = a;
+            ((VT*)el)[at] = b;
+        }
+    }
+}
+
 __global__ __launch_bounds__(256) void splitk_finish_kernel(const float* __restrict__ ws, float* __restrict__ y, int ksplit, int64_t slice,
                                                             int N, int Cout, int OH, int OW, int64_t ys0, int64_t ys1, int64_t ys2, int64_t ys3,
                                                             int osy, int osx, int ooy, int oox, pg_conv2d_fusion f) {
@@ -687,7 +735,7 @@
 template <int COUT>
 __global__ __launch_bounds__(256) void conv1x1_small_f32_kernel(const float* __restrict__ x, const float* __restrict__ w, const float* __restrict__ styles,
                                                                 const float* __restrict__ bias, const float* __restrict__ skip, float* __restrict__ y,
-                                                                int Cin, int64_t HW4, float scale, float clamp) {
+                                                                int Cin, int64_t HW4, float scale, float clamp, int up_w4) {
     extern __shared__ __attribute__((aligned(16))) float wl[];
     const int n = blockIdx.y;
     for (int e = threadIdx.x; e < 8 * Cin; e += 256) {
@@ -716,13 +764,17 @@
             for (int u = 0; u < 8; u++) mac(v[u], c0 + u);
         }
         for (; c0 < Cin; c0++) mac(xn[(int64_t)c0 * HW4 + p], c0);
+        const int oy = up_w4 ? (int)((unsigned)p / (unsigned)up_w4) : 0, ox = up_w4 ? 4 * ((int)p - oy * up_w4) : 0;
 #pragma unroll
         for (int o = 0; o < COUT; o++) {
             f32x4s r = acc[o] + (bias ? bias[o] : 0.f);
 #pragma unroll
             for (int e = 0; e < 4; e++) r[e] = fminf(fmaxf(r[e], -cl), cl);
             const int64_t off = ((int64_t)n * COUT + o) * HW4 + p;
-            if (skip) r += ((const f32x4s*)skip)[off];
+            if (skip) {
+                if (up_w4) r += pg::skip_up2_quad(skip + ((int64_t)n * COUT + o) * HW4, (int)(HW4 / up_w4) >> 1, 2 * up_w4, oy, ox);
+                else r += ((const f32x4s*)skip)[off];
+            }
             ((f32x4s*)y)[off] = r;
         }
     }
@@ -732,7 +784,7 @@
 template <int COUT, int QB>
 __global__ __launch_bounds__(256) void conv1x1_small_f32_split_kernel(const float* __restrict__ x, const float* __restrict__ w, const float* __restrict__ styles,
                                                                       const float* __restrict__ bias, const float* __restrict__ skip, float* __restrict__ y,
-                                                                      int Cin, int64_t HW4, float scale, float clamp) {
+                                                                      int Cin, int64_t HW4, float scale, float clamp, int up_w4) {
     constexpr int CS = 256 / QB;
     static_assert(QB * COUT <= 256, "one output thread per (quad, channel)");
     __shared__ f32x4s part[CS][COUT][QB];
@@ -777,7 +829,14 @@
         for (int e = 0; e < 4; e++) r[e] = fminf(fmaxf(r[e], -cl), cl);
         if (po < HW4) {
             const int64_t off = ((int64_t)n * COUT + o) * HW4 + po;
-            if (skip) r += ((const f32x4s*)skip)[off];
+            if (skip) {
+                if (up_w4) {
+                    const int oy = (int)((unsigned)po / (unsigned)up_w4), ox = 4 * ((int)po - oy * up_w4);
+                    r += pg::skip_up2_quad(skip + ((int64_t)n * COUT + o) * HW4, (int)(HW4 / up_w4) >> 1, 2 * up_w4, oy, ox);
+                } else {
+                    r += ((const f32x4s*)skip)[off];
+                }
+            }
             ((f32x4s*)y)[off] = r;
         }
     }
@@ -829,11 +888,14 @@
 }
 
 PG_EXPORT int pg_conv1x1_small(const float* x, const float* w, const float* styles, const float* bias, const float* skip, float* y,
-                               int N, int Cin, int64_t HW, int Cout, float scale, float clamp, void* stream) {
+                               int N, int Cin, int64_t HW, int Cout, float scale, float clamp, int skip_up2_width, void* stream) {
     if (!x || !w || !y || N <= 0 || Cin <= 0 || HW <= 0 || Cout <= 0) return PG_ERR_INVALID_ARG;
+    if (skip_up2_width < 0 || (skip_up2_width && (!skip || skip_up2_width % 2 || HW % skip_up2_width || (HW / skip_up2_width) % 2))) return PG_ERR_INVALID_ARG;
     if (Cout > 8 || HW % 4 != 0 || !pg::aligned16(x) || !pg::aligned16(y) || (skip && !pg::aligned16(skip)) || (size_t)Cin * 32 > 64 * 1024) return PG_ERR_UNSUPPORTED;
+    if (skip_up2_width && (skip_up2_width % 4 || HW / 4 > 0x7fffffffLL)) return PG_ERR_UNSUPPORTED;
     if (N > 65535) return PG_ERR_TOO_LARGE;
     const int64_t HW4 = HW / 4;
+    const int up_w4 = skip_up2_width / 4;
     hipStream_t s = (hipStream_t)stream;
     static const bool split_on = [] { const char* e = getenv("PG_HEAD32_SPLIT"); return !e || atoi(e) != 0; }();
     if (split_on && (int64_t)N * ((HW4 + 255) / 256) < (int64_t)pg::num_cu() / 2 && Cin >= 64) {
@@ -841,8 +903,8 @@
         if ((int64_t)N * ((HW4 + 15) / 16) >= 2 * (int64_t)pg::num_cu()) qb = 16;
         const dim3 g2((unsigned)((HW4 + qb - 1) / qb), (unsigned)N);
 #define PG_SPLIT(C) case C: \
-        if (qb == 16) hipLaunchKernelGGL((conv1x1_small_f32_split_kernel<C, 16>), g2, dim3(256), 0, s, x, w, styles, bias, skip, y, Cin, HW4, scale, clamp); \
-        else hipLaunchKernelGGL((conv1x1_small_f32_split_kernel<C, 4>), g2, dim3(256), 0, s, x, w, styles, bias, skip, y, Cin, HW4, scale, clamp); \
+        if (qb == 16) hipLaunchKernelGGL((conv1x1_small_f32_split_kernel<C, 16>), g2, dim3(256), 0, s, x, w, styles, bias, skip, y, Cin, HW4, scale, clamp, up_w4); \
+        else hipLaunchKernelGGL((conv1x1_small_f32_split_kernel<C, 4>), g2, dim3(256), 0, s, x, w, styles, bias, skip, y, Cin, HW4, scale, clamp, up_w4); \
         break;
         switch (Cout) { PG_SPLIT(1) PG_SPLIT(2) PG_SPLIT(3) PG_SPLIT(4) PG_SPLIT(5) PG_SPLIT(6) PG_SPLIT(7) PG_SPLIT(8) }
 #undef PG_SPLIT
@@ -853,7 +915,7 @@
     if (bx > cap) bx = cap;
     const dim3 grid((unsigned)bx, (unsigned)N);
     const size_t lds = (size_t)Cin * 32;
-#define PG_SMALL(C) case C: hipLaunchKernelGGL((conv1x1_small_f32_kernel<C>), grid, dim3(256), lds, s, x, w, styles, bias, skip, y, Cin, HW4, scale, clamp); break;
+#define PG_SMALL(C) case C: hipLaunchKernelGGL((conv1x1_small_f32_kernel<C>), grid, dim3(256), lds, s, x, w, styles, bias, skip, y, Cin, HW4, scale, clamp, up_w4); break;
     switch (Cout) { PG_SMALL(1) PG_SMALL(2) PG_SMALL(3) PG_SMALL(4) PG_SMALL(5) PG_SMALL(6) PG_SMALL(7) PG_SMALL(8) }
 #undef PG_SMALL
     return pg::launch_status();
@@ -1049,3 +1111,24 @@
                        sums_upper, sums_lower, counts_upper, counts_lower, out, C, H, W, vec);
     return pg::launch_status();
 }
+
+PG_EXPORT int pg_parsing_to_encoder_inputs(const float* pred_parsing, const float* parsing_index_in, const float* denorm_upper, const float* denorm_lower,
+                                           float* parsing_index_out, float* upper_mask, float* lower_mask, float* upper_input, float* lower_input,
+                                           int N, int C, int Ci, int H, int W, void* stream) {
+    if (!denorm_upper || !denorm_lower || !upper_mask || !lower_mask || !upper_input || !lower_input || N <= 0 || Ci <= 0 || H <= 0 || W <= 0) return PG_ERR_INVALID_ARG;
+    if ((pred_parsing != nullptr) == (parsing_index_in != nullptr) || (pred_parsing && (!parsing_index_out || C <= 0))) return PG_ERR_INVALID_ARG;
+    if (pred_parsing && C > 16) return PG_ERR_UNSUPPORTED;
+    const int64_t HW = (int64_t)H * W;
+    const bool vec = W % 4 == 0 && pg::aligned16(pred_parsing) && pg::aligned16(parsing_index_in) && pg::aligned16(denorm_upper) && pg::aligned16(denorm_lower) &&
+                     pg::aligned16(parsing_index_out) && pg::aligned16(upper_mask) && pg::aligned16(lower_mask) && pg::aligned16(upper_input) && pg::aligned16(lower_input);
+    const int64_t HWv = vec ? HW / 4 : HW, total = (int64_t)N * HWv;
+    int64_t blocks = (total + 255) / 256;
+    if (blocks > pg::max_stream_blocks()) blocks = pg::max_stream_blocks();
+    if (vec)
+        hipLaunchKernelGGL(parsing_to_encoder_inputs_kernel<4>, dim3((unsigned)blocks), dim3(256), 0, (hipStream_t)stream, pred_parsing, parsing_index_in, denorm_upper, denorm_lower,
+                           parsing_index_out, upper_mask, lower_mask, upper_input, lower_input, C, Ci, HWv, total);
+    else
+        hipLaunchKernelGGL(parsing_to_encoder_inputs_kernel<1>, dim3((unsigned)blocks), dim3(256), 0, (hipStream_t)stream, pred_parsing, parsing_index_in, denorm_upper, denorm_lower,
+                           parsing_index_out, upper_mask, lower_mask, upper_input, lower_input, C, Ci, HWv, total);
+    return pg::launch_status();
+}
diff --git a/pasta-gan-plusplus_amd/csrc/conv3x3_fold.hip b/pasta-gan-plusplus_amd/csrc/conv3x3_fold.hip
--- a/pasta-gan-plusplus_amd/csrc/conv3x3_fold.hip
+++ b/pasta-gan-plusplus_amd/csrc/conv3x3_fold.hip
@@ -1,4 +1,5 @@
 #include "pg_common.h"
+#include "skip_up2.h"
 
 namespace {
 typedef float f32x4s __attribute__((ext_vector_type(4)));
@@ -23,7 +24,7 @@
 template <int CO>
 __global__ __launch_bounds__(256, 2) void conv3x3_fold_head_kernel(const float* __restrict__ xa, const float* __restrict__ xb, const float* __restrict__ w,
                                                                    const float* __restrict__ bias, const float* __restrict__ skip, float* __restrict__ y,
-                                                                   int C, int H, int W, float clamp) {
+                                                                   int C, int H, int W, float clamp, int up2) {
     const int n = blockIdx.z;
     const int wave = __builtin_amdgcn_readfirstlane((int)threadIdx.x >> 6), lane = (int)threadIdx.x & 63;
     const int r0 = ((int)blockIdx.y * F3_WAVES + wave) * F3_ROWS;
@@ -127,7 +128,10 @@
                 f32x4s r;
 #pragma unroll
                 for (int q = 0; q < 4; q++) r[q] = fminf(fmaxf(acc[o][t][q] + bo, -cl), cl);
-                if (skip) r += *(const f32x4s*)(skip + at);
+                if (skip) {
+                    if (up2) r += pg::skip_up2_quad(skip + ((int64_t)n * CO + o) * (H >> 1) * (W >> 1), H >> 1, W >> 1, r0 + t, col);
+                    else r += *(const f32x4s*)(skip + at);
+                }
                 *(f32x4s*)(y + at) = r;
             }
         }
@@ -136,15 +140,16 @@
 }
 
 PG_EXPORT int pg_conv3x3_fold_head(const float* xa, const float* xb, const float* w, const float* bias, const float* skip, float* y,
-                                   int N, int C, int H, int W, int Cout, float clamp, void* stream) {
+                                   int N, int C, int H, int W, int Cout, float clamp, int skip_up2, void* stream) {
     if (!xa || !xb || !w || !bias || !y || N <= 0 || C <= 0 || H <= 0 || W <= 0 || Cout <= 0) return PG_ERR_INVALID_ARG;
+    if (skip_up2 && (!skip || H % 2 || W % 2)) return PG_ERR_INVALID_ARG;
     if (Cout > 4 || W % 4 != 0 || !pg::aligned16(xa) || !pg::aligned16(xb) || !pg::aligned16(y) || (skip && !pg::aligned16(skip))) return PG_ERR_UNSUPPORTED;
     if ((int64_t)H * W * 4 > (int64_t)1 << 29 || (int64_t)C * 10 * Cout > (int64_t)1 << 24) return PG_ERR_UNSUPPORTED;
     const int64_t by = ((int64_t)H + F3_WAVES * F3_ROWS - 1) / (F3_WAVES * F3_ROWS);
     if (N > 65535 || by > 65535) return PG_ERR_TOO_LARGE;
     const dim3 grid((unsigned)((W + F3_COLS - 1) / F3_COLS), (unsigned)by, (unsigned)N);
     hipStream_t s = (hipStream_t)stream;
-#define PG_FOLD3(P) case P: hipLaunchKernelGGL((conv3x3_fold_head_kernel<P>), grid, dim3(64 * F3_WAVES), 0, s, xa, xb, w, bias, skip, y, C, H, W, clamp); break;
+#define PG_FOLD3(P) case P: hipLaunchKernelGGL((conv3x3_fold_head_kernel<P>), grid, dim3(64 * F3_WAVES), 0, s, xa, xb, w, bias, skip, y, C, H, W, clamp, skip_up2 ? 1 : 0); break;
     switch (Cout) { PG_FOLD3(1) PG_FOLD3(2) PG_FOLD3(3) PG_FOLD3(4) }
 #undef PG_FOLD3
     return pg::launch_status();
diff --git a/pasta-gan-plusplus_amd/csrc/skip_up2.h b/pasta-gan-plusplus_amd/csrc/skip_up2.h
--- /dev/null
+++ b/pasta-gan-plusplus_amd/csrc/skip_up2.h
@@ -0,0 +1,41 @@
+#pragma once
+#include "pg_common.h"
+
+namespace pg {
+
+typedef float up2_f32x4 __attribute__((ext_vector_type(4)));
+typedef float up2_f32x2 __attribute__((ext_vector_type(2)));
+
+__device__ __forceinline__ void skip_up2_row(const float* __restrict__ sp, int hh, int hw, int yy, int m, float s[4]) {
+    const bool rok = yy >= 0 && yy < hh;
+    const float* row = sp + (int64_t)(rok ? yy : 0) * hw;
+    const up2_f32x2 mid = *(const up2_f32x2*)(row + m);
+    const float l = row[m > 0 ? m - 1 : 0], r = row[m + 2 < hw ? m + 2 : m];
+    s[0] = (rok && m > 0) ? l : 0.f;
+    s[1] = rok ? mid[0] : 0.f;
+    s[2] = rok ? mid[1] : 0.f;
+    s[3] = (rok && m + 2 < hw) ? r : 0.f;
+}
+
+__device__ __forceinline__ up2_f32x4 skip_up2_quad(const float* __restrict__ sp, int hh, int hw, int oy, int ox) {
+    const int m = ox >> 1, py = oy & 1;
+    const int y0 = py ? (oy >> 1) : (oy >> 1) - 1;
+    float s0[4], s1[4];
+    skip_up2_row(sp, hh, hw, y0, m, s0);
+    skip_up2_row(sp, hh, hw, y0 + 1, m, s1);
+    const float a0 = py ? 3.f : 1.f, a1 = py ? 1.f : 3.f;
+    up2_f32x4 out;
+#pragma unroll
+    for (int e = 0; e < 4; e++) {
+        const int px = e & 1, i = (e >> 1) + px;
+        const float b0 = px ? 3.f : 1.f, b1 = px ? 1.f : 3.f;
+        float acc = __builtin_fmaf(s0[i], a0 * b0 * 0.015625f, 0.f);
+        acc = __builtin_fmaf(s0[i + 1], a0 * b1 * 0.015625f, acc);
+        acc = __builtin_fmaf(s1[i], a1 * b0 * 0.015625f, acc);
+        acc = __builtin_fmaf(s1[i + 1], a1 * b1 * 0.015625f, acc);
+        out[e] = acc * 4.f;
+    }
+    return out;
+}
+
+}
diff --git a/pasta-gan-plusplus_amd/torch_utils/custom_ops.py b/pasta-gan-plusplus_amd/torch_utils/custom_ops.py
--- a/pasta-gan-plusplus_amd/torch_utils/custom_ops.py
+++ b/pasta-gan-plusplus_amd/torch_utils/custom_ops.py
@@ -35,7 +35,7 @@
                       'conv2d16_inst_k1x2.hip', 'conv2d16_inst_k3s2.hip', 'conv2d16_inst_up2f.hip', 'conv1x1_head16.hip', 'spade16.hip', 'conv1x1_fold.hip', 'conv3x3_fold.hip', 'optim.hip'],
 }
 
-ABI_VERSION = 20
+ABI_VERSION = 21
 
 _cached_plugins = dict()
 
diff --git a/pasta-gan-plusplus_amd/torch_utils/ops/conv2d_mfma.py b/pasta-gan-plusplus_amd/torch_utils/ops/conv2d_mfma.py
--- a/pasta-gan-plusplus_amd/torch_utils/ops/conv2d_mfma.py
+++ b/pasta-gan-plusplus_amd/torch_utils/ops/conv2d_mfma.py
@@ -108,6 +108,8 @@
         lib.pg_spade_masked_sums.argtypes = [vp, vp, vp, vp, vp, i, i, i, i, vp]
         lib.pg_spade_feat_assemble.restype = i
         lib.pg_spade_feat_assemble.argtypes = [vp] * 11 + [i, i, i, i, vp]
+        lib.pg_parsing_to_encoder_inputs.restype = i
+        lib.pg_parsing_to_encoder_inputs.argtypes = [vp] * 9 + [i, i, i, i, i, vp]
         lib.pg_modconv_dcoefs.restype = i
         lib.pg_modconv_dcoefs.argtypes = [vp, vp, vp, i, i, i, i, f, vp]
         lib.pg_modconv_w2.restype = i
@@ -161,13 +163,13 @@
         lib.pg_conv3x3_cin1.restype = i
         lib.pg_conv3x3_cin1.argtypes = [vp, vp, vp, i, i, i, i, f, i, vp]
         lib.pg_conv1x1_small.restype = i
-        lib.pg_conv1x1_small.argtypes = [vp] * 6 + [i, i, i64, i, f, f, vp]
+        lib.pg_conv1x1_small.argtypes = [vp] * 6 + [i, i, i64, i, f, f, i, vp]
         lib.pg_conv1x1_fold_prep.restype = i
-        lib.pg_conv1x1_fold_prep.argtypes = [vp] * 7 + [i, i, i, i, vp]
+        lib.pg_conv1x1_fold_prep.argtypes = [vp] * 7 + [i, i, i, i, i, vp]
         lib.pg_conv1x1_fold_heads.restype = i
-        lib.pg_conv1x1_fold_heads.argtypes = [vp] * 7 + [i, i, i, i64, i, i, i, f, vp]
+        lib.pg_conv1x1_fold_heads.argtypes = [vp] * 7 + [i, i, i, i64, i, i, i, f, i, vp]
         lib.pg_conv3x3_fold_head.restype = i
-        lib.pg_conv3x3_fold_head.argtypes = [vp] * 6 + [i, i, i, i, i, f, vp]
+        lib.pg_conv3x3_fold_head.argtypes = [vp] * 6 + [i, i, i, i, i, f, i, vp]
         _plugin = plugin
     return _plugin
 
@@ -679,28 +681,44 @@
             and (x.shape[2] * x.shape[3]) % 4 == 0 and int(x.shape[1]) <= 2048 and (skip is None or (skip.dtype == torch.float32 and skip.is_contiguous())))
 
 
-def conv1x1_small(x, weight, styles=None, bias=None, skip=None, scale=1.0, clamp=None):
+def skip_up2_ok(x, skip):
+    return (skip is not None and skip.dtype == torch.float32 and skip.is_cuda and skip.is_contiguous() and x.shape[2] % 2 == 0 and x.shape[3] % 4 == 0
+            and skip.shape[0] == x.shape[0] and tuple(skip.shape[2:]) == (x.shape[2] // 2, x.shape[3] // 2))
+
+
+def _skip_shape_ok(skip, n, cs, h, w, skip_up2):
+    return skip is None or tuple(skip.shape) == ((n, cs, h // 2, w // 2) if skip_up2 else (n, cs, h, w))
+
+
+def conv1x1_small(x, weight, styles=None, bias=None, skip=None, scale=1.0, clamp=None, skip_up2=False):
     lib = _init().lib
     n, cin, h, w = x.shape
     cout = int(weight.shape[0])
     wf = _f32c(weight.detach().reshape(cout, cin), 'weight')
     st = _f32c(styles.detach(), 'styles') if styles is not None else None
     b = _f32c(bias.detach(), 'bias') if bias is not None else None
+    skip_up2 = bool(skip_up2) and skip is not None
+    if skip is not None and (skip.dtype != torch.float32 or not skip.is_contiguous() or not _skip_shape_ok(skip, n, cout, h, w, skip_up2) or (skip_up2 and (h % 2 or w % 4))):
+        raise nat.NativeOpError('conv1x1_small: skip must be dense float32 [N, Cout, H, W] (or [N, Cout, H/2, W/2] with skip_up2: H even, W a multiple of 4)')
     y = torch.empty([n, cout, h, w], dtype=torch.float32, device=x.device)
     with torch.cuda.device(x.device):
         rc = lib.pg_conv1x1_small(nat.ptr(x), nat.ptr(wf), nat.ptr(st), nat.ptr(b), nat.ptr(skip), nat.ptr(y), n, cin, h * w, cout,
-                                  float(scale), float(clamp) if clamp is not None else -1.0, nat.stream_of(x))
+                                  float(scale), float(clamp) if clamp is not None else -1.0, w if skip_up2 else 0, nat.stream_of(x))
     nat.check(rc, 'pg_conv1x1_small')
     return y
 
 
-def conv1x1_fold_ok(x, x2, skip=None):
+def conv1x1_fold_ok(x, x2, skip=None, skip_up2=False):
+    if skip_up2 and not skip_up2_ok(x, skip):
+        return False
+    skip = None if skip_up2 else skip
     return (x.dtype == torch.float32 and x.is_cuda and x.is_contiguous() and x2.dtype == torch.float32 and x2.is_cuda and x2.is_contiguous()
             and x.shape[0] == x2.shape[0] and x.shape[2:] == x2.shape[2:] and (x.shape[2] * x.shape[3]) % 4 == 0
             and (skip is None or (skip.dtype == torch.float32 and skip.is_cuda and skip.is_contiguous() and skip.shape[0] == x.shape[0] and skip.shape[2:] == x.shape[2:])))
 
 
 def conv1x1_fold_prep(wm, bm, wh, bh, styles):
+    form = 1 if os.environ.get('PG_FOLD_PREP', '1') == '0' else 0
     lib = _init().lib
     wm, bm, wh, bh, styles = _f32c(wm, 'wm'), _f32c(bm, 'bm'), _f32c(wh, 'wh'), _f32c(bh, 'bh'), _f32c(styles, 'styles')
     cm, c = wm.shape
@@ -710,47 +728,53 @@
     w = torch.empty([n, cout, c], dtype=torch.float32, device=wm.device)
     b = torch.empty([n, cout], dtype=torch.float32, device=wm.device)
     with torch.cuda.device(wm.device):
-        rc = lib.pg_conv1x1_fold_prep(nat.ptr(wm), nat.ptr(bm), nat.ptr(wh), nat.ptr(bh), nat.ptr(styles), nat.ptr(w), nat.ptr(b), n, cm, c, cout, nat.stream_of(wm))
+        rc = lib.pg_conv1x1_fold_prep(nat.ptr(wm), nat.ptr(bm), nat.ptr(wh), nat.ptr(bh), nat.ptr(styles), nat.ptr(w), nat.ptr(b), n, cm, c, cout, form, nat.stream_of(wm))
     nat.check(rc, 'pg_conv1x1_fold_prep')
     return w, b
 
 
-def conv1x1_fold_heads(x, x2, w, b, c_a, skip=None, clamp=None):
+def conv1x1_fold_heads(x, x2, w, b, c_a, skip=None, clamp=None, skip_up2=False):
     lib = _init().lib
     x, x2, w, b, skip = _f32c(x, 'x'), _f32c(x2, 'x2'), _f32c(w, 'w'), _f32c(b, 'b'), _f32c(skip, 'skip')
     n, c1, h, wd = x.shape
     c2, cout, c_a = int(x2.shape[1]), int(w.shape[1]), int(c_a)
     n_skip = int(skip.shape[1]) if skip is not None else 0
+    skip_up2 = bool(skip_up2) and skip is not None
     if (tuple(x2.shape) != (n, c2, h, wd) or tuple(w.shape) != (n, cout, c1 + c2) or tuple(b.shape) != (n, cout) or not 0 < c_a <= cout
-            or (skip is not None and (tuple(skip.shape) != (n, n_skip, h, wd) or n_skip > cout))):
-        raise nat.NativeOpError('conv1x1_fold_heads: x [N, C1, H, W], x2 [N, C2, H, W], w [N, Cout, C1 + C2], b [N, Cout], skip [N, <= Cout, H, W]')
+            or not _skip_shape_ok(skip, n, n_skip, h, wd, skip_up2) or n_skip > cout or (skip_up2 and (h % 2 or wd % 4))):
+        raise nat.NativeOpError('conv1x1_fold_heads: x [N, C1, H, W], x2 [N, C2, H, W], w [N, Cout, C1 + C2], b [N, Cout], skip [N, <= Cout, H, W] '
+                                '(or [N, <= Cout, H/2, W/2] with skip_up2: H even, W a multiple of 4)')
     ya = torch.empty([n, c_a, h, wd], dtype=torch.float32, device=x.device)
     yb = torch.empty([n, cout - c_a, h, wd], dtype=torch.float32, device=x.device) if c_a < cout else None
     with torch.cuda.device(x.device):
         rc = lib.pg_conv1x1_fold_heads(nat.ptr(x), nat.ptr(x2), nat.ptr(w), nat.ptr(b), nat.ptr(skip), nat.ptr(ya), nat.ptr(yb), n, c1, c2, h * wd, cout, c_a,
-                                       n_skip, float(clamp) if clamp is not None else -1.0, nat.stream_of(x))
+                                       n_skip, float(clamp) if clamp is not None else -1.0, wd if skip_up2 else 0, nat.stream_of(x))
     nat.check(rc, 'pg_conv1x1_fold_heads')
     return ya, yb
 
 
-def conv3x3_fold_ok(xa, xb, skip=None):
+def conv3x3_fold_ok(xa, xb, skip=None, skip_up2=False):
+    if skip_up2 and not skip_up2_ok(xa, skip):
+        return False
+    skip = None if skip_up2 else skip
     return (xa.dtype == torch.float32 and xa.is_cuda and xa.is_contiguous() and xb.dtype == torch.float32 and xb.is_cuda and xb.is_contiguous()
             and xa.shape == xb.shape
             and (skip is None or (skip.dtype == torch.float32 and skip.is_cuda and skip.is_contiguous() and skip.shape[0] == xa.shape[0] and skip.shape[2:] == xa.shape[2:])))
 
 
-def conv3x3_fold_head(xa, xb, w, b, skip=None, clamp=None):
+def conv3x3_fold_head(xa, xb, w, b, skip=None, clamp=None, skip_up2=False):
     lib = _init().lib
     xa, xb, w, b, skip = _f32c(xa, 'xa'), _f32c(xb, 'xb'), _f32c(w, 'w'), _f32c(b, 'b'), _f32c(skip, 'skip')
     n, c, h, wd = xa.shape
     cout = int(w.shape[1])
+    skip_up2 = bool(skip_up2) and skip is not None
     if (tuple(xb.shape) != (n, c, h, wd) or tuple(w.shape) != (n, cout, 10 * c) or tuple(b.shape) != (n, cout)
-            or (skip is not None and tuple(skip.shape) != (n, cout, h, wd))):
-        raise nat.NativeOpError('conv3x3_fold_head: xa, xb [N, C, H, W], w [N, Cout, 10 C], b [N, Cout], skip [N, Cout, H, W]')
+            or not _skip_shape_ok(skip, n, cout, h, wd, skip_up2) or (skip_up2 and (h % 2 or wd % 4))):
+        raise nat.NativeOpError('conv3x3_fold_head: xa, xb [N, C, H, W], w [N, Cout, 10 C], b [N, Cout], skip [N, Cout, H, W] (or [N, Cout, H/2, W/2] with skip_up2)')
     y = torch.empty([n, cout, h, wd], dtype=torch.float32, device=xa.device)
     with torch.cuda.device(xa.device):
         rc = lib.pg_conv3x3_fold_head(nat.ptr(xa), nat.ptr(xb), nat.ptr(w), nat.ptr(b), nat.ptr(skip), nat.ptr(y), n, c, h, wd, cout,
-                                      float(clamp) if clamp is not None else -1.0, nat.stream_of(xa))
+                                      float(clamp) if clamp is not None else -1.0, int(skip_up2), nat.stream_of(xa))
     nat.check(rc, 'pg_conv3x3_fold_head')
     return y
 
@@ -927,3 +951,22 @@
         nat.check(lib.pg_spade_feat_assemble(nat.ptr(fu), nat.ptr(fl), nat.ptr(mu), nat.ptr(ml), nat.ptr(du), nat.ptr(dl), nat.ptr(sums[0]), nat.ptr(sums[1]),
                                              nat.ptr(counts[0]), nat.ptr(counts[1]), nat.ptr(out), n, c, h, w, st), 'pg_spade_feat_assemble')
     return out
+
+
+def parsing_to_encoder_inputs(pred_parsing, denorm_upper_input, denorm_lower_input, parsing_index=None):
+    lib = _init().lib
+    du, dl = _f32c(denorm_upper_input, 'denorm_upper_input'), _f32c(denorm_lower_input, 'denorm_lower_input')
+    n, ci, h, w = du.shape
+    given = parsing_index is not None
+    src = _f32c(parsing_index if given else pred_parsing.detach(), 'parsing_index' if given else 'pred_parsing')
+    c = int(src.shape[1])
+    if dl.shape != du.shape or src.ndim != 4 or src.shape[0] != n or tuple(src.shape[2:]) != (h, w) or (given and c != 1) or not 1 <= c <= 16:
+        raise nat.NativeOpError('parsing_to_encoder_inputs: pred_parsing [N, C <= 16, H, W] or parsing_index [N, 1, H, W], denorm inputs [N, Ci, H, W] x2')
+    index = src if given else torch.empty([n, 1, h, w], dtype=torch.float32, device=du.device)
+    mu, ml = torch.empty_like(index), torch.empty_like(index)
+    eu, el = torch.empty_like(du), torch.empty_like(dl)
+    with torch.cuda.device(du.device):
+        rc = lib.pg_parsing_to_encoder_inputs(None if given else nat.ptr(src), nat.ptr(src) if given else None, nat.ptr(du), nat.ptr(dl),
+                                              None if given else nat.ptr(index), nat.ptr(mu), nat.ptr(ml), nat.ptr(eu), nat.ptr(el), n, c, ci, h, w, nat.stream_of(du))
+    nat.check(rc, 'pg_parsing_to_encoder_inputs')
+    return index, mu, ml, eu, el
diff --git a/pasta-gan-plusplus_amd/training/networks.py b/pasta-gan-plusplus_amd/training/networks.py
--- a/pasta-gan-plusplus_amd/training/networks.py
+++ b/pasta-gan-plusplus_amd/training/networks.py
@@ -984,6 +984,11 @@
     return hit[1]
 
 
+def _fp32_head_up2_ok(x, skip_img, f):
+    return (os.environ.get('PG_HEAD_UP2', '1') != '0' and x.is_cuda and x.dtype == torch.float32 and not torch.is_grad_enabled()
+            and conv2d_mfma.skip_up2_ok(x, skip_img) and _is_1331(f))
+
+
 class _ToRGBBase(nn.Module):
     PARSING_CHANNELS = 7
 
@@ -1015,14 +1020,18 @@
             if self.is_last and self.is_style:
                 pred_parsing = conv2d_mfma16.conv1x1_small(x, self.m_weight1, styles, self.m_bias1, clamp=self.conv_clamp)
             return conv2d_mfma16.conv1x1_small(x, self.weight, styles, self.bias, skip=skip_img, clamp=self.conv_clamp, skip_up2=up2), pred_parsing
+        up2 = False
         if skip_up2_filter is not None and skip_img is not None:
-            skip_img = upfirdn2d.upsample2d(skip_img, skip_up2_filter)
+            up2 = (_fp32_head_up2_ok(x, skip_img, skip_up2_filter) and _fast_ok(x, self.weight, self.bias, styles, skip_img)
+                   and conv2d_mfma.conv1x1_small_ok(x, self.weight) and os.environ.get('PG_HEAD_STREAM', '1') != '0')
+            if not up2:
+                skip_img = upfirdn2d.upsample2d(skip_img, skip_up2_filter)
         fast = _fast_ok(x, self.weight, self.bias, styles, skip_img)
         if fast and conv2d_mfma.conv1x1_small_ok(x, self.weight, skip_img) and os.environ.get('PG_HEAD_STREAM', '1') != '0':
             pred_parsing = None
             if self.is_last and self.is_style:
                 pred_parsing = conv2d_mfma.conv1x1_small(x, self.m_weight1, styles, self.m_bias1, clamp=self.conv_clamp)
-            return conv2d_mfma.conv1x1_small(x, self.weight, styles, self.bias, skip=skip_img, clamp=self.conv_clamp), pred_parsing
+            return conv2d_mfma.conv1x1_small(x, self.weight, styles, self.bias, skip=skip_img, clamp=self.conv_clamp, skip_up2=up2), pred_parsing
         pred_parsing = None
         if self.is_last and self.is_style:
             if fast:
@@ -1095,7 +1104,7 @@
         convs = [self.conv1] if self.in_channels == 0 else [self.conv0, self.conv1]
         return [(m, i, 1.0) for i, m in enumerate(convs)] + ([(self.torgb, self.num_conv, self.torgb.weight_gain)] if self.has_torgb else [])
 
-    def _heads_folded(self, x, feat, w, styles, img):
+    def _heads_folded(self, x, feat, w, styles, img, up2=False):
         mc, tr = getattr(self, 'merge_conv', None), getattr(self, 'torgb', None)
         if mc is None or tr is None or self.TEXTURE or self.architecture != 'skip' or os.environ.get('PG_HEAD_FOLD', '1') == '0' or os.environ.get('PG_HEAD_STREAM', '1') == '0':
             return None
@@ -1104,7 +1113,7 @@
             return None
         parsing = tr.is_last and tr.is_style
         params = [mc.weight, tr.weight, tr.bias] + ([mc.bias] if mc.bias is not None else []) + ([tr.m_weight1, tr.m_bias1] if parsing else [])
-        if not (_fast_ok(x, feat, styles, img, tr.affine.weight, tr.affine.bias, *params) and conv2d_mfma.conv1x1_fold_ok(x, feat, img)):
+        if not (_fast_ok(x, feat, styles, img, tr.affine.weight, tr.affine.bias, *params) and conv2d_mfma.conv1x1_fold_ok(x, feat, img, skip_up2=up2)):
             return None
 
         def build():
@@ -1119,17 +1128,20 @@
             styles = tr.affine(w) * tr.weight_gain
         try:
             wn, bn = conv2d_mfma.conv1x1_fold_prep(wm, bm, wh, bh, styles)
-            return conv2d_mfma.conv1x1_fold_heads(x, feat, wn, bn, int(tr.weight.shape[0]), skip=img, clamp=tr.conv_clamp)
+            return conv2d_mfma.conv1x1_fold_heads(x, feat, wn, bn, int(tr.weight.shape[0]), skip=img, clamp=tr.conv_clamp, skip_up2=up2)
         except nat.NativeNotCovered:
             return None
 
-    def _merge_heads(self, x, feat, w, styles, img, fused_modconv, feat_unused=False):
+    def _merge_heads(self, x, feat, w, styles, img, fused_modconv, feat_unused=False, skip_up2_filter=None):
         if feat_unused:
-            heads = self._heads_folded(x, feat, w, styles, img)
+            up2 = skip_up2_filter is not None and img is not None
+            if up2 and not _fp32_head_up2_ok(x, img, skip_up2_filter):
+                img, up2, skip_up2_filter = upfirdn2d.upsample2d(img, skip_up2_filter), False, None
+            heads = self._heads_folded(x, feat, w, styles, img, up2=up2)
             if heads is not None:
                 return (None,) + tuple(heads)
         x = self.merge_conv(x, x2=feat)
-        rgb, pred_parsing = self.torgb(x, w, fused_modconv=fused_modconv, skip_img=img, styles=styles)
+        rgb, pred_parsing = self.torgb(x, w, fused_modconv=fused_modconv, skip_img=img, styles=styles, skip_up2_filter=skip_up2_filter if img is not None else None)
         return x, rgb, pred_parsing
 
     def _tail_fold_ok(self):
@@ -1142,11 +1154,11 @@
                 and tuple(c1.weight.shape[2:]) == (3, 3) and c1.padding == 1 and tuple(sk.weight.shape[2:]) == (1, 1) and sk.padding == 0
                 and c1.weight.shape[1] == sk.weight.shape[1] and tuple(tr.weight.shape[2:]) == (1, 1) and not (tr.is_last and tr.is_style))
 
-    def _tail_folded(self, h, s, w, styles, img):
+    def _tail_folded(self, h, s, w, styles, img, up2=False):
         sb, tr = self.spade_b512, self.torgb
         c1, sk = sb.conv1, sb.skip
         params = [c1.weight, sk.weight, tr.weight, tr.bias]
-        if not (_fast_ok(h, s, styles, img, tr.affine.weight, tr.affine.bias, *params) and conv2d_mfma.conv3x3_fold_ok(h, s, img)):
+        if not (_fast_ok(h, s, styles, img, tr.affine.weight, tr.affine.bias, *params) and conv2d_mfma.conv3x3_fold_ok(h, s, img, skip_up2=up2)):
             return None
 
         def build():
@@ -1158,18 +1170,21 @@
             styles = tr.affine(w) * tr.weight_gain
         try:
             wn, bn = conv2d_mfma.conv1x1_fold_prep(wm, None, wh, bh, styles)
-            return conv2d_mfma.conv3x3_fold_head(h, s, wn, bn, skip=img, clamp=tr.conv_clamp)
+            return conv2d_mfma.conv3x3_fold_head(h, s, wn, bn, skip=img, clamp=tr.conv_clamp, skip_up2=up2)
         except nat.NativeNotCovered:
             return None
 
-    def _spade_heads(self, x, parsing, w, styles, img, fused_modconv, feat_unused=False):
+    def _spade_heads(self, x, parsing, w, styles, img, fused_modconv, feat_unused=False, skip_up2_filter=None):
         x = self.spade_b512(x, parsing, _defer_tail=feat_unused and self._tail_fold_ok())
         if isinstance(x, tuple):
-            rgb = self._tail_folded(*x, w, styles, img)
+            up2 = skip_up2_filter is not None and img is not None
+            if up2 and not _fp32_head_up2_ok(x[0], img, skip_up2_filter):
+                img, up2, skip_up2_filter = upfirdn2d.upsample2d(img, skip_up2_filter), False, None
+            rgb = self._tail_folded(*x, w, styles, img, up2=up2)
             if rgb is not None:
                 return None, rgb, None
             x = self.spade_b512.tail(*x)
-        rgb, pred_parsing = self.torgb(x, w, fused_modconv=fused_modconv, skip_img=img, styles=styles)
+        rgb, pred_parsing = self.torgb(x, w, fused_modconv=fused_modconv, skip_img=img, styles=styles, skip_up2_filter=skip_up2_filter if img is not None else None)
         return x, rgb, pred_parsing
 
     def _forward(self, x, img, ws, pose_feature, cat_feat, parsing, force_fp32, fused_modconv, styles=None, _feat_unused=False, **layer_kwargs):
@@ -1199,25 +1214,27 @@
                     if _feat_unused and self.has_torgb and not self.TEXTURE and not half:
                         if img is not None:
                             misc.assert_shape(img, [None, self.img_channels, self.resolution // 2, self.resolution // 2])
-                            img = upfirdn2d.upsample2d(img, self.resample_filter)
-                        x, rgb, pred_parsing = self._merge_heads(x, feat, style(self.num_conv), st[self.num_conv], img, fused_modconv, feat_unused=True)
+                        x, rgb, pred_parsing = self._merge_heads(x, feat, style(self.num_conv), st[self.num_conv], img, fused_modconv, feat_unused=True,
+                                                                 skip_up2_filter=self.resample_filter)
                         return x, rgb.to(dtype=torch.float32, memory_format=torch.contiguous_format), pred_parsing
                     x = self.merge_conv(x, x2=feat)
                 if self.TEXTURE:
                     if _feat_unused and self.has_torgb and not half:
                         if img is not None:
                             misc.assert_shape(img, [None, self.img_channels, self.resolution // 2, self.resolution // 2])
-                            img = upfirdn2d.upsample2d(img, self.resample_filter)
-                        x, rgb, pred_parsing = self._spade_heads(x, parsing, style(self.num_conv), st[self.num_conv], img, fused_modconv, feat_unused=True)
+                        x, rgb, pred_parsing = self._spade_heads(x, parsing, style(self.num_conv), st[self.num_conv], img, fused_modconv, feat_unused=True,
+                                                                 skip_up2_filter=self.resample_filter)
                         return x, rgb.to(dtype=torch.float32, memory_format=torch.contiguous_format), pred_parsing
                     x = self.spade_b512(x, parsing)
 
         if img is not None:
             misc.assert_shape(img, [None, self.img_channels, self.resolution // 2, self.resolution // 2])
-            img = upfirdn2d.upsample2d(img, self.resample_filter)
+            if not self.has_torgb or half:
+                img = upfirdn2d.upsample2d(img, self.resample_filter)
         pred_parsing = None
         if self.has_torgb:
-            rgb, pred_parsing = self.torgb(x, style(self.num_conv), fused_modconv=fused_modconv, skip_img=img, styles=st[self.num_conv])
+            rgb, pred_parsing = self.torgb(x, style(self.num_conv), fused_modconv=fused_modconv, skip_img=img, styles=st[self.num_conv],
+                                           skip_up2_filter=self.resample_filter if (img is not None and not half) else None)
             img = rgb.to(dtype=torch.float32, memory_format=torch.contiguous_format)
         return x, img, pred_parsing
 
@@ -1375,16 +1392,30 @@
             kept[res] = (x, img)
         x_256, img_256 = kept[self.block_resolutions[-2]]
 
-        if gt_parsing is not None:
-            parsing_index = gt_parsing
+        fast = _fast_ok(x_256, denorm_upper_input, denorm_lower_input, denorm_upper_mask, denorm_lower_mask) and denorm_upper_mask.dtype == torch.float32
+        src = gt_parsing if gt_parsing is not None else pred_parsing
+        enc_in = None
+        if (fast and os.environ.get('PG_PARSING_FUSED', '1') != '0' and src is not None and src.ndim == 4 and src.is_cuda and src.dtype == torch.float32 and src.shape[1] <= 16
+                and (gt_parsing is None or gt_parsing.shape[1] == 1) and denorm_upper_input.dtype == denorm_lower_input.dtype == torch.float32
+                and denorm_upper_input.shape == denorm_lower_input.shape and denorm_upper_input.shape[0] == src.shape[0]
+                and denorm_upper_input.shape[2:] == src.shape[2:] and not _needs_graph(src)):
+            parsing_index, upper_mask, lower_mask, *enc_in = conv2d_mfma.parsing_to_encoder_inputs(
+                pred_parsing, denorm_upper_input, denorm_lower_input, parsing_index=gt_parsing)
+            if gt_parsing is not None:
+                parsing_index = gt_parsing
         else:
-            parsing_index = pred_parsing.detach().argmax(dim=1, keepdim=True).float()
-        upper_mask = ((parsing_index == 1) | (parsing_index == 4)).float()
-        lower_mask = ((parsing_index == 2) | (parsing_index == 3)).float()
-
-        if _fast_ok(x_256, denorm_upper_input, denorm_lower_input, denorm_upper_mask, denorm_lower_mask) and denorm_upper_mask.dtype == torch.float32:
-            feat_u = self.spade_encoder(torch.where(upper_mask > 0.9, denorm_upper_input, -1.0))
-            feat_l = self.spade_encoder(torch.where(lower_mask > 0.9, denorm_lower_input, -1.0))
+            if gt_parsing is not None:
+                parsing_index = gt_parsing
+            else:
+                parsing_index = pred_parsing.detach().argmax(dim=1, keepdim=True).float()
+            upper_mask = ((parsing_index == 1) | (parsing_index == 4)).float()
+            lower_mask = ((parsing_index == 2) | (parsing_index == 3)).float()
+
+        if fast:
+            if enc_in is None:
+                enc_in = [torch.where(upper_mask > 0.9, denorm_upper_input, -1.0), torch.where(lower_mask > 0.9, denorm_lower_input, -1.0)]
+            feat_u = self.spade_encoder(enc_in[0])
+            feat_l = self.spade_encoder(enc_in[1])
             spade_feat = conv2d_mfma.spade_feat_assemble(feat_u, feat_l, upper_mask, lower_mask, denorm_upper_mask, denorm_lower_mask)
         else:
             spade_feat = (self.get_spade_feat(upper_mask.detach(), denorm_upper_mask, denorm_upper_input) * (_half_nearest(upper_mask) > 0.9)
```

Result: no change. 294.8, median of 6 (+0.7%).
